# ml-jku/LaM-SLidE

Measured on AMD Instinct MI355X. Metric: sampled trajectories/sec (50-step ODE) + decoded-coord L2 vs ref, MD17, higher is better.
Workload: dtype bf16; 1 GPU; md17_bench; tail=False, ln_fuse=True, T=30, L=256, C=32, D=512, H=16, depth=4, sampler=ODE, state_updates=50, batch_per_gpu=32, global_batch=32, parallelism=batch-shard x1, 1 gather to rank 0 per step, noise_elem_stride_per_rank=7864320, kernels=general, trajectories_per_pass=32

## Files before the change

### include/lsl_api.h

```cpp
#ifndef LSL_API_H
#define LSL_API_H

#include <stddef.h>
#include <stdint.h>

#ifdef __cplusplus
extern "C" {
#endif
#if defined(__GNUC__)
#pragma GCC visibility push(default)
#endif

#define LSL_VERSION 6

typedef struct lsl_model lsl_model;

typedef struct lsl_model_desc {
    int32_t in_dim;
    int32_t hidden;
    int32_t heads;
    int32_t head_dim;
    int32_t head_dim_pad;
    int32_t mlp_dim;
    int32_t depth;
// ... 66 lines not shown
int32_t lsl_model_tail(const lsl_model *m);

int lsl_model_set_ln_fuse(lsl_model *m, int32_t on);
int32_t lsl_model_ln_fuse(const lsl_model *m);

int32_t lsl_pass_size(const lsl_model *m, int32_t B, int32_t T, int32_t L);

int32_t lsl_sampler_path(const lsl_model *m, int32_t T, int32_t L);

size_t lsl_workspace_bytes(const lsl_model *m, int32_t B, int32_t T, int32_t L);

int lsl_forward(lsl_model *m, const lsl_io *io, void *workspace, size_t workspace_bytes, void *stream);

size_t lsl_forward_jvp_workspace_bytes(const lsl_model *m, int32_t B, int32_t T, int32_t L);
int lsl_forward_jvp(lsl_model *m, const lsl_io *io, const float *x_tangent, float *out_tangent, void *workspace, size_t workspace_bytes,
                    void *stream);
int lsl_dot_rows(const float *a, const float *b, int32_t B, uint64_t per_trajectory, double *out, void *scratch, size_t scratch_bytes,
                 void *stream);

typedef struct lsl_si_row { float alpha, sigma, p, q1, q0, w; } lsl_si_row;
#define LSL_SI_SLAB 4096
size_t lsl_si_loss_workspace_bytes(const lsl_model *m, int32_t B, int32_t T, int32_t L);
int lsl_si_loss(lsl_model *m, const lsl_io *io, const float *x1, const float *x0, const lsl_si_row *rows, float *loss,
                void *workspace, size_t workspace_bytes, void *stream);
int lsl_si_reduce(const float *pred, const float *x1, const float *x0, const lsl_si_row *rows, int32_t B, uint64_t per_trajectory,
                  float *loss, void *scratch, size_t scratch_bytes, void *stream);

int lsl_geom_loss_sums(const float *pred, const float *target, const uint8_t *mask, int32_t F, int32_t A, int32_t D, float *sums, void *stream);
int lsl_geom_loss_final(const float *sums, int32_t F, float *out, void *stream);

int lsl_peptide_loss_sums(const float *pred, const float *target_frame, const uint8_t *atom14_mask, const float *tors_target, const uint8_t *tors_mask,
                          const int64_t *aatype, const int8_t *restab, int32_t F, int32_t R, int32_t kind, float *sums, void *stream);
int lsl_peptide_loss_final(const float *geom_sums, const float *pept_sums, int32_t F, float *out, void *stream);

int lsl_class_loss_sums(const float *logits, const int64_t *target, const uint8_t *mask, int32_t F, int32_t A, int32_t K, float label_smoothing,
                        float *sums, int64_t *confusion, void *stream);
int lsl_class_loss_final(const float *sums, int32_t F, float *out, void *stream);

int lsl_disp_error_rows(const float *pred, const float *target, int32_t K, int32_t B, int32_t Tp, int32_t t0p, int32_t Tt, int32_t t0t, int32_t Tf,
                        int32_t A, int32_t D, float *rows, float *traj, void *stream);
int lsl_disp_error_final(const float *rows, const float *traj, const uint8_t *mask, int32_t K, int32_t num_runs, int32_t B, int32_t A, float *agents,
                         double *totals, void *stream);

int lsl_dihedral_angles(const float *pos, const int32_t *quads, const int32_t *quads_host, int64_t F, int32_t A, int32_t Q, float *angles,
                        void *stream);
int lsl_histogram(const float *x, int32_t S, int32_t n, int32_t Q, const double *edges, int32_t bins, int64_t *counts, const int32_t *pairs,
                  const int32_t *pairs_host, int32_t P, const double *edges2a, const double *edges2b, int32_t bins2, int64_t *counts2, void *stream);
size_t lsl_lag_products_workspace_bytes(int32_t S, int32_t n, int32_t C, int32_t nlag);
int lsl_lag_products(const float *x, int32_t S, int32_t n, int32_t C, int32_t nlag, float *ac, void *workspace, size_t workspace_bytes, void *stream);
int lsl_js_distance(const int64_t *counts_a, const int64_t *counts_b, int32_t rows, int32_t bins, double *out, void *stream);

int lsl_pair_distances(const float *pos, const int32_t *pairs, const int32_t *pairs_host, int64_t F, int32_t A, int32_t P, float *dist,
                       void *stream);
int lsl_ca_frame_stats(const float *pos, const int32_t *sel, const int32_t *sel_host, int64_t F, int32_t A, int32_t R, float clash_thr,
                       float break_thr, float contact_thr, float *rg, int32_t *flags, int64_t *tally, int64_t *contacts, void *stream);
int lsl_histogram_columns(const float *x, int32_t n, int32_t Q, const double *edges, int32_t bins, int64_t *counts, void *stream);
int lsl_js_distance_density(const int64_t *counts_a, const int64_t *counts_b, const double *measure, int32_t rows, int32_t bins, double pseudo,
                            double *out, void *stream);

size_t lsl_lagged_moments_workspace_bytes(int32_t S, int32_t n, int32_t F, int32_t lag);
int lsl_lagged_moments(const float *x, int32_t S, int32_t n, int32_t F, int32_t lag, double *moments, void *workspace, size_t workspace_bytes,
                       void *stream);
int lsl_project(const float *x, int32_t n, int32_t F, const double *mean, const double *W, int32_t d, float *y, float *lim, void *stream);
int lsl_assign_centers(const float *y, int32_t n, int32_t d, const float *centers, int32_t k, const int32_t *map, int32_t nstates, int32_t *labels,
                       int64_t *state_counts, void *stream);
int lsl_transition_counts(const int32_t *dtraj, int32_t S, int32_t n, int32_t lag, int32_t nstates, int64_t *counts, void *stream);

size_t lsl_weighted_moments_workspace_bytes(int32_t n, int32_t F, int32_t lag);
int lsl_weighted_moments(const float *x, int32_t n, int32_t F, int32_t lag, const double *w, double *moments, void *workspace, size_t workspace_bytes,
                         void *stream);
int lsl_affine_weights(const float *x, int32_t m, int32_t F, const double *u, double c, double *w, void *stream);
int lsl_project_wide(const float *x, int32_t n, int32_t F, const double *mean, const double *W, int32_t d, float *y, float *lim, void *stream);

size_t lsl_kmeans_workspace_bytes(int32_t S, int32_t n, int32_t d, int32_t k);
int lsl_kmeans_step(const float *y, int32_t S, int32_t n, int32_t d, float *centers, int32_t k, int32_t *labels, int64_t *counts, double *state,
                    int32_t *done, int32_t update, double rel_tol, double center_tol, void *workspace, size_t workspace_bytes, void *stream);
int lsl_kmeans_nearest_rows(const float *y, int32_t S, int32_t n, int32_t d, const float *centers, int32_t k, int32_t *rows, void *stream);

int lsl_msm_active_set(const int64_t *counts, int32_t S, int32_t ns, int32_t *active, int32_t *n_active, void *stream);
int lsl_msm_reversible_step(const int64_t *counts, const int32_t *active, int32_t S, int32_t ns, int32_t iters, int32_t maxiter, double maxerr,
                            int32_t restart, double *x, int32_t *n_iter, double *err, int32_t *done, void *stream);
int lsl_msm_transition_matrix(const int64_t *counts, const int32_t *active, const double *x, int32_t S, int32_t ns, double *T, double *pi, void *stream);

#define LSL_SUP_CENTER_ONLY 1
int lsl_superpose(const float *pos, const float *ref, int32_t ref_frames, const int32_t *sel, const int32_t *sel_host, int32_t n_sel,
                  const uint8_t *fixed, int64_t F, int32_t A, int32_t flags, float *out, float *rmsd, double *rot, double *trans, void *stream);
size_t lsl_atom_rmsf_workspace_bytes(int64_t F, int32_t A);
int lsl_atom_rmsf(const float *pos, int64_t F, int32_t A, double *mean_out, float *rmsf_out, void *workspace, size_t workspace_bytes,
                  void *stream);

int lsl_sample_ex(lsl_model *m, const lsl_io *io, const lsl_step_ex *steps, int32_t n_steps,
                  const float *noise, int32_t n_noise, uint64_t seed, uint64_t elem_offset, float *trace, int32_t n_trace,
                  void *workspace, size_t workspace_bytes, void *stream);
int lsl_sample(lsl_model *m, const lsl_io *io, const lsl_step *steps, int32_t n_steps,
               const float *noise, int32_t n_noise, uint64_t seed, uint64_t elem_offset, float *trace,
               void *workspace, size_t workspace_bytes, void *stream);

int lsl_randn(float *x, uint64_t n, uint64_t seed, uint64_t elem_offset, void *stream);

#define LSL_RK_SCRATCH_BYTES 8192
int lsl_rk_lincomb(float *out, const float *const *x, const float *c, int32_t n_x, uint64_t n, void *stream);
int lsl_rk_dense(float *out, const float *a, const float *b, const float *c, const float *d, const float *e, float x, uint64_t n, void *stream);
int lsl_rk_error_ratio(float *ratio, const float *y0, const float *y1, const float *const *k, const float *c, int32_t n_k, float atol, float rtol,
                       uint64_t n, void *scratch, void *stream);

#define LSL_DOPRI_MAX_ATTEMPTS 100000
#define LSL_DOPRI_CTL_OFFSET 0
#define LSL_DOPRI_LOG_OFFSET 256
#define LSL_DOPRI_STATE_OFFSET (256 + 32 * LSL_DOPRI_MAX_ATTEMPTS)
enum { LSL_PATH_LINEAR = 0, LSL_PATH_GVP = 1, LSL_PATH_VP = 2 };
enum { LSL_PRED_VELOCITY = 0, LSL_PRED_DATA = 1, LSL_PRED_NOISE = 2, LSL_PRED_SCORE = 3 };
enum { LSL_DOPRI_OK = 0, LSL_DOPRI_MAX_STEPS = 1, LSL_DOPRI_NON_FINITE = 2 };
typedef struct lsl_dopri_desc {
    int32_t path_type, model_type, reverse, max_steps;
    double rtol, atol;
} lsl_dopri_desc;
typedef struct lsl_dopri_ctl {
    double t, dt, t_lo;
    double ratio, t_new, dt_next;
    double rtol, atol;
    float *out;
    int32_t accept, out_end;
    int32_t accepted, rejected, nfe, next_out, done, status;
    int32_t n_out, max_steps, path_type, model_type, reverse;
} lsl_dopri_ctl;
size_t lsl_dopri_workspace_bytes(const lsl_model *m, int32_t B, int32_t T, int32_t L, int32_t n_out);
int lsl_dopri_begin(lsl_model *m, const lsl_io *io, const lsl_dopri_desc *desc, const double *grid, int32_t n_out, float *out, void *workspace,
                    size_t workspace_bytes, void *stream);
int lsl_dopri_advance(lsl_model *m, const lsl_io *io, int32_t n_attempts, void *workspace, size_t workspace_bytes, void *stream);

#define LSL_DOPRI_EACH_SUMMARY_OFFSET 0
#define LSL_DOPRI_EACH_CTL_OFFSET 256
#define LSL_DOPRI_EACH_LOG_OFFSET(B) (256 + 256 * ((128 * (size_t)(B) + 255) / 256))
#define LSL_DOPRI_EACH_STATE_OFFSET(B, log_rows) (LSL_DOPRI_EACH_LOG_OFFSET(B) + 256 * ((32 * (size_t)(B) * (size_t)(log_rows) + 255) / 256))
typedef struct lsl_dopri_each_summary {
    int32_t B;
    int32_t n_done;
    int32_t n_failed;
    int32_t max_attempts;
    int32_t done;
} lsl_dopri_each_summary;
size_t lsl_dopri_each_workspace_bytes(const lsl_model *m, int32_t B, int32_t T, int32_t L, int32_t n_out, int32_t log_rows);
int lsl_dopri_each_begin(lsl_model *m, const lsl_io *io, const lsl_dopri_desc *desc, const double *grid, int32_t n_out, float *out,
                         int32_t log_rows, void *workspace, size_t workspace_bytes, void *stream);
int lsl_dopri_each_advance(lsl_model *m, const lsl_io *io, int32_t n_attempts, void *workspace, size_t workspace_bytes, void *stream);

int lsl_debug_dopri_coeffs(int32_t path_type, int32_t model_type, const float *t, int32_t n, double *out, void *stream);

int lsl_debug_block(lsl_model *m, int32_t block_index , const float *h_in, float *h_out,
                    const float *mods , int32_t B, int32_t T, int32_t L,
                    void *workspace, size_t workspace_bytes, void *stream);
int lsl_debug_block_ex(lsl_model *m, int32_t block_index, const float *h_in, float *h_out, void *a_out, const float *mods, int32_t mod_rows,
                       int32_t B, int32_t T, int32_t L, void *workspace, size_t workspace_bytes, void *stream);
int lsl_debug_taps(lsl_model *m, int32_t block_index, const float *h_in, const float *mods, int32_t B, int32_t T, int32_t L,
                   void *qkv_out, void *z_out, void *workspace, size_t workspace_bytes, void *stream);
int lsl_debug_mods(lsl_model *m, const float *t, const float *y, int32_t B, float *vec_out, float *mods_out,
                   void *workspace, size_t workspace_bytes, void *stream);
int lsl_debug_mods_ex(lsl_model *m, const float *t, float t_scalar, const float *y, int32_t B, float *vec_out, float *mods_out, float *tfeat_out,
                      float *hid_out, float *yhid_out, float *yemb_out, void *workspace, size_t workspace_bytes, void *stream);
int lsl_debug_mods_steps(lsl_model *m, const float *times, int32_t count, float *mods_out, float *vec_out, void *workspace, size_t workspace_bytes,
                         void *stream);
int lsl_debug_embed(lsl_model *m, const float *x, const float *x_cond, const int64_t *mask, int32_t B, int32_t T, int32_t L, float *cond_emb_out,
                    float *h_out, float *hn_out, void *stats_out, void *workspace, size_t workspace_bytes, void *stream);
int lsl_debug_head(lsl_model *m, const float *h, const float *mods, int32_t mod_rows, float *x, float *out, const lsl_step_ex *rec, const float *noise,
                   uint64_t seed, uint64_t elem_offset, float *trace, const float *saved, float *save_out, int32_t B, int32_t T, int32_t L,
                   void *stream);

int lsl_profile_enable(lsl_model *m, int32_t kernel, int32_t max_launches);
const char *lsl_profile_kernel_name(const lsl_model *m);
int lsl_profile_read(lsl_model *m, double *total_ms, int32_t *launches);

typedef struct lsl_dec_block {
    const float *ln_w, *ln_b;
    const float *lnc_w, *lnc_b;
    const float *w_q;
    const float *w_kv;
    const float *w_out, *b_out;
    const float *q_scale, *k_scale;
    const float *ff_ln_w, *ff_ln_b;
    const float *ff_w1, *ff_b1;
    const float *ff_w2, *ff_b2;
} lsl_dec_block;

typedef struct lsl_decoder_desc {
    int32_t in_dim;
    int32_t dim_latent, dim_query, dim_emb, n_entities;
    int32_t heads_latent, dim_head_latent, heads_cross, dim_head_cross;
    int32_t num_block_attn, num_block_cross;
    int32_t act;
    int32_t out_dim;
    int32_t num_split;
} lsl_decoder_desc;

typedef struct lsl_decoder_weights {
    const float *pq_w, *pq_b;
    const float *table;
    const float *qm_w, *qm_b;
    const lsl_dec_block *self_blocks;
    const lsl_dec_block *cross_blocks;
    lsl_dec_block out_block;
    const float *ext_w, *ext_b;
    const float *head_w1, *head_b1;
    const float *head_w2, *head_b2;
} lsl_decoder_weights;

typedef struct lsl_decoder lsl_decoder;
int lsl_decoder_create(const lsl_decoder_desc *desc, const lsl_decoder_weights *w, lsl_decoder **out);
void lsl_decoder_destroy(lsl_decoder *d);
size_t lsl_decode_workspace_bytes(const lsl_decoder *d, int32_t frames, int32_t L, int32_t A);
int lsl_decode(lsl_decoder *d, const float *z, const int64_t *entities, int32_t frames, int32_t L, int32_t A, float *out,
               void *workspace, size_t workspace_bytes, void *stream);

#define LSL_DECODE_MAX_HEADS 8
typedef struct lsl_decoder_head {
    const float *w1, *b1;
    const float *w2, *b2;
    int32_t out_dim;
} lsl_decoder_head;
int lsl_decode_heads(lsl_decoder *d, const lsl_decoder_head *heads, int32_t n_heads, const float *z, const int64_t *entities,
                     int32_t frames, int32_t L, int32_t A, float *const *outs, void *workspace, size_t workspace_bytes, void *stream);

typedef struct lsl_encoder_desc {
    int32_t dim_input, dim_emb, n_entities, dim_latent, num_latents;
    int32_t heads_cross, dim_head_cross, heads_latent, dim_head_latent;
    int32_t num_block_cross, num_block_attn;
    int32_t act;
} lsl_encoder_desc;

typedef struct lsl_encoder_weights {
    const float *table;
    const float *mlp_w1, *mlp_b1;
    const float *mlp_w2, *mlp_b2;
    const float *latents;
    const lsl_dec_block *cross_blocks;
    const lsl_dec_block *self_blocks;
    const float *quant_w, *quant_b;
} lsl_encoder_weights;

typedef struct lsl_encoder lsl_encoder;
int lsl_encoder_create(const lsl_encoder_desc *desc, const lsl_encoder_weights *w, lsl_encoder **out);
void lsl_encoder_destroy(lsl_encoder *e);
size_t lsl_encode_workspace_bytes(const lsl_encoder *e, int32_t frames, int32_t A);
int lsl_encode(lsl_encoder *e, const float *x, const int64_t *entities, const unsigned char *mask, int32_t frames, int32_t A, float *out,
               void *workspace, size_t workspace_bytes, void *stream);

#if defined(__GNUC__)
#pragma GCC visibility pop
#endif
#ifdef __cplusplus
}
#endif
#endif
```

### lam_slide_amd/_lib.py

```python
from __future__ import annotations

import ctypes as C
import os
import subprocess
from collections import OrderedDict
from typing import Optional

import torch

_HERE = os.path.dirname(os.path.abspath(__file__))
LIB_PATH = os.path.join(_HERE, "liblamslide_hip.so")
SRC_DIR = os.path.join(_HERE, "csrc")
INCLUDE_DIR = os.path.join(os.path.dirname(_HERE), "include")

ABI_VERSION = 6
RK_SCRATCH_BYTES = 8192
GEOM_MAX_A, GEOM_MAX_D = 2048, 4
DISP_MAX_D, DISP_MAX_UNITS = 4, 16777215
TORS_MAX_A, TORS_MAX_Q, HIST_MAX_BINS, HIST2_MAX_BINS = 2044, 65536, 2048, 90
LAG_CHUNK, LAG_MAX_LAGS, LAG_MAX_ROWS = 448, 1 << 21, 65535
MOM_SEG = 1024
MOM_CHAIN = MOM_SEG
MOM_MAX_F, PROJ_MAX_D = 128, 16
ASG_MAX_K, ASG_MAX_D, ASG_CELLS, ASG_MAX_STATES, TR_MAX_STATES = 1024, 64, 8192, 1024, 128
KM_SEG, KM_MAX_S = 2048, 65535
WMOM_MIN_F, WMOM_MAX_F, WPROJ_MAX_D = 129, 2048, 64
WMOM_SEG, WMOM_CHAIN = 1024, 4130
PAIR_MAX_P, CA_MAX_R = 65536, 146
SI_SLAB = 4096
CLS_MAX_K, CLS_IGNORE = 128, -100

EXPORTED = (
    "lsl_version", "lsl_build_info", "lsl_last_error", "lsl_model_create", "lsl_model_set_weights", "lsl_model_destroy",
    "lsl_model_set_chunk", "lsl_model_set_attention_mode", "lsl_model_set_tail", "lsl_model_tail", "lsl_model_set_ln_fuse", "lsl_model_ln_fuse", "lsl_profile_kernel_name", "lsl_pass_size", "lsl_sampler_path", "lsl_workspace_bytes", "lsl_forward", "lsl_sample", "lsl_sample_ex", "lsl_debug_block", "lsl_debug_block_ex", "lsl_debug_taps", "lsl_debug_mods",
    "lsl_debug_mods_ex", "lsl_debug_mods_steps", "lsl_debug_embed", "lsl_debug_head",
    "lsl_si_loss_workspace_bytes", "lsl_si_loss", "lsl_si_reduce", "lsl_geom_loss_sums", "lsl_geom_loss_final",
    "lsl_peptide_loss_sums", "lsl_peptide_loss_final", "lsl_disp_error_rows", "lsl_disp_error_final",
    "lsl_dihedral_angles", "lsl_histogram", "lsl_lag_products_workspace_bytes", "lsl_lag_products", "lsl_js_distance",
    "lsl_pair_distances", "lsl_ca_frame_stats", "lsl_histogram_columns", "lsl_js_distance_density",
    "lsl_lagged_moments_workspace_bytes", "lsl_lagged_moments", "lsl_project", "lsl_assign_centers", "lsl_transition_counts",
    "lsl_kmeans_workspace_bytes", "lsl_kmeans_step", "lsl_kmeans_nearest_rows",
    "lsl_weighted_moments_workspace_bytes", "lsl_weighted_moments", "lsl_affine_weights", "lsl_project_wide",
    "lsl_msm_active_set", "lsl_msm_reversible_step", "lsl_msm_transition_matrix",
    "lsl_superpose", "lsl_atom_rmsf_workspace_bytes", "lsl_atom_rmsf",
    "lsl_profile_enable", "lsl_profile_read", "lsl_randn", "lsl_rk_lincomb", "lsl_rk_dense", "lsl_rk_error_ratio",
    "lsl_dopri_workspace_bytes", "lsl_dopri_begin", "lsl_dopri_advance", "lsl_debug_dopri_coeffs",
    "lsl_dopri_each_workspace_bytes", "lsl_dopri_each_begin", "lsl_dopri_each_advance",
    "lsl_forward_jvp_workspace_bytes", "lsl_forward_jvp", "lsl_dot_rows",
    "lsl_decoder_create", "lsl_decoder_destroy", "lsl_decode_workspace_bytes", "lsl_decode",
    "lsl_encoder_create", "lsl_encoder_destroy", "lsl_encode_workspace_bytes", "lsl_encode",
    "lsl_decode_heads", "lsl_class_loss_sums", "lsl_class_loss_final",
)


def mom_segments(n: int, lag: int) -> int:
    return -(-(int(n) - int(lag)) // MOM_SEG)


class ModelDesc(C.Structure):
    _fields_ = [(n, C.c_int32) for n in ("in_dim", "hidden", "heads", "head_dim", "head_dim_pad", "mlp_dim", "depth",
                                         "vec_in_dim", "normalize")] + [("theta", C.c_float)]


class BlockWeights(C.Structure):
    _fields_ = [(n, C.c_void_p) for n in ("w1", "b1", "qs", "ks", "w2", "b2")]


class Weights(C.Structure):
    _fields_ = [(n, C.c_void_p) for n in (
        "x_in_w", "x_in_b", "cond_w", "cond_b", "mask_emb", "time_freqs", "time_w1", "time_b1", "time_w2", "time_b2",
        "vec_w1", "vec_b1", "vec_w2", "vec_b2", "mod_w", "mod_b", "out_w", "out_b")] + [("blocks", C.POINTER(BlockWeights))]


class IO(C.Structure):
    _fields_ = [("x", C.c_void_p), ("x_cond", C.c_void_p), ("mask", C.c_void_p), ("y", C.c_void_p), ("t", C.c_void_p),
                ("out", C.c_void_p), ("B", C.c_int32), ("T", C.c_int32), ("L", C.c_int32)]


class DecBlock(C.Structure):
    _fields_ = [(n, C.c_void_p) for n in ("ln_w", "ln_b", "lnc_w", "lnc_b", "w_q", "w_kv", "w_out", "b_out", "q_scale", "k_scale",
                                          "ff_ln_w", "ff_ln_b", "ff_w1", "ff_b1", "ff_w2", "ff_b2")]


class DecoderDesc(C.Structure):
    _fields_ = [(n, C.c_int32) for n in ("in_dim", "dim_latent", "dim_query", "dim_emb", "n_entities", "heads_latent", "dim_head_latent",
                                         "heads_cross", "dim_head_cross", "num_block_attn", "num_block_cross", "act", "out_dim", "num_split")]


class DecoderWeights(C.Structure):
    _fields_ = [("pq_w", C.c_void_p), ("pq_b", C.c_void_p), ("table", C.c_void_p), ("qm_w", C.c_void_p), ("qm_b", C.c_void_p),
                ("self_blocks", C.POINTER(DecBlock)), ("cross_blocks", C.POINTER(DecBlock)), ("out_block", DecBlock),
                ("ext_w", C.c_void_p), ("ext_b", C.c_void_p), ("head_w1", C.c_void_p), ("head_b1", C.c_void_p), ("head_w2", C.c_void_p), ("head_b2", C.c_void_p)]


class DecoderHead(C.Structure):
    _fields_ = [("w1", C.c_void_p), ("b1", C.c_void_p), ("w2", C.c_void_p), ("b2", C.c_void_p), ("out_dim", C.c_int32)]


class EncoderDesc(C.Structure):
    _fields_ = [(n, C.c_int32) for n in ("dim_input", "dim_emb", "n_entities", "dim_latent", "num_latents", "heads_cross", "dim_head_cross",
                                         "heads_latent", "dim_head_latent", "num_block_cross", "num_block_attn", "act")]


class EncoderWeights(C.Structure):
    _fields_ = [("table", C.c_void_p), ("mlp_w1", C.c_void_p), ("mlp_b1", C.c_void_p), ("mlp_w2", C.c_void_p), ("mlp_b2", C.c_void_p),
                ("latents", C.c_void_p), ("cross_blocks", C.POINTER(DecBlock)), ("self_blocks", C.POINTER(DecBlock)),
                ("quant_w", C.c_void_p), ("quant_b", C.c_void_p)]


class Step(C.Structure):
    _fields_ = [("t", C.c_float), ("ax", C.c_float), ("am", C.c_float), ("aw", C.c_float)]


class StepEx(C.Structure):
    _fields_ = [("t", C.c_float), ("ax", C.c_float), ("am", C.c_float), ("aw", C.c_float), ("as_", C.c_float), ("flags", C.c_int32),
                ("noise_index", C.c_int32), ("trace_index", C.c_int32)]


class SiRow(C.Structure):
    _fields_ = [(n, C.c_float) for n in ("alpha", "sigma", "p", "q1", "q0", "w")]


STEP_NO_NETWORK, STEP_SAVE = 1, 2


class DopriDesc(C.Structure):
    _fields_ = [(n, C.c_int32) for n in ("path_type", "model_type", "reverse", "max_steps")] + [("rtol", C.c_double), ("atol", C.c_double)]


class DopriCtl(C.Structure):
    _fields_ = [(n, C.c_double) for n in ("t", "dt", "t_lo", "ratio", "t_new", "dt_next", "rtol", "atol")] + [("out", C.c_void_p)] + [
        (n, C.c_int32) for n in ("accept", "out_end", "accepted", "rejected", "nfe", "next_out", "done", "status", "n_out", "max_steps", "path_type",
                                 "model_type", "reverse")]


class DopriEachSummary(C.Structure):
    _fields_ = [(n, C.c_int32) for n in ("B", "n_done", "n_failed", "max_attempts", "done")]


class Dopri:
    MAX_ATTEMPTS = 100000
    CTL_OFFSET, LOG_OFFSET, STATE_OFFSET = 0, 256, 256 + 32 * MAX_ATTEMPTS
    PATHS = {"LINEAR": 0, "GVP": 1, "VP": 2}
    PREDICTIONS = {"VELOCITY": 0, "DATA": 1, "NOISE": 2, "SCORE": 3}
    STATUS_MAX_STEPS, STATUS_NON_FINITE = 1, 2
    EACH_SUMMARY_OFFSET, EACH_CTL_OFFSET, EACH_CTL_STRIDE, EACH_MAX_B = 0, 256, 128, 65535

    @staticmethod
    def each_log_offset(B: int) -> int:
        return 256 + 256 * ((128 * int(B) + 255) // 256)

    @staticmethod
    def each_state_offset(B: int, log_rows: int) -> int:
        return Dopri.each_log_offset(B) + 256 * ((32 * int(B) * int(log_rows) + 255) // 256)


BASE_FLAGS = ("-O3", "--offload-arch=gfx950", "-std=c++17", "-fPIC", "-fvisibility=hidden", "-Wno-unused-value")
UNITS = (("lsl_api.hip", ()), ("unit_lin1.hip", ("-fno-slp-vectorize",)), ("unit_loss.hip", ()), ("unit_stat.hip", ()), ("unit_stage1.hip", ()))
BUILD_DIR = os.path.join(_HERE, "build")


def unit_options(extra) -> str:
    return " ".join(BASE_FLAGS[:1] + tuple(extra))


def build(force: bool = False, verbose: bool = False) -> str:
    from concurrent.futures import ThreadPoolExecutor
    srcs = [os.path.join(SRC_DIR, f) for f in sorted(os.listdir(SRC_DIR))] + [os.path.join(INCLUDE_DIR, "lsl_api.h"), os.path.abspath(__file__)]
    if not force and os.path.exists(LIB_PATH) and all(os.path.getmtime(LIB_PATH) >= os.path.getmtime(s) for s in srcs):
        return LIB_PATH
    hipcc = os.environ.get("HIPCC", "/opt/rocm/bin/hipcc")
    os.makedirs(BUILD_DIR, exist_ok=True)

    def run(cmd):
        res = subprocess.run(cmd, capture_output=True, text=True)
        if verbose or res.returncode != 0:
            print(" ".join(cmd))
            print(res.stdout + res.stderr)
        if res.returncode != 0:
            raise RuntimeError("hipcc failed building liblamslide_hip.so")

    objs = [os.path.join(BUILD_DIR, os.path.splitext(name)[0] + ".o") for name, _ in UNITS]
    cmds = [[hipcc, *BASE_FLAGS, *extra, f'-DLSL_UNIT_OPTIONS="{unit_options(extra)}"', "-c", os.path.join(SRC_DIR, name), "-o", obj]
            for (name, extra), obj in zip(UNITS, objs)]
    with ThreadPoolExecutor(max_workers=min(16, len(cmds))) as pool:
        list(pool.map(run, cmds))
    run([hipcc, "--offload-arch=gfx950", "-shared", "-fPIC", "-Wl,--version-script=" + os.path.join(SRC_DIR, "exports.map"), "-o", LIB_PATH, *objs])
    return LIB_PATH


class LibraryMissing(RuntimeError):
    """liblamslide_hip.so has not been built (the only failure a caller may treat as "no library": anything else - a HIP error, an
    out-of-memory condition - propagates)."""


_lib: Optional[C.CDLL] = None


def load() -> C.CDLL:
    global _lib
    if _lib is not None:
        return _lib
    if not os.path.exists(LIB_PATH):
        raise LibraryMissing(f"{LIB_PATH} is missing: run `python -c 'import __graft_entry__ as g; g.build()'` "
                           "(the HIP extension is the only compute path of lam_slide_amd)")
    lib = C.CDLL(LIB_PATH)
    missing = [s for s in EXPORTED if not hasattr(lib, s)]
    if missing:
        raise RuntimeError(f"{LIB_PATH} is stale: it lacks {', '.join(missing)}; rebuild it (python -c 'import __graft_entry__ as g; g.build()')")
    lib.lsl_version.restype = C.c_int
    lib.lsl_build_info.restype = C.c_char_p
    lib.lsl_last_error.restype = C.c_char_p
    lib.lsl_model_create.argtypes = [C.POINTER(ModelDesc), C.POINTER(C.c_void_p)]
    lib.lsl_model_set_weights.argtypes = [C.c_void_p, C.POINTER(Weights)]
    lib.lsl_model_destroy.argtypes = [C.c_void_p]
    lib.lsl_model_destroy.restype = None
    lib.lsl_model_set_chunk.argtypes = [C.c_void_p, C.c_int32]
    lib.lsl_model_set_attention_mode.argtypes = [C.c_void_p, C.c_int32]
    lib.lsl_model_set_tail.argtypes = [C.c_void_p, C.c_int32]
    lib.lsl_model_tail.argtypes = [C.c_void_p]
    lib.lsl_model_set_ln_fuse.argtypes = [C.c_void_p, C.c_int32]
    lib.lsl_model_ln_fuse.argtypes = [C.c_void_p]
    lib.lsl_profile_kernel_name.argtypes = [C.c_void_p]
    lib.lsl_profile_kernel_name.restype = C.c_char_p
    lib.lsl_pass_size.argtypes = [C.c_void_p, C.c_int32, C.c_int32, C.c_int32]
    lib.lsl_sampler_path.argtypes = [C.c_void_p, C.c_int32, C.c_int32]
    lib.lsl_workspace_bytes.argtypes = [C.c_void_p, C.c_int32, C.c_int32, C.c_int32]
    lib.lsl_workspace_bytes.restype = C.c_size_t
    lib.lsl_forward.argtypes = [C.c_void_p, C.POINTER(IO), C.c_void_p, C.c_size_t, C.c_void_p]
    lib.lsl_sample.argtypes = [C.c_void_p, C.POINTER(IO), C.POINTER(Step), C.c_int32, C.c_void_p, C.c_int32, C.c_uint64, C.c_uint64,
                               C.c_void_p, C.c_void_p, C.c_size_t, C.c_void_p]
    lib.lsl_sample_ex.argtypes = [C.c_void_p, C.POINTER(IO), C.POINTER(StepEx), C.c_int32, C.c_void_p, C.c_int32, C.c_uint64, C.c_uint64,
                                  C.c_void_p, C.c_int32, C.c_void_p, C.c_size_t, C.c_void_p]
    lib.lsl_debug_block.argtypes = [C.c_void_p, C.c_int32, C.c_void_p, C.c_void_p, C.c_void_p, C.c_int32, C.c_int32, C.c_int32,
                                    C.c_void_p, C.c_size_t, C.c_void_p]
    lib.lsl_debug_block_ex.argtypes = [C.c_void_p, C.c_int32, C.c_void_p, C.c_void_p, C.c_void_p, C.c_void_p, C.c_int32, C.c_int32, C.c_int32,
                                       C.c_int32, C.c_void_p, C.c_size_t, C.c_void_p]
    lib.lsl_debug_taps.argtypes = [C.c_void_p, C.c_int32, C.c_void_p, C.c_void_p, C.c_int32, C.c_int32, C.c_int32, C.c_void_p, C.c_void_p,
                                   C.c_void_p, C.c_size_t, C.c_void_p]
    lib.lsl_debug_mods.argtypes = [C.c_void_p, C.c_void_p, C.c_void_p, C.c_int32, C.c_void_p, C.c_void_p, C.c_void_p, C.c_size_t,
                                   C.c_void_p]
    lib.lsl_debug_mods_ex.argtypes = [C.c_void_p, C.c_void_p, C.c_float, C.c_void_p, C.c_int32] + [C.c_void_p] * 6 + [C.c_void_p, C.c_size_t, C.c_void_p]
    lib.lsl_debug_mods_steps.argtypes = [C.c_void_p, C.POINTER(C.c_float), C.c_int32, C.c_void_p, C.c_void_p, C.c_void_p, C.c_size_t, C.c_void_p]
    lib.lsl_debug_embed.argtypes = [C.c_void_p, C.c_void_p, C.c_void_p, C.c_void_p, C.c_int32, C.c_int32, C.c_int32] + [C.c_void_p] * 4 + [
        C.c_void_p, C.c_size_t, C.c_void_p]
    lib.lsl_debug_head.argtypes = [C.c_void_p, C.c_void_p, C.c_void_p, C.c_int32, C.c_void_p, C.c_void_p, C.POINTER(StepEx), C.c_void_p, C.c_uint64,
                                   C.c_uint64, C.c_void_p, C.c_void_p, C.c_void_p, C.c_int32, C.c_int32, C.c_int32, C.c_void_p]
    lib.lsl_forward_jvp_workspace_bytes.argtypes = [C.c_void_p, C.c_int32, C.c_int32, C.c_int32]
    lib.lsl_forward_jvp_workspace_bytes.restype = C.c_size_t
    lib.lsl_forward_jvp.argtypes = [C.c_void_p, C.POINTER(IO), C.c_void_p, C.c_void_p, C.c_void_p, C.c_size_t, C.c_void_p]
    lib.lsl_dot_rows.argtypes = [C.c_void_p, C.c_void_p, C.c_int32, C.c_uint64, C.c_void_p, C.c_void_p, C.c_size_t, C.c_void_p]
    lib.lsl_si_loss_workspace_bytes.argtypes = [C.c_void_p, C.c_int32, C.c_int32, C.c_int32]
    lib.lsl_si_loss_workspace_bytes.restype = C.c_size_t
    lib.lsl_si_loss.argtypes = [C.c_void_p, C.POINTER(IO), C.c_void_p, C.c_void_p, C.c_void_p, C.c_void_p, C.c_void_p, C.c_size_t, C.c_void_p]
    lib.lsl_si_reduce.argtypes = [C.c_void_p, C.c_void_p, C.c_void_p, C.c_void_p, C.c_int32, C.c_uint64, C.c_void_p, C.c_void_p, C.c_size_t,
                                  C.c_void_p]
    lib.lsl_geom_loss_sums.argtypes = [C.c_void_p, C.c_void_p, C.c_void_p, C.c_int32, C.c_int32, C.c_int32, C.c_void_p, C.c_void_p]
    lib.lsl_geom_loss_final.argtypes = [C.c_void_p, C.c_int32, C.c_void_p, C.c_void_p]
    lib.lsl_peptide_loss_sums.argtypes = [C.c_void_p] * 7 + [C.c_int32, C.c_int32, C.c_int32, C.c_void_p, C.c_void_p]
    lib.lsl_peptide_loss_final.argtypes = [C.c_void_p, C.c_void_p, C.c_int32, C.c_void_p, C.c_void_p]
    lib.lsl_disp_error_rows.argtypes = [C.c_void_p, C.c_void_p] + [C.c_int32] * 9 + [C.c_void_p, C.c_void_p, C.c_void_p]
    lib.lsl_disp_error_final.argtypes = [C.c_void_p, C.c_void_p, C.c_void_p] + [C.c_int32] * 4 + [C.c_void_p, C.c_void_p, C.c_void_p]
    lib.lsl_dihedral_angles.argtypes = [C.c_void_p, C.c_void_p, C.c_void_p, C.c_int64, C.c_int32, C.c_int32, C.c_void_p, C.c_void_p]
    lib.lsl_histogram.argtypes = [C.c_void_p] + [C.c_int32] * 3 + [C.c_void_p, C.c_int32, C.c_void_p, C.c_void_p, C.c_void_p, C.c_int32, C.c_void_p,
                                  C.c_void_p, C.c_int32, C.c_void_p, C.c_void_p]
    lib.lsl_lag_products_workspace_bytes.argtypes = [C.c_int32] * 4
    lib.lsl_lag_products_workspace_bytes.restype = C.c_size_t
    lib.lsl_lag_products.argtypes = [C.c_void_p] + [C.c_int32] * 4 + [C.c_void_p, C.c_void_p, C.c_size_t, C.c_void_p]
    lib.lsl_js_distance.argtypes = [C.c_void_p, C.c_void_p, C.c_int32, C.c_int32, C.c_void_p, C.c_void_p]
    lib.lsl_pair_distances.argtypes = [C.c_void_p, C.c_void_p, C.c_void_p, C.c_int64, C.c_int32, C.c_int32, C.c_void_p, C.c_void_p]
    lib.lsl_ca_frame_stats.argtypes = [C.c_void_p, C.c_void_p, C.c_void_p, C.c_int64, C.c_int32, C.c_int32, C.c_float, C.c_float, C.c_float] + [C.c_void_p] * 5
    lib.lsl_histogram_columns.argtypes = [C.c_void_p, C.c_int32, C.c_int32, C.c_void_p, C.c_int32, C.c_void_p, C.c_void_p]
    lib.lsl_js_distance_density.argtypes = [C.c_void_p, C.c_void_p, C.c_void_p, C.c_int32, C.c_int32, C.c_double, C.c_void_p, C.c_void_p]
    lib.lsl_lagged_moments_workspace_bytes.argtypes = [C.c_int32] * 4
    lib.lsl_lagged_moments_workspace_bytes.restype = C.c_size_t
    lib.lsl_lagged_moments.argtypes = [C.c_void_p] + [C.c_int32] * 4 + [C.c_void_p, C.c_void_p, C.c_size_t, C.c_void_p]
    lib.lsl_project.argtypes = [C.c_void_p, C.c_int32, C.c_int32, C.c_void_p, C.c_void_p, C.c_int32, C.c_void_p, C.c_void_p, C.c_void_p]
    lib.lsl_assign_centers.argtypes = [C.c_void_p, C.c_int32, C.c_int32, C.c_void_p, C.c_int32, C.c_void_p, C.c_int32, C.c_void_p, C.c_void_p, C.c_void_p]
    lib.lsl_transition_counts.argtypes = [C.c_void_p] + [C.c_int32] * 4 + [C.c_void_p, C.c_void_p]
    lib.lsl_weighted_moments_workspace_bytes.argtypes = [C.c_int32] * 3
    lib.lsl_weighted_moments_workspace_bytes.restype = C.c_size_t
    lib.lsl_weighted_moments.argtypes = [C.c_void_p] + [C.c_int32] * 3 + [C.c_void_p, C.c_void_p, C.c_void_p, C.c_size_t, C.c_void_p]
    lib.lsl_affine_weights.argtypes = [C.c_void_p, C.c_int32, C.c_int32, C.c_void_p, C.c_double, C.c_void_p, C.c_void_p]
    lib.lsl_project_wide.argtypes = [C.c_void_p, C.c_int32, C.c_int32, C.c_void_p, C.c_void_p, C.c_int32, C.c_void_p, C.c_void_p, C.c_void_p]
    lib.lsl_kmeans_workspace_bytes.argtypes = [C.c_int32] * 4
    lib.lsl_kmeans_workspace_bytes.restype = C.c_size_t
    lib.lsl_kmeans_step.argtypes = [C.c_void_p] + [C.c_int32] * 3 + [C.c_void_p, C.c_int32] + [C.c_void_p] * 4 + [C.c_int32, C.c_double, C.c_double,
                                    C.c_void_p, C.c_size_t, C.c_void_p]
    lib.lsl_kmeans_nearest_rows.argtypes = [C.c_void_p] + [C.c_int32] * 3 + [C.c_void_p, C.c_int32, C.c_void_p, C.c_void_p]
    lib.lsl_msm_active_set.argtypes = [C.c_void_p, C.c_int32, C.c_int32, C.c_void_p, C.c_void_p, C.c_void_p]
    lib.lsl_msm_reversible_step.argtypes = [C.c_void_p, C.c_void_p] + [C.c_int32] * 4 + [C.c_double, C.c_int32] + [C.c_void_p] * 5
    lib.lsl_msm_transition_matrix.argtypes = [C.c_void_p] * 3 + [C.c_int32, C.c_int32, C.c_void_p, C.c_void_p, C.c_void_p]
    lib.lsl_superpose.argtypes = [C.c_void_p, C.c_void_p, C.c_int32, C.c_void_p, C.c_void_p, C.c_int32, C.c_void_p, C.c_int64, C.c_int32, C.c_int32] + [C.c_void_p] * 5
    lib.lsl_atom_rmsf_workspace_bytes.argtypes = [C.c_int64, C.c_int32]
    lib.lsl_atom_rmsf_workspace_bytes.restype = C.c_size_t
    lib.lsl_atom_rmsf.argtypes = [C.c_void_p, C.c_int64, C.c_int32, C.c_void_p, C.c_void_p, C.c_void_p, C.c_size_t, C.c_void_p]
    lib.lsl_randn.argtypes = [C.c_void_p, C.c_uint64, C.c_uint64, C.c_uint64, C.c_void_p]
    lib.lsl_rk_lincomb.argtypes = [C.c_void_p, C.POINTER(C.c_void_p), C.POINTER(C.c_float), C.c_int32, C.c_uint64, C.c_void_p]
    lib.lsl_rk_dense.argtypes = [C.c_void_p] * 6 + [C.c_float, C.c_uint64, C.c_void_p]
    lib.lsl_rk_error_ratio.argtypes = [C.c_void_p, C.c_void_p, C.c_void_p, C.POINTER(C.c_void_p), C.POINTER(C.c_float), C.c_int32, C.c_float, C.c_float,
                                       C.c_uint64, C.c_void_p, C.c_void_p]
    lib.lsl_dopri_workspace_bytes.argtypes = [C.c_void_p] + [C.c_int32] * 4
    lib.lsl_dopri_workspace_bytes.restype = C.c_size_t
    lib.lsl_dopri_begin.argtypes = [C.c_void_p, C.POINTER(IO), C.POINTER(DopriDesc), C.POINTER(C.c_double), C.c_int32, C.c_void_p, C.c_void_p, C.c_size_t,
                                    C.c_void_p]
    lib.lsl_dopri_advance.argtypes = [C.c_void_p, C.POINTER(IO), C.c_int32, C.c_void_p, C.c_size_t, C.c_void_p]
    lib.lsl_dopri_each_workspace_bytes.argtypes = [C.c_void_p] + [C.c_int32] * 5
    lib.lsl_dopri_each_workspace_bytes.restype = C.c_size_t
    lib.lsl_dopri_each_begin.argtypes = [C.c_void_p, C.POINTER(IO), C.POINTER(DopriDesc), C.POINTER(C.c_double), C.c_int32, C.c_void_p, C.c_int32, C.c_void_p,
                                         C.c_size_t, C.c_void_p]
    lib.lsl_dopri_each_advance.argtypes = [C.c_void_p, C.POINTER(IO), C.c_int32, C.c_void_p, C.c_size_t, C.c_void_p]
    lib.lsl_debug_dopri_coeffs.argtypes = [C.c_int32, C.c_int32, C.c_void_p, C.c_int32, C.c_void_p, C.c_void_p]
    lib.lsl_profile_enable.argtypes = [C.c_void_p, C.c_int32, C.c_int32]
    lib.lsl_profile_read.argtypes = [C.c_void_p, C.POINTER(C.c_double), C.POINTER(C.c_int32)]
    lib.lsl_decoder_create.argtypes = [C.POINTER(DecoderDesc), C.POINTER(DecoderWeights), C.POINTER(C.c_void_p)]
    lib.lsl_decoder_destroy.argtypes = [C.c_void_p]
    lib.lsl_decoder_destroy.restype = None
    lib.lsl_decode_workspace_bytes.argtypes = [C.c_void_p, C.c_int32, C.c_int32, C.c_int32]
    lib.lsl_decode_workspace_bytes.restype = C.c_size_t
    lib.lsl_decode.argtypes = [C.c_void_p, C.c_void_p, C.c_void_p, C.c_int32, C.c_int32, C.c_int32, C.c_void_p, C.c_void_p, C.c_size_t,
                               C.c_void_p]
    lib.lsl_decode_heads.argtypes = [C.c_void_p, C.POINTER(DecoderHead), C.c_int32, C.c_void_p, C.c_void_p, C.c_int32, C.c_int32, C.c_int32,
                                     C.POINTER(C.c_void_p), C.c_void_p, C.c_size_t, C.c_void_p]
    lib.lsl_class_loss_sums.argtypes = [C.c_void_p, C.c_void_p, C.c_void_p, C.c_int32, C.c_int32, C.c_int32, C.c_float, C.c_void_p, C.c_void_p,
                                        C.c_void_p]
    lib.lsl_class_loss_final.argtypes = [C.c_void_p, C.c_int32, C.c_void_p, C.c_void_p]
    lib.lsl_encoder_create.argtypes = [C.POINTER(EncoderDesc), C.POINTER(EncoderWeights), C.POINTER(C.c_void_p)]
    lib.lsl_encoder_destroy.argtypes = [C.c_void_p]
    lib.lsl_encoder_destroy.restype = None
    lib.lsl_encode_workspace_bytes.argtypes = [C.c_void_p, C.c_int32, C.c_int32]
    lib.lsl_encode_workspace_bytes.restype = C.c_size_t
    lib.lsl_encode.argtypes = [C.c_void_p, C.c_void_p, C.c_void_p, C.c_void_p, C.c_int32, C.c_int32, C.c_void_p, C.c_void_p, C.c_size_t,
                               C.c_void_p]
    if lib.lsl_version() != ABI_VERSION:
        raise RuntimeError(f"liblamslide_hip.so reports ABI version {lib.lsl_version()}, this package binds version {ABI_VERSION}: rebuild it "
                           "(python -c 'import __graft_entry__ as g; g.build()')")
    _lib = lib
    return lib


def last_error() -> str:
    return load().lsl_last_error().decode()


def check(rc: int):
    if rc == 0:
        return
    msg = last_error()
    if rc in (-3, -20, -21):
        raise ValueError(msg)
    raise RuntimeError(f"lamslide_hip error {rc}: {msg}")


def call(dev, name: str, *args) -> None:
    fn = getattr(load(), name)
    with torch.cuda.device(dev):
        check(fn(*args, torch.cuda.current_stream(dev).cuda_stream))


def to_host(t: "torch.Tensor"):
    if not t.is_cuda:
        return t.numpy()
    mode = torch.cuda.get_sync_debug_mode()
    torch.cuda.set_sync_debug_mode("default")
    try:
        return t.cpu().numpy()
    finally:
        torch.cuda.set_sync_debug_mode(mode)


def to_device(a, dev) -> "torch.Tensor":
    import numpy as np
    t = torch.from_numpy(np.ascontiguousarray(a))
    if torch.device(dev).type != "cuda":
        return t
    mode = torch.cuda.get_sync_debug_mode()
    torch.cuda.set_sync_debug_mode("default")
    try:
        return t.to(dev)
    finally:
        torch.cuda.set_sync_debug_mode(mode)


def device_form(*tensors, dtype=torch.float32, same_device: bool = True) -> bool:
    dev, grad = tensors[0].device, torch.is_grad_enabled()
    return all(t.is_cuda and t.dtype == dtype and (t.device == dev or not same_device) and not (grad and t.requires_grad) for t in tensors)


def flat(x, lead: tuple, trailing: tuple, dtype, dev, shape_error, device_error) -> "torch.Tensor":
    if tuple(x.shape) != tuple(lead) + tuple(trailing):
# ... 47 lines not shown
```

### lam_slide_amd/csrc/host_eval.hip.h

```cpp
#pragma once
#include "host_launch.hip.h"

namespace {


int run_mods(lsl_model *m, const Workspace &ws, const float *t_dev, float t_scalar, const float *yemb, int rows,
             float *vec_out, float *mods_out, hipStream_t st) {
    const lsl_weights &w = m->w;
    const int D = m->d.hidden;
    m->prof.begin(6, st);
    hipLaunchKernelGGL(k_time_features, dim3((rows * 128 + 255) / 256), dim3(256), 0, st, ws.tfeat, t_dev, t_scalar, w.time_freqs, rows);
    const bool single = !t_dev && !yemb;
    char k1[32], k2[32], k3[32];
    const bool lab = m->prof.kernel == 6;
    launch_dense<false, true>(ws.hid, ws.tfeat, w.time_w1, w.time_b1, nullptr, rows, 256, D, 0, st, single, 0, lab ? k1 : nullptr);
    launch_dense<false, false>(vec_out, ws.hid, w.time_w2, w.time_b2, yemb, rows, D, D, D, st, single, 0, lab ? k2 : nullptr);
    launch_dense<true, false>(mods_out, vec_out, w.mod_w, w.mod_b, nullptr, rows, D, m->MODW, 0, st, single, 0, lab ? k3 : nullptr);
    if (lab) m->prof.label(6, "k_time_features > %s > %s > %s", k1, k2, k3);
    m->prof.end(6, st);
    LSL_CHECK_LAUNCH("modulation");
    return 0;
}

int run_mods_steps(lsl_model *m, const Workspace &ws, const float *times, int count, hipStream_t st) {
    const lsl_weights &w = m->w;
    const int D = m->d.hidden;
    m->prof.begin(6, st);
    for (int c0 = 0; c0 < count; c0 += 48) {
        StepTimes tt;
        const int nc = std::min(48, count - c0);
        for (int s = 0; s < nc; ++s) tt.t[s] = times[c0 + s];
        hipLaunchKernelGGL(k_time_features_steps, dim3((nc * 128 + 255) / 256), dim3(256), 0, st, ws.tf_all + (size_t)c0 * 256, tt, nc, 1, w.time_freqs);
    }
    const unsigned gy = (unsigned)((count + 7) / 8);
    hipLaunchKernelGGL((k_dense_rows<false, true>), dim3((D + 3) / 4, gy), dim3(256), 0, st, ws.hid_all, ws.tf_all, w.time_w1, w.time_b1, nullptr, count, 256, D, 0, 0);
    hipLaunchKernelGGL((k_dense_rows<false, false>), dim3((D + 3) / 4, gy), dim3(256), 0, st, ws.vec_all, ws.hid_all, w.time_w2, w.time_b2, nullptr, count, D, D, D, 0);
    hipLaunchKernelGGL((k_dense_rows<true, false>), dim3((m->MODW + 3) / 4, (unsigned)((count + 15) / 16)), dim3(256), 0, st, ws.mods_all, ws.vec_all, w.mod_w, w.mod_b, nullptr, count, D, m->MODW, 0, 0);
    m->prof.label(6, "k_time_features_steps > k_dense_rows<0, 1> > k_dense_rows<0, 0> > k_dense_rows<1, 0> (row ranges of 8, 8, 16)");
    m->prof.end(6, st);
    LSL_CHECK_LAUNCH("modulation (group of records)");
    return 0;
}

int run_yemb(lsl_model *m, const Workspace &ws, const float *y, int rows, hipStream_t st, float *yhid_tap = nullptr) {
    const lsl_weights &w = m->w;
    const int D = m->d.hidden, V = m->d.vec_in_dim;
    char k1[32], k2[32];
    const bool lab = m->prof.kernel == 6;
    launch_dense<false, true>(ws.hid, y, w.vec_w1, w.vec_b1, nullptr, rows, V, D, 0, st, false, 0, lab ? k1 : nullptr);
    if (yhid_tap) hipMemcpyAsync(yhid_tap, ws.hid, (size_t)rows * D * 4, hipMemcpyDeviceToDevice, st);
    launch_dense<false, false>(ws.yemb, ws.hid, w.vec_w2, w.vec_b2, nullptr, rows, D, D, 0, st, false, 0, lab ? k2 : nullptr);
    if (lab) m->prof.label(6, "%s > %s", k1, k2);
    LSL_CHECK_LAUNCH("vec_in");
    return 0;
}

void run_tables(const lsl_model *m, const Workspace &ws, int T, int L, hipStream_t st) {
    const int half = m->d.head_dim_pad / 2;
    if (ws.w2p) {
        const size_t per = (size_t)m->d.hidden * m->K2;
        for (int bi = 0; bi < 2 * m->d.depth; ++bi)
            hipLaunchKernelGGL(k_lin2_pack, dim3(128), dim3(256), 0, st, ws.w2p + (size_t)bi * per, (const u16 *)m->blocks[bi].w2, m->d.hidden, m->K2);
    }
    if (ws.wtail) {
        for (int bi = 0; bi < 2 * m->d.depth; ++bi)
            hipLaunchKernelGGL(k_tail_pack, dim3(256), dim3(256), 0, st, ws.wtail + (size_t)bi * ws.wtail_stride, (const u16 *)m->blocks[bi].w1,
                               (const u16 *)m->blocks[bi].w2, m->d.hidden, m->HHD, m->d.mlp_dim);
    }
    hipLaunchKernelGGL(k_rope_table, dim3((L * half + 255) / 256), dim3(256), 0, st, ws.rope_l, L, m->d.head_dim, m->d.head_dim_pad, m->d.theta);
    hipLaunchKernelGGL(k_rope_table, dim3((T * half + 255) / 256), dim3(256), 0, st, ws.rope_t, T, m->d.head_dim, m->d.head_dim_pad, m->d.theta);
    const int nb = 2 * m->d.depth;
    for (int b0 = 0; b0 < 2 * nb; b0 += 16) {
        RopeScaledJobs jobs{};
        jobs.n_jobs = std::min(16, 2 * nb - b0);
        int max_pos = 0;
        for (int k = 0; k < jobs.n_jobs; ++k) {
            const int t = b0 + k, bi = t >> 1;
            jobs.out[k] = ws.rope_qk + (size_t)t * ws.rope_qk_stride;
            jobs.scale[k] = (t & 1) ? m->blocks[bi].ks : m->blocks[bi].qs;
            jobs.n_pos[k] = (bi & 1) ? T : L;
            jobs.sq_bound[k] = ws.kmax2 + ((t & 1) ? 0 : nb) + bi;
            max_pos = std::max(max_pos, jobs.n_pos[k]);
        }
        hipLaunchKernelGGL(k_rope_scaled, dim3((max_pos * half + 255) / 256, jobs.n_jobs), dim3(256), 0, st, jobs, m->d.head_dim, m->d.head_dim_pad, m->d.theta);
    }
}


enum class PlanMode { eval, debug_block, debug_taps };
enum class Lin2Kind { none, tail, ws, gemm };

struct PassPlan {
    PlanMode mode;
    int bc, n, npad, T, L, mod_stride, blocks;
    bool tail;
    int F1;
    bool lin1_ts;
    int lin1_waves;
    bool ln_stats;
    bool emb_stats;
    int gemm1;
    bool planes[2];
    AttnPlan attn[2];
    Lin2Kind lin2;
    Lin2Grid l2grid;
    int gemm2;

    bool a_from_tail(int bi) const { return mode == PlanMode::eval && tail && bi > 0; }
    bool lin1_lnf(int bi) const { return mode == PlanMode::eval && ln_stats && (bi > 0 || emb_stats); }
    bool lin2_stats(int bi) const { return ln_stats && bi + 1 < blocks; }
};

int plan_pass(const lsl_model *m, const Workspace &ws, int bc, int T, int L, int mod_stride, PlanMode mode, int block, PassPlan &p) {
    const lsl_model_desc &d = m->d;
    const int D = d.hidden, n = bc * T * L;
    p = PassPlan{};
    p.mode = mode;
    p.bc = bc;
    p.n = n;
    p.npad = (n + 255) & ~255;
    p.T = T;
    p.L = L;
    p.mod_stride = mod_stride;
    p.blocks = 2 * d.depth;
    p.tail = m->tail && mode != PlanMode::debug_taps;
    p.F1 = p.tail ? 3 * m->HHD : m->F1;
    p.lin1_ts = linear1_ts_ok(d.head_dim_pad, D, p.F1, m->HHD, n);
    p.lin1_waves = linear1_ts_waves(D, n);
    p.ln_stats = m->ln_fuse && !m->tail && ws.w2p && mode != PlanMode::debug_taps &&
                 linear1_lnf_ok(d.head_dim_pad, D, m->F1, m->HHD, n, T * L, mod_stride);
    p.emb_stats = p.ln_stats && mode == PlanMode::eval && !d.normalize && embed_stats_ok(d.in_dim, D);
    if (!p.lin1_ts) p.gemm1 = gemm_variant(false, p.F1, D, n);
    for (int t = 0; t < 2; ++t) {
        p.attn[t] = plan_attention(m->attention_linear, d.head_dim_pad, d.heads, d.head_dim, bc, T, L, t != 0);
        p.planes[t] = qkv_planes_ok(d.head_dim_pad, d.heads, t ? T : L, t != 0, p.lin1_ts, p.attn[t]);
    }
    const bool ws_reach = ws.w2p && (unsigned long long)n * (unsigned)(4 * D) < (1ull << 32);
    if (ws_reach) p.l2grid = linear2_ws_grid(D, n, T * L, mod_stride == 0);
    const bool on_ws = ws_reach && p.l2grid.gate_rows <= linear2_ws_max_gate_rows(m->K2);
    p.lin2 = mode == PlanMode::debug_taps ? Lin2Kind::none : p.tail ? Lin2Kind::tail : on_ws ? Lin2Kind::ws : Lin2Kind::gemm;
    if (p.lin2 == Lin2Kind::gemm) p.gemm2 = gemm_variant(true, D, m->K2, n);

    const int b0 = mode == PlanMode::eval ? 0 : block, b1 = mode == PlanMode::eval ? p.blocks : block + 1;
    for (int bi = b0; bi < b1; ++bi) {
        const int temporal = bi & 1, pdiv = temporal ? L : 1, pmod = temporal ? T : L;
        if ((unsigned long long)n * (unsigned)std::max(pdiv, pmod) >= (1ull << 32)) return fail(-3, "pass too large for the position arithmetic");
        if (p.planes[temporal] && (unsigned long long)p.npad * 3ull * (unsigned)m->HHD * 2ull >= (1ull << 32))
            return fail(-3, "pass too large for the q/k/v plane offsets (%d tokens: at most %llu with this model)", n, (unsigned long long)((1ull << 32) / (6ull * (unsigned)m->HHD)) - 256);
        if (p.attn[temporal].form == AttnForm::none)
            return fail(-3, "attention axis of %d positions is not on the stream kernel and too long for k_attention_rows (at most %d positions at %d-wide heads)",
                        pmod, attention_rows_max_s(d.head_dim_pad), d.head_dim_pad);
        if (p.lin2 == Lin2Kind::none) continue;
        if ((unsigned long long)n * (unsigned)(T * L) >= (1ull << 32)) return fail(-3, "pass too large for the trajectory arithmetic");
        if (p.tail && (unsigned long long)p.npad * (unsigned)(4 * D) >= (1ull << 32)) return fail(-3, "pass too large for the residual-stream offsets");
        if (p.lin2_stats(bi) && !on_ws) {
            if (ws_reach) return fail(-3, "ln_fuse: a pass of %d tokens has too many trajectories per token range for k_linear2_ws; use smaller passes (lsl_model_set_chunk)", n);
            return fail(-3, "ln_fuse: pass too large for the residual-stream offsets (%d tokens)", n);
        }
    }
    return 0;
}

struct CallPlans {
    PassPlan full, rest;
    const PassPlan &of(int bc) const { return bc == full.bc ? full : rest; }
};
int plan_call(const lsl_model *m, const Workspace &ws, const lsl_io *io, int chunk, int mod_stride, CallPlans &cp) {
    if (int rc = plan_pass(m, ws, chunk, io->T, io->L, mod_stride, PlanMode::eval, 0, cp.full)) return rc;
    if (io->B % chunk) return plan_pass(m, ws, io->B % chunk, io->T, io->L, mod_stride, PlanMode::eval, 0, cp.rest);
    return 0;
}

void label_block(lsl_model *m, const PassPlan &p, int bi) {
    const lsl_model_desc &d = m->d;
    Profiler &pr = m->prof;
    switch (pr.kernel) {
        case 0:
            if (!p.lin1_ts) pr.label(0, "k_gemm_glds<EpiLinear1<%d>> (tiling %d)", d.head_dim_pad, p.gemm1);
            else if (p.lin1_lnf(bi)) pr.label(0, "k_linear1_ts<%d, %d, 8, true> (LayerNorm fused)", d.head_dim_pad, d.hidden);
            else pr.label(0, "k_linear1_ts<%d, %d, %d>%s", d.head_dim_pad, d.hidden, p.lin1_waves, p.tail ? " (q | k | v)" : "");
            break;
        case 1:
            if (p.lin2 == Lin2Kind::tail) pr.label(1, "k_tail<%d, %d>", d.hidden, m->HHD);
            else if (p.lin2 == Lin2Kind::ws) pr.label(1, p.lin2_stats(bi) ? "k_linear2_ws<%d> (+ row statistics)" : "k_linear2_ws<%d>", m->K2);
            else if (p.lin2 == Lin2Kind::gemm) pr.label(1, "k_gemm_glds<EpiLinear2> (tiling %d)", p.gemm2);
            break;
        case 2: {
            const AttnPlan &a = p.attn[bi & 1];
            pr.label(2, "%s", a.form == AttnForm::linear ? "k_attention_linear" : a.stream() ? "k_attention_stream" : "k_attention_rows / k_attention_tiny");
            break;
        }
        default: break;
    }
}

unsigned magic_of(int dv) { return dv == 1 ? 0u : (unsigned)((1ull << 32) / (unsigned)dv + 1); }

template <int HDP>
void launch_linear1_gemm(const lsl_model *m, const Workspace &ws, const PassPlan &p, int bi, int pdiv, int pmod, float premul, hipStream_t st) {
    const lsl_block_weights &bw = m->blocks[bi];
    const EpiLinear1<HDP> e{bw.b1, bw.qs, bw.ks, (bi & 1) ? ws.rope_t : ws.rope_l, ws.rope_qk + (size_t)(2 * bi) * ws.rope_qk_stride,
                            ws.rope_qk + (size_t)(2 * bi + 1) * ws.rope_qk_stride, ws.qkv, ws.z, m->HHD, m->d.mlp_dim,
                            pdiv, pmod, magic_of(pdiv), magic_of(pmod), 1.0f / m->d.head_dim, premul, 0};
    launch_gemm(p.gemm1, (const u16 *)bw.w1, ws.a, p.F1, p.n, m->d.hidden, e, st, m->HHD);
}

AttnArgs attention_args(const lsl_model *m, const Workspace &ws, const PassPlan &p, int bi, float premul) {
    const lsl_model_desc &d = m->d;
    const AttnPlan &ap = p.attn[bi & 1];
    static const int nt_mask = tune_int("LSL_NT", 3);
    static const int attn_bound = tune_int("LSL_ATTN_BOUND", 1);
    AttnArgs aa{};
    aa.nt = (nt_mask >> 2) & 1;
    aa.qkv = ws.qkv; aa.z = ws.z; aa.HHD = m->HHD; aa.zw = m->K2; aa.H = d.heads; aa.hd = d.head_dim; aa.premul = premul;
    aa.kmax2 = ws.kmax2 + bi;
    aa.qmax2 = ws.kmax2 + 2 * d.depth + bi;
    aa.planes = p.planes[bi & 1] ? 1 : 0;
    aa.npad = p.npad;
    aa.bound = attn_bound == 2 || (attn_bound == 1 && ((bi & 1) ? p.T : p.L) > 96);
    aa.S = ap.S; aa.n_seq = ap.n_seq; aa.inner = ap.inner; aa.outer_stride = ap.outer_stride; aa.pos_stride = ap.pos_stride;
    aa.blk = ap.blk; aa.n_tok = ap.n_tok;
    return aa;
}

struct EvalTangent {
    virtual int embedded() = 0;
    virtual int normed(int bi, const float *mbase) = 0;
    virtual int attended(int bi, const float *mbase, float premul, int pdiv, int pmod) = 0;
    virtual int head(const float *fm) = 0;
    virtual ~EvalTangent() = default;
};

int run_block(lsl_model *m, const Workspace &ws, const PassPlan &p, int bi, const float *mods, hipStream_t st, void *a_tap = nullptr,
              EvalTangent *tg = nullptr) {
    const lsl_model_desc &d = m->d;
    const lsl_block_weights &bw = m->blocks[bi];
    const int D = d.hidden, n = p.n, tpt = p.T * p.L, mod_stride = p.mod_stride, temporal = bi & 1;
    const float *mbase = mods + (size_t)(bi / 2) * 6 * D + (temporal ? 3 * D : 0);
    const bool lnf = p.lin1_lnf(bi);
    const float premul = m->attention_linear ? 1.0f : (float)(1.4426950408889634 / std::sqrt((double)d.head_dim));
    const int pdiv = temporal ? p.L : 1, pmod = temporal ? p.T : p.L;
    label_block(m, p, bi);
    if (!p.a_from_tail(bi) && !lnf) {
        m->prof.begin(3, st);
        DISPATCH_D(D, launch_ln_mod_t, ws.a, ws.h, mbase, mbase + D, mod_stride, n, tpt, st);
        m->prof.end(3, st);
        if (a_tap) hipMemcpyAsync(a_tap, ws.a, (size_t)n * D * 2, hipMemcpyDeviceToDevice, st);
    }
    if (tg)
        if (int rc = tg->normed(bi, mbase)) return rc;
    m->prof.begin(0, st);
    if (p.lin1_ts) {
        const Lin1Args la{(const u16 *)bw.w1, lnf ? (const u16 *)ws.h : ws.a, bw.b1, ws.rope_qk + (size_t)(2 * bi) * ws.rope_qk_stride,
                          ws.rope_qk + (size_t)(2 * bi + 1) * ws.rope_qk_stride, ws.qkv, ws.z, p.F1, n, m->HHD, d.mlp_dim,
                          pdiv, pmod, magic_of(pdiv), magic_of(pmod), 1.0f / d.head_dim, premul, 1, 0, p.planes[temporal] ? 1 : 0, p.npad,
                          ws.lnstat, mbase, mbase + D, mod_stride, tpt, magic_of(tpt)};
        launch_linear1_ts(d.head_dim_pad, D, p.lin1_waves, lnf, la, st);
    } else if (d.head_dim_pad == 32) launch_linear1_gemm<32>(m, ws, p, bi, pdiv, pmod, premul, st);
    else launch_linear1_gemm<16>(m, ws, p, bi, pdiv, pmod, premul, st);
    m->prof.end(0, st);

    const AttnArgs aa = attention_args(m, ws, p, bi, premul);
    m->prof.begin(2, st);
    if (d.head_dim_pad == 32) launch_attention_t<32>(p.attn[temporal], aa, st);
    else launch_attention_t<16>(p.attn[temporal], aa, st);
    m->prof.end(2, st);
    if (p.lin2 == Lin2Kind::none) {
        LSL_CHECK_LAUNCH("block");
        return 0;
    }
    if (tg)
        if (int rc = tg->attended(bi, mbase, premul, pdiv, pmod)) return rc;
    m->prof.begin(1, st);
    if (p.lin2 == Lin2Kind::tail) {
        const bool next = bi + 1 < 2 * d.depth;
        const float *nb = mods + (size_t)((bi + 1) / 2) * 6 * D + (((bi + 1) & 1) ? 3 * D : 0);
        const TailArgs ta{ws.wtail + (size_t)bi * ws.wtail_stride, ws.a, ws.z, bw.b1 + 3 * m->HHD, bw.b2, mbase + 2 * D, ws.h, next ? ws.a : nullptr,
                          nb, nb + D, n, d.mlp_dim, m->K2, mod_stride, tpt, magic_of(tpt)};
        launch_tail(ta, st);
    } else if (p.lin2 == Lin2Kind::ws) {
        const bool stats = p.lin2_stats(bi);
        const Lin2Args l2{ws.w2p + (size_t)bi * D * m->K2, ws.z, bw.b2, mbase + 2 * D, ws.h, D, n, mod_stride, tpt, magic_of(tpt),
                          p.l2grid.slices, p.l2grid.rpx, p.l2grid.gate_rows, stats ? ws.lnparts : nullptr, p.npad};
        launch_linear2_ws(m->K2, l2, st);
        if (stats) hipLaunchKernelGGL(k_ln_finalize, dim3((n + 255) / 256), dim3(256), 0, st, ws.lnstat, ws.lnparts, D / 32, p.npad, n, 32.0f);
    } else {
        const EpiLinear2 e2{bw.b2, mbase + 2 * D, ws.h, D, mod_stride, tpt, 0, magic_of(tpt)};
        launch_gemm(p.gemm2, (const u16 *)bw.w2, ws.z, D, n, m->K2, e2, st);
    }
    m->prof.end(1, st);
    LSL_CHECK_LAUNCH(p.lin2 == Lin2Kind::tail ? "block (tail)" : "block");
    return 0;
}

struct EvalArgs {
    float *x = nullptr;
    float *out = nullptr;
    const float *t = nullptr;
    bool have_y = false;
    const lsl_step_ex *rec = nullptr;
    const float *noise = nullptr;
    uint64_t seed = 0, elem_off = 0;
    float *trace = nullptr;
    const float *saved = nullptr;
    float *save_out = nullptr;
    const float *mods_ready = nullptr;
};
StepUpdate step_update(const EvalArgs &e) {
    const lsl_step_ex r = e.rec ? *e.rec : lsl_step_ex{};
    return StepUpdate{e.noise, e.trace, e.saved, e.save_out, (unsigned long long)e.seed, (unsigned long long)e.elem_off, r.ax, r.am, r.aw, r.as, (unsigned)r.noise_index};
}

int run_embed(lsl_model *m, const Workspace &ws, const PassPlan &p, const float *x, hipStream_t st, float *h_tap = nullptr, EvalTangent *tg = nullptr) {
    const lsl_model_desc &d = m->d;
    const int D = d.hidden, n = p.n;
    m->prof.begin(5, st);
    launch_embed<1>(ws.h, x, m->w.x_in_w, nullptr, nullptr, nullptr, nullptr, ws.cond_emb, n, d.in_dim, D, st, p.emb_stats ? ws.lnparts : nullptr, p.npad,
                    &m->prof);
    if (p.emb_stats) hipLaunchKernelGGL(k_ln_finalize, dim3((n + 255) / 256), dim3(256), 0, st, ws.lnstat, ws.lnparts, D / 256, p.npad, n, 256.0f);
    if (h_tap) hipMemcpyAsync(h_tap, ws.h, (size_t)n * D * 4, hipMemcpyDeviceToDevice, st);
    if (tg)
        if (int rc = tg->embedded()) return rc;
    if (d.normalize) { DISPATCH_D(D, launch_ln_inplace_t, ws.h, n, 1e-5f, st); }
    m->prof.end(5, st);
    LSL_CHECK_LAUNCH("embed");
    return 0;
}

int run_head(lsl_model *m, const float *h, const float *fm, int mod_stride, int n, int tpt, const EvalArgs &e, hipStream_t st) {
    const int D = m->d.hidden;
    const HeadArgs a{e.x, e.out, h, fm, fm + D, mod_stride, m->w.out_w, m->w.out_b, n, m->d.in_dim, tpt, e.rec ? 1 : 0, step_update(e)};
    m->prof.begin(4, st);
    DISPATCH_D(D, launch_head_mfma, a, st, &m->prof);
    m->prof.end(4, st);
    LSL_CHECK_LAUNCH("head");
    return 0;
}

int run_eval(lsl_model *m, const Workspace &ws, const PassPlan &p, const EvalArgs &e, hipStream_t st, EvalTangent *tg = nullptr) {
    const lsl_model_desc &d = m->d;
    const int D = d.hidden, n = p.n;
    const lsl_step_ex r = e.rec ? *e.rec : lsl_step_ex{};
    const bool shared = p.mod_stride == 0;
    int rc = 0;
    const float *mods = ws.mods;
    if (e.mods_ready && shared) mods = e.mods_ready;
    else rc = run_mods(m, ws, e.t, r.t, e.have_y ? ws.yemb : nullptr, shared ? 1 : p.bc, ws.vec, ws.mods, st);
    if (rc) return rc;
    if ((rc = run_embed(m, ws, p, e.x, st, nullptr, tg))) return rc;
    for (int bi = 0; bi < 2 * d.depth; ++bi)
        if ((rc = run_block(m, ws, p, bi, mods, st, nullptr, tg))) return rc;
    const float *fm = mods + (size_t)d.depth * 6 * D;
    if ((rc = run_head(m, ws.h, fm, p.mod_stride, n, p.T * p.L, e, st))) return rc;
    return tg ? tg->head(fm) : 0;
}

int prepare_pass(lsl_model *m, const Workspace &ws, const float *x_cond, const int64_t *mask, const float *y, int bc, int T,
                 int L, hipStream_t st) {
    const lsl_model_desc &d = m->d;
    const int n = bc * T * L;
    launch_embed<0>(ws.cond_emb, x_cond, m->w.cond_w, m->w.cond_b, m->w.x_in_b, m->w.mask_emb, mask, nullptr, n, d.in_dim, d.hidden, st, nullptr, 0, &m->prof);
    LSL_CHECK_LAUNCH("cond_embed");
    if (y) return run_yemb(m, ws, y, bc, st);
    return 0;
}

bool resident_ok(const lsl_model *m, int T, int L) {
    static const int off = env_int("LSL_RESIDENT", 1) == 0;
    const lsl_model_desc &d = m->d;
    return !off && !m->attention_linear && d.hidden == RES_D && d.heads == RES_H && d.head_dim == RES_HD && d.head_dim_pad == RES_HD && d.mlp_dim == RES_M &&
           d.in_dim <= RES_MAX_C && d.in_dim % 4 == 0 && 2 * d.depth <= RES_MAX_BLOCKS && (long)T * L <= 48 && T <= 32 && L <= 32;
}

struct ResWorkspace {
    float *cond_emb, *yemb, *tfeat, *hid, *vec, *mods, *blkpar;
    u16 *blkw;
    int steps_per_launch;
    size_t bytes;
};
ResWorkspace carve_resident(const lsl_model *m, char *base, int B, int T, int L, bool have_y) {
    const size_t n = (size_t)B * T * L, D = m->d.hidden;
    size_t off = 0;
    auto take = [&](size_t bytes) {
        char *p = base ? base + off : nullptr;
        off += align_up(bytes, 256);
        return p;
    };
    ResWorkspace ws;
    const size_t rows = have_y ? (size_t)B : 1;
    size_t spl = ((size_t)256 << 20) / (rows * m->MODW * 4);
    ws.steps_per_launch = (int)std::max<size_t>(1, std::min<size_t>(spl, RES_MAX_STEPS));
    const size_t rt = rows * ws.steps_per_launch;
    ws.cond_emb = (float *)take(n * D * 4);
    ws.yemb = (float *)take((size_t)B * D * 4);
    ws.tfeat = (float *)take(rt * 256 * 4);
    ws.hid = (float *)take(std::max(rt, (size_t)B) * D * 4);
    ws.vec = (float *)take(rt * D * 4);
    ws.mods = (float *)take(rt * m->MODW * 4);
    ws.blkpar = (float *)take((size_t)2 * m->d.depth * RES_P_SHIFT * 4);
    ws.blkw = (u16 *)take((size_t)2 * m->d.depth * (RES_W1_ELEMS + RES_W2_ELEMS) * 2);
    ws.bytes = off;
    return ws;
}

template <int NNT>
void launch_resident(const ResArgs &a, int B, int T, int L, hipStream_t st) {
    auto kern = k_resident<NNT>;
    const size_t lds = ResLds<NNT>::bytes(T, L);
    LSL_ALLOW_LDS(kern, (size_t)163840);
    hipLaunchKernelGGL(kern, dim3(B), dim3(RES_NTHR), lds, st, a);
}

int resident_sample(lsl_model *m, const lsl_io *io, const lsl_step *steps, int n_steps, const float *noise, uint64_t seed, uint64_t elem_offset,
                    float *trace, void *workspace, hipStream_t st) {
    const lsl_model_desc &d = m->d;
    const lsl_weights &w = m->w;
    const int B = io->B, T = io->T, L = io->L, n_t = T * L, D = d.hidden;
    const bool have_y = io->y != nullptr;
    const ResWorkspace ws = carve_resident(m, (char *)workspace, B, T, L, have_y);
// ... 128 lines not shown
```

### lam_slide_amd/csrc/host_launch.hip.h

```cpp
#pragma once
#include <atomic>
#include <type_traits>

#include "host_common.hip.h"

namespace {

struct HeadArgs {
    float *x, *out;
    const float *h, *shift, *scale;
    int mod_stride;
    const float *Wo, *bo;
    int n, C, tpt, do_step;
    StepUpdate u;
};

#ifdef LSL_EXPERIMENTS
constexpr bool lsl_experiments = true;
template <int NE, int VEC>
bool launch_head_experiment(const HeadArgs &, hipStream_t);
template <class Epi>
bool launch_gemm_experiment(int, const GemmArgs &, const Epi &, hipStream_t, bool);
#else
constexpr bool lsl_experiments = false;
// ... 42 lines not shown
void launch_ln_inplace_t(float *h, int n, float eps, hipStream_t st) {
    hipLaunchKernelGGL((k_ln_inplace<NE, VEC>), dim3((n + 3) / 4), dim3(256), 0, st, h, n, eps);
}
template <int NE, int VEC>
void launch_head_mfma(const HeadArgs &a, hipStream_t st, Profiler *pr = nullptr) {
    if (launch_head_experiment<NE, VEC>(a, st)) return;
    auto kern = k_head_step_mfma<NE, VEC>;
    const size_t lds = head_mfma_lds_bytes<NE>(a.C <= 32);
    LSL_ALLOW_LDS(kern, head_mfma_lds_bytes<NE>(false));
    static const int per_cu = tune_int("LSL_HEAD_PER_CU", 2);
    const int wgs = device_cus() * (per_cu >= 2 && 2 * lds <= LDS_BUDGET ? 2 : 1);
    if (pr) pr->label(4, "k_head_step_mfma<%d, %d> (%s, %d per CU)", NE, VEC, a.C <= 32 ? "one slab" : "cycled slabs", wgs / device_cus());
    hipLaunchKernelGGL(kern, dim3(std::min((a.n + HEAD_TOK - 1) / HEAD_TOK, wgs)), dim3(256), lds, st, a.x, a.out, a.h, a.shift, a.scale, a.mod_stride,
                       a.Wo, a.bo, a.n, a.C, a.tpt, a.do_step, a.u);
}
void launch_state_affine(float *x, unsigned long long n, const StepUpdate &u, hipStream_t st) {
    hipLaunchKernelGGL(k_state_affine, dim3((unsigned)std::min<unsigned long long>((n + 255) / 256, 2048)), dim3(256), 0, st, x, n, u);
}

#define DISPATCH_D(D, FN, ...)                          \
    switch ((D) / 64) {                                 \
        case 1: FN<1, 1>(__VA_ARGS__); break;           \
        case 2: FN<2, 2>(__VA_ARGS__); break;           \
        case 3: FN<3, 1>(__VA_ARGS__); break;           \
        case 4: FN<4, 2>(__VA_ARGS__); break;           \
        case 5: FN<5, 1>(__VA_ARGS__); break;           \
        case 6: FN<6, 2>(__VA_ARGS__); break;           \
        case 7: FN<7, 1>(__VA_ARGS__); break;           \
        default: FN<8, 2>(__VA_ARGS__); break;          \
    }

bool embed_stats_ok(int C, int D) { return C <= 32 && D % 256 == 0 && D <= 512; }
template <int MODE>
int launch_embed(float *out, const float *in, const float *W, const float *b, const float *b2, const float *me,
                 const int64_t *mask, const float *base, int n, int C, int D, hipStream_t st, float2 *stats = nullptr, int npad = 0,
                 Profiler *pr = nullptr) {
    if (C > 32 && C % 8 == 0 && C <= 128 && D % 32 == 0) {
        const int tpw = 3, ngrp = (D / 32 + tpw - 1) / tpw;
        const long units = (long)((n + 31) / 32) * ngrp;
        const dim3 g((unsigned)((units + 3) / 4));
        if (pr) pr->label(5, "k_embed_mfma<%d, %d> (32-token tiles)", MODE, C / 8);
        switch (C / 8) {
#define LSL_EMB_CASE(CK) case CK: hipLaunchKernelGGL((k_embed_mfma<MODE, CK>), g, dim3(256), 0, st, out, in, W, b, b2, me, mask, base, n, C, D, tpw); return 0;
            LSL_EMB_CASE(5) LSL_EMB_CASE(6) LSL_EMB_CASE(7) LSL_EMB_CASE(8) LSL_EMB_CASE(9) LSL_EMB_CASE(10) LSL_EMB_CASE(11) LSL_EMB_CASE(12)
            LSL_EMB_CASE(13) LSL_EMB_CASE(14) LSL_EMB_CASE(15) LSL_EMB_CASE(16)
#undef LSL_EMB_CASE
        }
    }
    int tok = EMB_TOK;
    static const int stage = tune_int("LSL_EMBED_LDS", 1);
    const bool w_lds = stage && C == 32 && D % 4 == 0 && D <= 512;
    if (w_lds)
        while (tok > 16 && (n + tok - 1) / tok < 2 * device_cus()) tok /= 2;
    const dim3 grid(std::min((n + tok - 1) / tok, 2 * device_cus())), blk(256);
    const bool with_stats = stats && MODE == 1 && C <= 32 && embed_stats_ok(C, D);
    if (pr)
        pr->label(5, "k_embed<%d, %d, %d%s> (%d-token tiles%s)", C <= 32 ? 32 : C <= 64 ? 64 : C <= 96 ? 96 : 128, MODE, C <= 32 ? 4 : C <= 96 ? 2 : 1,
                  with_stats ? ", true" : "", tok, w_lds ? ", weights through LDS" : (C & 3) ? ", scalar weight loads" : "");
    if (C <= 32) {
        const size_t lds = w_lds ? embed_w_lds_bytes<32, 4>(D) : 0;
        if (with_stats) {
            auto kern = k_embed<32, 1, 4, true>;
            LSL_ALLOW_LDS(kern, (embed_w_lds_bytes<32, 4>(512)));
            hipLaunchKernelGGL(kern, grid, blk, lds, st, out, in, W, b, b2, me, mask, base, n, C, D, w_lds ? 1 : 0, tok, stats, npad);
            return 0;
        }
        auto kern = k_embed<32, MODE, 4>;
        LSL_ALLOW_LDS(kern, (embed_w_lds_bytes<32, 4>(512)));
        hipLaunchKernelGGL(kern, grid, blk, lds, st, out, in, W, b, b2, me, mask, base, n, C, D, w_lds ? 1 : 0, tok, (float2 *)nullptr, 0);
    } else if (C <= 64) hipLaunchKernelGGL((k_embed<64, MODE, 2>), grid, blk, 0, st, out, in, W, b, b2, me, mask, base, n, C, D, 0, tok, (float2 *)nullptr, 0);
    else if (C <= 96) hipLaunchKernelGGL((k_embed<96, MODE, 2>), grid, blk, 0, st, out, in, W, b, b2, me, mask, base, n, C, D, 0, tok, (float2 *)nullptr, 0);
    else hipLaunchKernelGGL((k_embed<128, MODE, 1>), grid, blk, 0, st, out, in, W, b, b2, me, mask, base, n, C, D, 0, tok, (float2 *)nullptr, 0);
    return 0;
}

template <int BF, int BT, int NWF, int NWT, int BK, int NS, bool PERSIST, class Epi>
void launch_gemm_glds(const GemmArgs &g, const Epi &epi, hipStream_t st) {
    auto kern = k_gemm_glds<BF, BT, NWF, NWT, BK, NS, PERSIST, Epi>;
    const size_t lds = GemmCfg<BF, BT, NWF, NWT, BK, NS, PERSIST, Epi>::lds_bytes + (Epi::lds_bias ? (size_t)((g.F + BF - 1) / BF) * BF * 4 : 0);
    LSL_ALLOW_LDS(kern, LDS_BUDGET);
    const int tiles = ((g.N + BT - 1) / BT) * ((g.F + BF - 1) / BF);
    int grid = tiles;
    if (PERSIST) {
        const int per_cu = (int)std::max<size_t>(1, LDS_BUDGET / lds);
        grid = device_cus() * per_cu;
        grid -= grid % 8;
        if (grid > tiles) grid = tiles;
    }
    hipLaunchKernelGGL(kern, dim3(grid), dim3(NWF * NWT * 64), lds, st, g, epi);
}

}

#ifdef LSL_EXPERIMENTS
#include "host_launch_experiments.hip.h"
#endif

namespace {

template <class Fn>
bool with_linear1_ts_instance(int hdp, int D, Fn &&fn) {
#define X(H, K) if (hdp == H && D == K) return fn(ic<H>{}, ic<K>{}), true;
    LSL_LIN1_TS_INSTANCES(X)
#undef X
    return false;
}
template <int HDP, int K, int NW = 8, bool LNF = false>
void launch_linear1_ts_t(const Lin1Args &a, hipStream_t st) {
    using C = Lin1Cfg<HDP, K, NW>;
    const int ntile = (a.N + C::TT - 1) / C::TT, nb = a.F / 32;
    const long units = (long)ntile * nb;
    int grid = (int)std::min<long>(device_cus(), units / 2);
    Lin1Args b = a;
    static const int align = tune_int("LSL_LIN1_ALIGN", 1);
    const int wpt = std::min(device_cus() / ntile, nb / 2);
    b.wpt = align && wpt >= 2 ? wpt : 0;
    if (b.wpt) grid = b.wpt * ntile;
    lsl_lin1_launch(HDP, K, NW, LNF, b, grid, LNF ? C::lds_bytes_lnf(a.F) : C::lds_bytes(a.F), st);
}
int linear1_ts_waves(int D, int N) {
    static const int nw4_max = tune_int("LSL_LIN1_NW4_MAX", 10240);
    return D == 512 && N <= nw4_max ? 4 : 8;
}
bool linear1_ts_ok(int hdp, int D, int F1, int HHD, int N) {
    static const int on = tune_int("LSL_LIN1_TS", 1);
    if (!on || F1 % 64 != 0 || HHD % 64 != 0 || N < 1) return false;
    size_t lds = 0;
    return with_linear1_ts_instance(hdp, D, [&](auto h, auto k) { lds = Lin1Cfg<decltype(h)::value, decltype(k)::value, 8>::lds_bytes(F1); }) && lds <= LDS_BUDGET;
}
int ln_fuse_env() {
    static const int v = env_int("LSL_LN_FUSE", -1);
    return v;
}
bool linear1_lnf_ok(int hdp, int D, int F1, int HHD, int N, int tpt, int mod_stride) {
    if (ln_fuse_env() == 0 || !linear1_ts_ok(hdp, D, F1, HHD, N)) return false;
    size_t lds = 0;
    int min_tpt = 0;
    with_linear1_ts_instance(hdp, D, [&](auto h, auto k) {
        using C = Lin1Cfg<decltype(h)::value, decltype(k)::value, 8>;
        lds = C::lds_bytes_lnf(F1);
        min_tpt = C::LN_SLOTS >= 3 ? C::TT / 2 : C::TT;
    });
    return (mod_stride == 0 || tpt >= min_tpt) && lds <= LDS_BUDGET;
}
void launch_linear1_ts(int hdp, int D, int waves, bool lnf, const Lin1Args &a, hipStream_t st) {
    with_linear1_ts_instance(hdp, D, [&](auto h, auto k) {
        constexpr int H = decltype(h)::value, K = decltype(k)::value;
        if (lnf) return launch_linear1_ts_t<H, K, 8, true>(a, st);
        if constexpr (K == 512) {
            if (waves == 4) return launch_linear1_ts_t<H, K, 4>(a, st);
        }
        launch_linear1_ts_t<H, K, 8>(a, st);
    });
}

#define LSL_LIN2_WS_INSTANCES(X) X(1536, 3, 3) X(1280, 4, 4) X(768, 3, 3) X(384, 3, 3)
template <class Fn>
bool with_linear2_ws_instance(int K2, Fn &&fn) {
#define X(K, NCH, NS) if (K2 == K) return fn(ic<K>{}, ic<NCH>{}, ic<NS>{}), true;
    LSL_LIN2_WS_INSTANCES(X)
#undef X
    return false;
}
bool linear2_ws_shape_ok(int D, int K2) {
    static const int on = env_int("LSL_LIN2_WS", 1);
    return on && D % 128 == 0 && D <= 512 && with_linear2_ws_instance(K2, [](auto, auto, auto) {});
}
struct Lin2Grid {
    int slices, rpx, gate_rows;
};
Lin2Grid linear2_ws_grid(int F, int N, int tpt, bool shared) {
    const int slices = F / 128, cus = device_cus(), NBLK = (N + 31) / 32;
    int rpx = std::max(1, cus / (8 * slices));
    while (rpx > 1 && 8 * rpx > NBLK) --rpx;
    const int ranges = 8 * rpx, max_blocks = (NBLK + ranges - 1) / ranges + 1;
    return {slices, rpx, shared ? 1 : (max_blocks * 32 + tpt - 1) / tpt + 1};
}
int linear2_ws_max_gate_rows(int K2) {
    int rows = 0;
    with_linear2_ws_instance(K2, [&](auto k, auto nch, auto ns) { rows = Lin2Cfg<decltype(k)::value, decltype(nch)::value, decltype(ns)::value, true>::max_gate_rows; });
    return rows;
}
template <int K, int NCH, int NS, bool LNS>
void launch_linear2_ws_t(const Lin2Args &a, hipStream_t st) {
    using C = Lin2Cfg<K, NCH, NS, true>;
    auto kern = k_linear2_ws<K, NCH, NS, true, LNS>;
    LSL_ALLOW_LDS(kern, LDS_BUDGET);
    hipLaunchKernelGGL(kern, dim3(8 * a.slices * a.rpx), dim3(512), C::lds_bytes(a.gate_rows), st, a);
}
void launch_linear2_ws(int K2, const Lin2Args &a, hipStream_t st) {
    with_linear2_ws_instance(K2, [&](auto k, auto nch, auto ns) {
        constexpr int K = decltype(k)::value, NCH = decltype(nch)::value, NS = decltype(ns)::value;
        if (a.stats) launch_linear2_ws_t<K, NCH, NS, true>(a, st);
        else launch_linear2_ws_t<K, NCH, NS, false>(a, st);
    });
}

int tail_env() {
    static const int v = env_int("LSL_TAIL", -1);
    return v;
}
bool tail_shape_ok(int D, int HHD, int M) {
    return tail_env() != 0 && D == 256 && HHD == 256 && M % 64 == 0 && M >= 64 && TailCfg<256, 256>::lds_bytes(M) <= LDS_BUDGET;
}
size_t tail_stream_bytes(const lsl_model *m) { return TailCfg<256, 256>::stream_bytes(m->d.mlp_dim); }
void launch_tail(const TailArgs &a, hipStream_t st) {
    using C = TailCfg<256, 256>;
    auto kern = k_tail<256, 256>;
    LSL_ALLOW_LDS(kern, LDS_BUDGET);
    const int nwt = (a.N + 31) / 32;
    hipLaunchKernelGGL(kern, dim3(std::min(nwt, device_cus())), dim3(512), C::lds_bytes(a.M), st, a);
}

int gemm_variant(bool lin2, int F, int K, int N) {
    static const int forced_all = tune_int("LSL_GEMM", -1);
    static const int forced_1 = tune_int("LSL_GEMM1", -1), forced_2 = tune_int("LSL_GEMM2", -1);
    const int forced_one = lin2 ? forced_2 : forced_1;
    const int forced = forced_one >= 0 ? forced_one : forced_all;
    const bool ragged = F % 256 != 0 && (F % 256 <= 128);
    const int ragged_variant = lin2 && K % 64 == 0 ? 11 : 10;
    if (forced >= 0) return forced;
    if (lin2 && F % 192 == 0 && F % 256 != 0 && K % 64 == 0 && (long)((N + 127) / 128) * (F / 192) * 2 >= (long)device_cus())
        return 28;
    if (ragged) return ragged_variant;
    static const int small_rule = tune_int("LSL_SMALL_TILES", 1);
    const long tiles256 = (long)((N + 255) / 256) * ((F + 255) / 256);
    const int cus = device_cus();
    if (small_rule && K % 64 == 0 && tiles256 * (lin2 ? 2 : 4) <= (long)cus * (lin2 ? 1 : 5))
        return 11;
    return lin2 ? (K % 128 == 0 ? 7 : 15) : (K % 128 == 0 ? 12 : 5);
}

template <class Epi>
void launch_gemm(int variant, const u16 *W, const u16 *X, int F, int N, int K, const Epi &epi_in, hipStream_t st, int hhd = 32) {
    constexpr bool lin2 = std::is_same<Epi, EpiLinear2>::value;
    static const int probe = tune_int("LSL_PROBE", 0);
    static const int stagger = tune_int("LSL_STAGGER", 0);
    GemmArgs g{W, X, F, N, K, stagger, probe};
    static const int nt = tune_int("LSL_NT", 3);
    Epi epi = epi_in;
    epi.probe = probe | ((nt >> (lin2 ? 1 : 0)) & 1 ? 32 : 0);
    const bool pp_ok = lin2 || hhd % 32 == 0;
    if (launch_gemm_experiment(variant, g, epi, st, pp_ok)) return;
    if (variant == 12 && K % 128 == 0) return launch_gemm_glds<256, 256, 2, 4, 64, 2, true>(g, epi, st);
    if constexpr (lsl_experiments || lin2) {
        if (variant == 7 && F % 32 == 0 && pp_ok && K % 128 == 0) return launch_gemm_glds<256, 256, 2, 4, 64, 2, true>(g, EpiPieces<Epi>(epi), st);
    }
    switch (variant) {
        case 5: return launch_gemm_glds<256, 256, 2, 4, 64, 2, false>(g, epi, st);
        case 10: return launch_gemm_glds<128, 128, 2, 2, 32, 3, false>(g, epi, st);
        case 11: return launch_gemm_glds<128, 128, 2, 2, 64, 2, false>(g, epi, st);
        case 28:
            if constexpr (lin2) return launch_gemm_glds<192, 128, 2, 4, 64, 3, false>(g, epi, st);
            else break;
        case 15: return launch_gemm_glds<256, 256, 4, 4, 64, 2, false>(g, epi, st);
        default: return launch_gemm_glds<256, 256, 2, 4, 64, 2, false>(g, epi, st);
    }
}


int attention_stream_mode(int S, int H) {
    static const int on = env_int("LSL_ATTN_STREAM", 1);
    if (!on) return 0;
    static const int long_min = tune_int("LSL_ATTN_LONG_MIN", 129);
    if (S >= long_min) return 2;
    if (S > 8 && S <= 32 && H % 8 == 0) return 1;
    return 0;
}

enum class AttnForm {
    linear,
    stream_short,
    stream_grouped,
    stream_long,
    stream_chunked,
    stream_chunked_den,
    tiny,
    rows,
    none
};
struct AttnPlan {
    AttnForm form;
    int stream_mode;
    int S, n_seq, inner, outer_stride, pos_stride, blk, n_tok;
    int nw, items, nkt;
    bool stream() const { return form >= AttnForm::stream_short && form <= AttnForm::stream_chunked_den; }
};
bool attention_grouped_ok(const AttnPlan &a, int H) {
    static const int on = env_int("LSL_ATTN_GROUP", 1), stream_on = env_int("LSL_ATTN_STREAM", 1);
    return on && stream_on && a.S >= 2 && a.S <= 8 && (a.S & (a.S - 1)) == 0 && a.inner == 1 && a.pos_stride == 1 && a.outer_stride == a.S && H % 8 == 0;
}
constexpr size_t attention_stream_lds(int hdp) { return (size_t)2 * 2 * 256 * hdp * 2 + (size_t)8 * 32 * hdp * 2; }
constexpr size_t attention_rows_lds(int hdp, int nw, int items, int key_rows) { return (size_t)items * 2 * key_rows * hdp * 2 + nw * sizeof(float); }
constexpr int attention_rows_max_s(int hdp) { return (int)((LDS_BUDGET - 16 * sizeof(float)) / (4 * hdp)) & ~31; }
static_assert(attention_rows_lds(32, 16, 1, attention_rows_max_s(32)) <= LDS_BUDGET && attention_rows_lds(32, 16, 1, attention_rows_max_s(32) + 32) > LDS_BUDGET);

AttnPlan plan_attention(bool linear, int hdp, int H, int hd, int bc, int T, int L, bool temporal) {
    AttnPlan p{};
    if (!temporal) {
        p.S = L; p.n_seq = bc * T; p.inner = 1; p.outer_stride = L; p.pos_stride = 1;
    } else {
        p.S = T; p.n_seq = bc * L; p.inner = L; p.outer_stride = T * L; p.pos_stride = L;
    }
    p.form = AttnForm::linear;
    if (linear) return p;
    const AttnPlan axis = p;
// ... 113 lines not shown
```

### lam_slide_amd/csrc/k_lin1.hip.h

```cpp
#pragma once
#include "k_mm_frag.hip.h"

struct Lin1Args {
    const u16 *W;
    const u16 *X;
    const float *bias;
    const float4 *rope_q, *rope_k;
    u16 *qkv;
    u16 *z;
    int F, N, HHD, M;
    int pos_div, pos_mod;
    unsigned div_magic, mod_magic;
    float inv_hd, q_premul;
    int nt;
    int wpt;
    int planes;
    int npad;
    const float2 *ln_stat;
    const float *ln_shift, *ln_scale;
    int ln_mod_stride, ln_tpt;
    unsigned ln_tpt_magic;
};

#ifndef LIN1_B2
#define LIN1_B2 1
#endif
#ifndef LIN1_B2_KMAX
#define LIN1_B2_KMAX 256
#endif

template <int HDP, int K, int NW = 8>
struct Lin1Cfg {
    static_assert(K % 128 == 0 && K <= 512, "hidden sizes 128 / 256 / 384 / 512");
    static constexpr int KS = K / 16;
    static constexpr int ROWB = 2 * K;
    static constexpr int PITCH = ROWB + 16;
    static constexpr int BLK = 32 * PITCH;
    static constexpr int NS = (LIN1_B2 && K <= LIN1_B2_KMAX) ? 4 : 3;
    static constexpr int RING = NS * BLK;
    static_assert(NW == 8 || NW == 4, "two waves per SIMD (256-token tiles) or one (128-token tiles)");
    static constexpr int TT = 32 * NW;
    static constexpr int STAGE = NW * 4096;
    static constexpr int LPR = ROWB / 16;
    static constexpr int PPW = 32 / NW;
    static constexpr size_t lds_bytes(int F) { return (size_t)RING + STAGE + (size_t)F * 4; }
    static constexpr int LN_SLOTS = K <= 256 ? 3 : 2;
    static constexpr size_t lds_bytes_lnf(int F) { return lds_bytes(F) + (size_t)LN_SLOTS * 2 * K * 4; }
};

#define LSL_LIN1_TS_INSTANCES(X) X(32, 128) X(32, 256) X(32, 384) X(32, 512) X(16, 128) X(16, 256) X(16, 384) X(16, 512)

bool lsl_lin1_launch(int hdp, int K, int waves, bool lnf, const Lin1Args &a, int grid, size_t lds, hipStream_t st);

#ifndef LSL_LIN1_HOST_SIDE

enum { LIN1_QK = 0, LIN1_V = 1, LIN1_MLP = 2 };

#ifndef LIN1_XLOAD
#define LIN1_XLOAD 1
#endif
#ifndef LIN1_PD
#define LIN1_PD 3
#endif

__device__ __forceinline__ float lin1_gelu(float x) {
    const float ax = fabsf(x);
    const float h = __builtin_amdgcn_exp2f(LSL_GELU_Q(ax));
    float relu;
    asm("v_max_f32 %0, 0, %1" : "=v"(relu) : "v"(x));
    return fmaf(-ax, h, relu);
}

template <int HDP, int K, int NW = 8, bool LNF = false>
__global__ void __launch_bounds__(NW * 64, NW / 4) k_linear1_ts(Lin1Args g) {
    using C = Lin1Cfg<HDP, K, NW>;
    constexpr int KS = C::KS, BLK = C::BLK, PPW = C::PPW, ROWB = C::ROWB;
    constexpr int NCO = HDP == 32 ? 8 : 4;
    extern __shared__ __attribute__((aligned(16))) char smem[];

    const int tid = threadIdx.x, lane = tid & 63;
    const int wave = __builtin_amdgcn_readfirstlane(tid >> 6);
    const int r = lane & 31, hf = lane >> 5;
    char *const stage = smem + C::RING + wave * 4096;
    float *const bias_lds = reinterpret_cast<float *>(smem + C::RING + C::STAGE);

    const int NB = g.F >> 5;
    const int ntile = (g.N + C::TT - 1) / C::TT;
    const long U = (long)ntile * NB;
    long i0, i1;
    if (g.wpt > 0) {
        const int tile = blockIdx.x / g.wpt, part = blockIdx.x - tile * g.wpt;
        i0 = (long)tile * NB + ((NB * part / g.wpt) & ~1);
        i1 = (long)tile * NB + (part + 1 == g.wpt ? NB : ((NB * (part + 1) / g.wpt) & ~1));
    } else {
        i0 = (U * blockIdx.x / gridDim.x) & ~1L;
        i1 = blockIdx.x + 1 == gridDim.x ? U : ((U * (blockIdx.x + 1) / gridDim.x) & ~1L);
    }
    if (i0 >= i1) return;

    for (int i = tid * 4; i < g.F; i += NW * 64 * 4) *reinterpret_cast<float4 *>(bias_lds + i) = *reinterpret_cast<const float4 *>(g.bias + i);

    const unsigned lds0 = (unsigned)(size_t)(LDS_PTR(char))(smem);
    const unsigned lane_src = lane * 16;
    const char *const w_rows = reinterpret_cast<const char *>(g.W) + (size_t)(PPW * wave) * ROWB;
    auto issue_piece = [&](const char *src, unsigned dst, auto ic) __attribute__((always_inline)) {
        constexpr int I = decltype(ic)::value & 3;
        if (decltype(ic)::value >= 4) {
            src += 4 * ROWB;
            dst += 4 * C::PITCH;
        }
        const unsigned ls = lane_src;
        if (C::LPR == 64 || lane < C::LPR) {
            if (I == 0 || decltype(ic)::value >= 4)
                asm volatile("s_add_u32 m0, %2, %3\n\ts_nop 4\n\tglobal_load_lds_dwordx4 %0, %1 offset:%4" ::"v"(ls), "s"(src), "s"(dst), "n"(16 * I), "n"(ROWB * I) : "memory", "scc");
            else
                asm volatile("s_add_u32 m0, %2, %3\n\ts_nop 0\n\tglobal_load_lds_dwordx4 %0, %1 offset:%4" ::"v"(ls), "s"(src), "s"(dst), "n"(16 * I), "n"(ROWB * I) : "memory", "scc");
        }
    };
    auto req_src = [&](int blk) __attribute__((always_inline)) { return w_rows + (size_t)blk * (32 * ROWB); };
    auto req_dst = [&](int slot) __attribute__((always_inline)) { return lds0 + slot * BLK + PPW * wave * C::PITCH; };
    auto issue = [&](int blk, int slot) __attribute__((always_inline)) {
        const char *src = req_src(blk);
        const unsigned dst = req_dst(slot);
        static_for<PPW>([&](auto pc) __attribute__((always_inline)) { issue_piece(src, dst, pc); });
    };
    const int aoff = r * C::PITCH + 16 * hf;

    bf16x8 xreg[KS];
    float4 co[NCO];
    f32x16 acc0, acc1;
    int slot_c = 0;
    int dma_blk, dma_slot;
    int n_wave = 0;
    float post = 1.0f;

    auto advance = [&](int &b) __attribute__((always_inline)) { b = b + 1 == NB ? 0 : b + 1; };
    auto next_slot = [&](int s) __attribute__((always_inline)) { return s == C::NS - 1 ? 0 : s + 1; };

    {
        int b = (int)(i0 - (i0 / NB) * NB);
        issue(b, 0);
        advance(b);
        issue(b, 1);
        advance(b);
        dma_blk = b;
        dma_slot = 2;
    }

    auto init_acc = [&](f32x16 &a, int blk) __attribute__((always_inline)) {
#pragma unroll
        for (int q4 = 0; q4 < 4; ++q4) {
            const float4 b = *reinterpret_cast<const float4 *>(bias_lds + blk * 32 + 8 * q4 + 4 * hf);
            a[4 * q4] = b.x; a[4 * q4 + 1] = b.y; a[4 * q4 + 2] = b.z; a[4 * q4 + 3] = b.w;
        }
    };
    constexpr bool B2 = LIN1_B2 != 0 && K <= LIN1_B2_KMAX;
    auto step_head = [&](auto flushed_c) __attribute__((always_inline)) {
        if (B2) {
            if (decltype(flushed_c)::value) wait_vmcnt<PPW>();
            else wait_vmcnt<0>();
        } else {
            if (decltype(flushed_c)::value) wait_vmcnt<PPW + 4>();
            else wait_vmcnt<PPW>();
        }
        __builtin_amdgcn_s_barrier();
        asm volatile("" ::: "memory");
    };
    const unsigned wr0 = (unsigned)(size_t)(LDS_PTR(char))(stage) + r * 128 + 8 * hf + ((r & 7) << 4);
    const unsigned rd0 = (unsigned)(size_t)(LDS_PTR(char))(stage) + (lane >> 3) * 128 + (((lane & 7) ^ ((lane >> 3) & 7)) << 4);
    const char *row_q = nullptr, *row_z = nullptr;
    const bool planes = g.planes != 0;
    constexpr unsigned PROW = 2u * HDP, CPH = HDP / 8;
    const unsigned plane_bytes = PROW * (unsigned)g.npad;
    const unsigned stride_q = planes ? PROW : 2u * 3 * g.HHD, stride_z = 2u * (g.HHD + g.M);
    const unsigned blk_q = planes ? (32 / HDP) * plane_bytes : 64u;
    const unsigned voff_q = planes ? ((lane & 7) / CPH) * plane_bytes + (lane >> 3) * PROW + 16 * ((lane & 7) % CPH) : (lane >> 3) * stride_q + 16 * (lane & 7);
    const unsigned voff_z = (lane >> 3) * stride_z + 16 * (lane & 7);
    const int slab_z = 3 * (g.HHD >> 5);
    const char *fl_base = nullptr;
    unsigned fl_stride8 = 0, fl_voff = 0;
    auto flush_setup = [&](int b_even) __attribute__((always_inline)) {
        const bool to_qkv = b_even < slab_z;
        fl_base = to_qkv ? row_q : row_z;
        fl_stride8 = 8 * (to_qkv ? stride_q : stride_z);
        fl_voff = to_qkv ? voff_q + blk_q * (unsigned)b_even : voff_z + 64u * (unsigned)b_even;
    };
    auto flush_read = [&](int half, u32x4 (&pk)[2]) __attribute__((always_inline)) {
#pragma unroll
        for (int i = 0; i < 2; ++i) pk[i] = *reinterpret_cast<const LDS_PTR(u32x4)>(rd0 + 1024 * (2 * half + i));
    };
    auto flush_store = [&](int half, const u32x4 (&pk)[2]) __attribute__((always_inline)) {
        stream_store16<true>(fl_voff + (2 * half) * fl_stride8, pk[0], fl_base);
        stream_store16<false>(fl_voff + (2 * half + 1) * fl_stride8, pk[1], fl_base);
    };
    auto flush_store_visible = [&](int half, const u32x4 (&pk)[2]) __attribute__((always_inline)) {
#pragma unroll
        for (int i = 0; i < 2; ++i)
            __builtin_nontemporal_store(pk[i], reinterpret_cast<u32x4 *>(const_cast<char *>(fl_base) + (size_t)(fl_voff + (2 * half + i) * fl_stride8)));
    };
    auto put_group = [&](int ii, int q, float v0, float v1, float v2, float v3) __attribute__((always_inline)) {
        const u32x2 pk = {pack2(v0, v1), pack2(v2, v3)};
        *reinterpret_cast<LDS_PTR(u32x2)>(wr0 ^ (unsigned)(64 * ii + 16 * q)) = pk;
    };
    auto epi_slice = [&](auto sec_c, int s, const f32x16 &a, int ii, float &c0, float &c1) __attribute__((always_inline)) {
        constexpr int SEC = decltype(sec_c)::value;
        if constexpr (SEC == LIN1_QK && HDP == 32) {
            if (s == 0) c0 = 0.0f;
            if (s < 2) {
#pragma unroll
                for (int e = 0; e < 8; ++e) c0 = fmaf(a[8 * s + e], a[8 * s + e], c0);
            }
            if (s == 1) c0 = qk_factor(c0, g.inv_hd, post);
            if (s >= 2 && s < 6) {
                const int q = s - 2;
                float o[4];
#pragma unroll
                for (int kk = 0; kk < 2; ++kk) rope_pair(c0, co[2 * q + kk], a[2 * (2 * q + kk)], a[2 * (2 * q + kk) + 1], o[2 * kk], o[2 * kk + 1]);
                put_group(ii, q, o[0], o[1], o[2], o[3]);
            }
        } else if constexpr (SEC == LIN1_QK) {
            if (s == 0) {
                c0 = 0.0f;
#pragma unroll
                for (int e = 0; e < 8; ++e) c0 = fmaf(a[e], a[e], c0);
            }
            if (s == 1) {
                c1 = 0.0f;
#pragma unroll
                for (int e = 0; e < 8; ++e) c1 = fmaf(a[8 + e], a[8 + e], c1);
                c0 = qk_factor(c0, g.inv_hd, post);
                c1 = qk_factor(c1, g.inv_hd, post);
            }
            if (s >= 2 && s < 6) {
                const int q = s - 2;
                const float rr = q < 2 ? c0 : c1;
                float o[4];
#pragma unroll
                for (int kk = 0; kk < 2; ++kk) rope_pair(rr, co[(2 * q + kk) & (NCO - 1)], a[2 * (2 * q + kk)], a[2 * (2 * q + kk) + 1], o[2 * kk], o[2 * kk + 1]);
                put_group(ii, q, o[0], o[1], o[2], o[3]);
            }
        } else if constexpr (SEC == LIN1_MLP) {
            const float g0 = lin1_gelu(a[2 * s]), g1 = lin1_gelu(a[2 * s + 1]);
            if (s & 1) put_group(ii, s >> 1, c0, c1, g0, g1);
            else { c0 = g0; c1 = g1; }
        } else {
            if (s < 4) put_group(ii, s, a[4 * s], a[4 * s + 1], a[4 * s + 2], a[4 * s + 3]);
        }
    };
    auto step = [&](auto sec_c, auto par_c, auto mfma_c, auto epi_c, auto side) __attribute__((always_inline)) {
        constexpr int PAR = decltype(par_c)::value;
        constexpr bool DO_MFMA = decltype(mfma_c)::value != 0, DO_EPI = decltype(epi_c)::value != 0;
        constexpr int MPS = KS / 8, PD = LIN1_PD, MH = (MPS + 1) / 2;
        f32x16 &ac = PAR ? acc0 : acc1;
        const f32x16 &ae = PAR ? acc1 : acc0;
        const char *sb = smem + slot_c * BLK + aoff;
        bf16x8 fr[PD];
        float c0 = 0.0f, c1 = 0.0f;
        if (DO_MFMA) {
#pragma unroll
            for (int ks = 0; ks < PD; ++ks) fr[ks] = as_bf16x8(*reinterpret_cast<const u32x4 *>(sb + 32 * ks));
        }
        side(ic<-1>());
        auto side_of = [&](int s) __attribute__((always_inline)) {
            static_for<8>([&](auto sc) __attribute__((always_inline)) { if (s == decltype(sc)::value) side(sc); });
        };
#pragma unroll
        for (int s = 0; s < 8; ++s) {
#pragma unroll
            for (int m = 0; m < MPS; ++m) {
                if (m == MH) side_of(s);
                if (DO_MFMA) {
                    const int ks = s * MPS + m;
                    ac = mfma32(fr[ks % PD], xreg[ks], ac);
                    if (ks + PD < KS) fr[ks % PD] = as_bf16x8(*reinterpret_cast<const u32x4 *>(sb + 32 * (ks + PD)));
                }
            }
            if (MH == MPS) side_of(s);
            if (DO_EPI) epi_slice(sec_c, s, ae, PAR, c0, c1);
            __builtin_amdgcn_sched_barrier(0);
        }
        if (decltype(mfma_c)::value != 0) slot_c = next_slot(slot_c);
    };
    ic<0> I0;
    ic<1> I1;
    auto no_side = [](auto) __attribute__((always_inline)) {};
    auto fused = [&](auto sec_c, auto par_c, auto flush_c, auto prev_c, int e) __attribute__((always_inline)) {
        constexpr int PAR = decltype(par_c)::value;
        constexpr bool FLUSH = decltype(flush_c)::value != 0;
        if (!B2 || PAR == 1) step_head(prev_c);
        u32x4 pk[2];
        if (FLUSH) flush_setup(e - 2);
        const char *src = req_src(dma_blk);
        const unsigned dst = req_dst(dma_slot);
        int blk2 = dma_blk;
        advance(blk2);
        const char *src2 = req_src(blk2);
        const unsigned dst2 = req_dst(next_slot(dma_slot));
        init_acc(PAR ? acc0 : acc1, e + 1);
        step(sec_c, par_c, I1, I1, [&](auto sl) __attribute__((always_inline)) {
            constexpr int SL = decltype(sl)::value;
            if (FLUSH) {
                if (SL == -1) flush_read(0, pk);
                if (SL == 0) {
                    flush_store(0, pk);
                    flush_read(1, pk);
                }
                if (SL == 1) flush_store(1, pk);
            }
            constexpr int PS = PPW / 4;
            if (!B2) {
                if (SL >= 2 && SL < 6) {
                    issue_piece(src, dst, ic<(SL >= 2 && SL < 6) ? PS * (SL - 2) : 0>());
                    if (PS == 2) issue_piece(src, dst, ic<(SL >= 2 && SL < 6) ? PS * (SL - 2) + 1 : 0>());
                }
            } else if (PAR == 1) {
                if (SL >= 0 && SL < 4) {
                    issue_piece(src, dst, ic<(SL >= 0 && SL < 4) ? PS * SL : 0>());
                    if (PS == 2) issue_piece(src, dst, ic<(SL >= 0 && SL < 4) ? PS * SL + 1 : 0>());
                }
                if (SL >= 4 && SL < 8) {
                    issue_piece(src2, dst2, ic<(SL >= 4 && SL < 8) ? PS * (SL - 4) : 0>());
                    if (PS == 2) issue_piece(src2, dst2, ic<(SL >= 4 && SL < 8) ? PS * (SL - 4) + 1 : 0>());
                }
            }
        });
        if (!B2) {
            advance(dma_blk);
            dma_slot = next_slot(dma_slot);
        } else if (PAR == 1) {
            advance(dma_blk);
            advance(dma_blk);
            dma_slot = next_slot(next_slot(dma_slot));
        }
    };
    auto run = [&](auto sec_c, int ea, int eb) __attribute__((always_inline)) {
        int e = ea;
        if (e < eb && (e & 1)) {
            fused(sec_c, I1, I0, I0, e);
            ++e;
        }
        for (; e + 1 < eb; e += 2) {
            fused(sec_c, I0, I1, I0, e);
            fused(sec_c, I1, I0, I1, e + 1);
        }
        if (e < eb) fused(sec_c, I0, I1, I0, e);
    };
    auto load_co = [&](const float4 *tab, unsigned pos) __attribute__((always_inline)) { rope_rows<HDP>(co, tab, pos, hf); };
    auto co_arrived = [&]() __attribute__((always_inline)) {
#pragma unroll
        for (int k = 0; k < NCO; ++k) asm volatile("" ::"v"(co[k].w));
    };
    ic<LIN1_QK> SQK;
    ic<LIN1_V> SV;
    ic<LIN1_MLP> SMLP;

    constexpr bool XLINES = LIN1_XLOAD != 0 && (K <= 384 || LIN1_XLOAD >= 2);
    auto load_x = [&](int nw) __attribute__((always_inline)) {
        if (!XLINES) {
            const u16 *xr = g.X + (size_t)(nw + r) * K + 8 * hf;
#pragma unroll
            for (int ks = 0; ks < KS; ++ks) xreg[ks] = as_bf16x8(*reinterpret_cast<const u32x4 *>(xr + 16 * ks));
        } else {
            load_lines<KS>(xreg, g.X, nw, K, lane);
        }
    };
    auto finish_x = [&]() __attribute__((always_inline)) {
        if (!XLINES) return;
        const unsigned t0 = lane >> 3;
        const unsigned xw = (unsigned)(size_t)(LDS_PTR(char))(stage) + t0 * 128;
        const unsigned xr0 = (unsigned)(size_t)(LDS_PTR(char))(stage) + r * 128;
#pragma unroll
        for (int j = 0; j < KS / 4; ++j) {
#pragma unroll
            for (int q = 0; q < 4; ++q)
                *reinterpret_cast<LDS_PTR(u32x4)>(xw + 1024 * q + ((((lane & 7) ^ ((t0 >> 1) + 4 * q)) & 7) << 4)) = as_u32x4(xreg[4 * j + q]);
#pragma unroll
            for (int m = 0; m < 4; ++m)
                xreg[4 * j + m] = as_bf16x8(*reinterpret_cast<const LDS_PTR(u32x4)>(xr0 + ((((2 * m + hf) ^ (r >> 1)) & 7) << 4)));
        }
    };

    float *const ln_tab = bias_lds + ((g.F + 3) & ~3);
    auto traj_of = [&](unsigned n) __attribute__((always_inline)) { return magic_div(n, g.ln_tpt_magic); };
    auto load_x_lnf = [&](int tile_, int nw) __attribute__((always_inline)) {
        typedef __attribute__((ext_vector_type(4))) float f4;
        const float *xf = reinterpret_cast<const float *>(g.X);
        const unsigned t_first = g.ln_mod_stride ? traj_of((unsigned)(tile_ * C::TT)) : 0u;
        const unsigned t_last = g.ln_mod_stride ? traj_of((unsigned)(g.N - 1)) : 0u;
        for (int i = tid * 4; i < C::LN_SLOTS * K; i += NW * 64 * 4) {
            const int slot = i / K, col = i - slot * K;
            const size_t mo = (size_t)min(t_first + (unsigned)slot, t_last) * g.ln_mod_stride + col;
            const f4 sc = *reinterpret_cast<const f4 *>(g.ln_scale + mo), sh = *reinterpret_cast<const f4 *>(g.ln_shift + mo);
            *reinterpret_cast<f4 *>(ln_tab + (size_t)slot * 2 * K + col) = f4{1.0f + sc[0], 1.0f + sc[1], 1.0f + sc[2], 1.0f + sc[3]};
            *reinterpret_cast<f4 *>(ln_tab + (size_t)slot * 2 * K + K + col) = sh;
        }
        const unsigned l = (unsigned)opaque_lane(lane), rowi = l >> 3, chunk = l & 7, rl = l & 31, hl = l >> 5;
        const unsigned sbase = (unsigned)(size_t)(LDS_PTR(char))(stage);
        const unsigned xr0 = sbase + rl * 128;
        const unsigned tab0 = (unsigned)(size_t)(LDS_PTR(char))(ln_tab) + 16 * chunk;
        const float *xr = xf + (size_t)(nw + rowi) * K + 4 * chunk;
        float2 st[4];
        unsigned tb[4];
#pragma unroll
        for (int q = 0; q < 4; ++q) {
            const unsigned nn = (unsigned)min(nw + (int)rowi + 8 * q, g.N - 1);
            st[q] = g.ln_stat[nn];
            const unsigned slot = g.ln_mod_stride ? min(traj_of(nn) - t_first, (unsigned)(C::LN_SLOTS - 1)) : 0u;
            tb[q] = tab0 + slot * (2 * K * 4);
        }
        __syncthreads();
#pragma unroll
        for (int p = 0; p < K / 64; ++p) {
            f4 v[2][4];
#pragma unroll
            for (int e = 0; e < 2; ++e)
#pragma unroll
                for (int q = 0; q < 4; ++q) v[e][q] = *reinterpret_cast<const f4 *>(xr + (size_t)(8 * q) * K + 64 * p + 32 * e);
#pragma unroll
            for (int q = 0; q < 4; ++q) {
                const unsigned row = rowi + 8 * q, sw = (row >> 1) & 7;
#pragma unroll
                for (int e = 0; e < 2; ++e) {
                    const f4 sc = *reinterpret_cast<const LDS_PTR(f4)>(tb[q] + 4 * (64 * p + 32 * e)), sh = *reinterpret_cast<const LDS_PTR(f4)>(tb[q] + 4 * (K + 64 * p + 32 * e));
                    f4 x = v[e][q];
#pragma unroll
                    for (int c = 0; c < 4; ++c) x[c] = fmaf(x[c], st[q].x, st[q].y) * sc[c] + sh[c];
                    const u32x2 pk = {pack2(x[0], x[1]), pack2(x[2], x[3])};
                    *reinterpret_cast<LDS_PTR(u32x2)>(sbase + row * 128 + ((((4 * e + (chunk >> 1)) ^ sw) & 7) << 4) + 8 * (chunk & 1)) = pk;
                }
            }
#pragma unroll
            for (int m = 0; m < 4; ++m)
                xreg[4 * p + m] = as_bf16x8(*reinterpret_cast<const LDS_PTR(u32x4)>(xr0 + ((((2 * m + hl) ^ (rl >> 1)) & 7) << 4)));
            __builtin_amdgcn_sched_barrier(0);
        }
    };
    const int qb = g.HHD >> 5;
    int tile = (int)(i0 / NB), b0 = (int)(i0 - (long)tile * NB), left = (int)(i1 - i0);
    bool first_seg = true;
    bool co_ready = false;
    __syncthreads();
    while (left > 0) {
        const int b1 = NB - b0 < left ? NB : b0 + left;
        n_wave = tile * C::TT + wave * 32;
        row_q = reinterpret_cast<const char *>(g.qkv) + (size_t)n_wave * stride_q;
        row_z = reinterpret_cast<const char *>(g.z) + (size_t)n_wave * stride_z - 4 * (size_t)g.HHD;
        if constexpr (LNF) load_x_lnf(tile, n_wave);
        else {
            if (first_seg) load_x(n_wave);
            finish_x();
        }
        const unsigned nn = (unsigned)min(n_wave + r, g.N - 1);
        const unsigned pos = token_pos(nn, g.div_magic, g.mod_magic, g.pos_mod);

        if (first_seg) wait_vmcnt<0>();
        else wait_vmcnt<4>();
        __builtin_amdgcn_s_barrier();
        asm volatile("" ::: "memory");
        issue(dma_blk, dma_slot);
        advance(dma_blk);
        dma_slot = next_slot(dma_slot);
        if (B2) {
            issue(dma_blk, dma_slot);
            advance(dma_blk);
            dma_slot = next_slot(dma_slot);
        }
        init_acc(acc0, b0);
        step(SV, I1, I1, I0, no_side);
        const int e_end = b1 - 1;
        if (b0 < 2 * qb) {
            if (!co_ready) load_co(b0 < qb ? g.rope_q : g.rope_k, pos);
            post = b0 < qb ? g.q_premul : 1.0f;
            fused(SQK, I0, I0, I0, b0);
        } else if (b0 < 3 * qb) {
            fused(SV, I0, I0, I0, b0);
        } else {
            fused(SMLP, I0, I0, I0, b0);
        }
        {
            const int lo = max(b0 + 1, 0), hi = min(e_end, qb);
            if (lo < hi) run(SQK, lo, hi);
        }
        {
            const int lo = max(b0 + 1, qb), hi = min(e_end, 2 * qb);
            if (lo < hi) {
                if (lo == qb) {
                    load_co(g.rope_k, pos);
                    post = 1.0f;
                    co_arrived();
                }
                run(SQK, lo, hi);
            }
        }
        {
            const int lo = max(b0 + 1, 2 * qb), hi = min(e_end, 3 * qb);
            if (lo < hi) run(SV, lo, hi);
        }
        {
            const int lo = max(b0 + 1, 3 * qb), hi = min(e_end, NB);
            if (lo < hi) run(SMLP, lo, hi);
        }
        const int left_next = left - (b1 - b0);
        co_ready = false;
        if (left_next > 0) {
            asm volatile("" ::: "memory");
            const int nw = (tile + 1) * C::TT + wave * 32;
            if constexpr (!LNF) load_x(nw);
            if (b1 - 1 >= 2 * qb) {
                const unsigned nn2 = (unsigned)min(nw + r, g.N - 1);
                load_co(g.rope_q, token_pos(nn2, g.div_magic, g.mod_magic, g.pos_mod));
                co_ready = true;
            }
            asm volatile("" ::: "memory");
        }
        {
            const int e = b1 - 1;
            if (e < 2 * qb) {
                step(SQK, I1, I0, I1, no_side);
            } else if (e < 3 * qb) {
                step(SV, I1, I0, I1, no_side);
            } else {
                step(SMLP, I1, I0, I1, no_side);
            }
            flush_setup(e - 1);
            u32x4 pk[2];
            flush_read(0, pk);
            flush_store_visible(0, pk);
            flush_read(1, pk);
            flush_store_visible(1, pk);
        }
        left = left_next;
        tile += 1;
        b0 = 0;
        first_seg = false;
    }
    wait_vmcnt<0>();
}

#endif
```

### lam_slide_amd/csrc/lsl_api.hip

```cpp
#include "../../include/lsl_api.h"

#include <hip/hip_runtime.h>

#include <algorithm>
#include <cmath>
#include <cstdarg>
#include <cstdio>
#include <cstdlib>
#include <cstring>
#include <initializer_list>
#include <string>
#include <vector>

#include "k_attn.hip.h"
#include "k_gemm.hip.h"
#define LSL_LIN1_HOST_SIDE
#include "k_lin1.hip.h"
#include "k_lin2.hip.h"
#include "k_tail.hip.h"
#include "k_small.hip.h"
#include "k_dopri5.hip.h"
#include "k_resident.hip.h"
#include "k_jvp.hip.h"
#ifdef LSL_EXPERIMENTS
#include "k_gemm_pp.hip.h"
#include "k_gemm_drain.hip.h"
#include "k_head_scalar.hip.h"
#endif

#include "host_eval.hip.h"
#include "host_jvp.hip.h"
#include "host_dopri.hip.h"

LSL_UNIT_INFO;

namespace {
thread_local char g_err[512] = "";
std::string &unit_info() {
    static std::string lines;
    return lines;
}
}

int fail(int code, const char *fmt, ...) {
    va_list ap;
    va_start(ap, fmt);
    vsnprintf(g_err, sizeof(g_err), fmt, ap);
    va_end(ap);
    return code;
}

void lsl_add_unit_info(const char *line) { unit_info().append("; ").append(line); }

LSL_HIDDEN void lsl_si_mix_launch(float *x, const float *x1, const float *x0, const lsl_si_row *rows, uint64_t per, uint64_t total, int cus, hipStream_t st);
LSL_HIDDEN int lsl_si_reduce_launch(const float *pred, const float *x1, const float *x0, const lsl_si_row *rows, int B, uint64_t per, float *loss,
                                    float *partial, hipStream_t st);

extern "C" {

int lsl_version(void) { return LSL_VERSION; }
const char *lsl_build_info(void) {
    static const std::string info = "clang " __clang_version__ " gfx950" + unit_info();
    return info.c_str();
}
const char *lsl_last_error(void) { return g_err; }

int lsl_model_create(const lsl_model_desc *desc, lsl_model **out) try {
    if (!desc || !out) return fail(-1, "null argument");
    const lsl_model_desc &d = *desc;
    if (d.heads <= 0 || d.hidden % d.heads != 0)
        return fail(-20, "Hidden size %d must be divisible by num_heads %d", d.hidden, d.heads);
    if (d.head_dim != d.hidden / d.heads) return fail(-21, "head_dim must equal hidden / heads");
    if (d.hidden % 64 != 0 || d.hidden < 64 || d.hidden > 512) return fail(-21, "hidden_size %d unsupported (multiple of 64, 64..512)", d.hidden);
    if (d.head_dim % 2 != 0 || d.head_dim > 32) return fail(-21, "head_dim %d unsupported (even, <= 32)", d.head_dim);
    if (d.head_dim_pad != (d.head_dim <= 16 ? 16 : 32)) return fail(-21, "head_dim_pad must be 16 (head_dim <= 16) or 32");
    if ((d.heads * d.head_dim_pad) % 32 != 0) return fail(-21, "heads * head_dim_pad must be a multiple of 32");
    if (d.mlp_dim <= 0 || d.mlp_dim % 32 != 0) return fail(-21, "mlp_dim %d must be a positive multiple of 32", d.mlp_dim);
    if ((d.heads * d.head_dim_pad + d.mlp_dim) % 64 != 0) return fail(-21, "heads*head_dim_pad + mlp_dim must be a multiple of 64");
    if (3 * d.heads * d.head_dim_pad + d.mlp_dim > 7936) return fail(-21, "3 * heads * head_dim_pad + mlp_dim = %d too wide (the linear1 bias lives in LDS beside a 128 KiB operand ring: <= 7936)", 3 * d.heads * d.head_dim_pad + d.mlp_dim);
    if (d.in_dim <= 0 || d.in_dim > 128) return fail(-21, "in_dim %d unsupported (1..128)", d.in_dim);
    if (d.depth <= 0 || d.depth > 64) return fail(-21, "depth %d unsupported", d.depth);
    if (d.vec_in_dim < 0 || d.vec_in_dim > 512) return fail(-21, "vec_in_dim %d unsupported (<= 512)", d.vec_in_dim);
    lsl_model *m = new (std::nothrow) lsl_model();
    if (!m) return fail(-5, "out of host memory");
    m->d = d;
    m->HHD = d.heads * d.head_dim_pad;
    m->F1 = 3 * m->HHD + d.mlp_dim;
    m->K2 = m->HHD + d.mlp_dim;
    m->MODW = (6 * d.depth + 2) * d.hidden;
    m->tail = tail_env() == 1 && tail_shape_ok(d.hidden, m->HHD, d.mlp_dim);
    m->ln_fuse = ln_fuse_env() == 1;
    *out = m;
    return 0;
} LSL_API_CATCH

int lsl_model_set_weights(lsl_model *m, const lsl_weights *w) try {
    if (!m || !w || !w->blocks) return fail(-1, "null argument");
    const void *req[] = {w->x_in_w, w->x_in_b, w->cond_w, w->cond_b, w->mask_emb, w->time_freqs, w->time_w1, w->time_b1,
                         w->time_w2, w->time_b2, w->mod_w, w->mod_b, w->out_w, w->out_b};
    for (const void *p : req)
        if (!p) return fail(-2, "missing weight pointer");
    if (m->d.vec_in_dim > 0 && (!w->vec_w1 || !w->vec_b1 || !w->vec_w2 || !w->vec_b2)) return fail(-2, "missing vec_in weights");
    m->blocks.assign(w->blocks, w->blocks + 2 * m->d.depth);
    for (const auto &b : m->blocks)
        if (!b.w1 || !b.b1 || !b.qs || !b.ks || !b.w2 || !b.b2) return fail(-2, "missing block weight pointer");
    m->w = *w;
    m->w.blocks = m->blocks.data();
    m->has_weights = true;
    m->graphs.clear();
    return 0;
} LSL_API_CATCH

void lsl_model_destroy(lsl_model *m) {
    if (m) m->prof.clear();
    delete m;
}

int lsl_profile_enable(lsl_model *m, int32_t kernel, int32_t max_launches) try {
    if (!m) return fail(-1, "null model");
    m->prof.clear();
    if (kernel < 0 || max_launches <= 0) return 0;
    m->prof.ev.resize(2 * (size_t)max_launches);
    for (auto &e : m->prof.ev)
        if (hipEventCreate(&e) != hipSuccess) return fail(-10, "hipEventCreate failed");
    m->prof.kernel = kernel;
    m->prof.cap = max_launches;
    return 0;
} LSL_API_CATCH

int lsl_profile_read(lsl_model *m, double *total_ms, int32_t *launches) {
    if (!m || !total_ms || !launches) return fail(-1, "null argument");
    double tot = 0.0;
    for (int i = 0; i < m->prof.used; ++i) {
        hipEventSynchronize(m->prof.ev[2 * i + 1]);
        float ms = 0.0f;
        if (hipEventElapsedTime(&ms, m->prof.ev[2 * i], m->prof.ev[2 * i + 1]) != hipSuccess) return fail(-10, "hipEventElapsedTime failed");
        tot += ms;
    }
    *total_ms = tot;
    *launches = m->prof.used;
    m->prof.used = 0;
    return 0;
}

int lsl_model_set_chunk(lsl_model *m, int32_t c) try {
    if (!m || c < 0) return fail(-1, "bad argument");
    m->chunk = c;
    m->graphs.clear();
    return 0;
} LSL_API_CATCH

int lsl_model_set_attention_mode(lsl_model *m, int32_t mode) try {
    if (!m || (mode != 0 && mode != 1)) return fail(-1, "attention mode must be 0 (scaled_dot_product) or 1 (linear)");
    m->attention_linear = mode == 1;
    m->graphs.clear();
    return 0;
} LSL_API_CATCH

int lsl_model_set_tail(lsl_model *m, int32_t on) try {
    if (!m || (on != 0 && on != 1)) return fail(-1, "tail must be 0 or 1");
    if (on && !tail_shape_ok(m->d.hidden, m->HHD, m->d.mlp_dim))
        return fail(-21, "no tail kernel for this model (hidden 256 with heads * head_dim_pad = 256, mlp_dim a multiple of 64; LSL_TAIL=0 disables it)");
    if (m->tail != (on == 1)) m->graphs.clear();
    m->tail = on == 1;
    return 0;
} LSL_API_CATCH
int32_t lsl_model_tail(const lsl_model *m) { return m && m->tail ? 1 : 0; }
int lsl_model_set_ln_fuse(lsl_model *m, int32_t on) try {
    if (!m || (on != 0 && on != 1)) return fail(-1, "ln_fuse must be 0 or 1");
// ... 188 lines not shown
    CallPlans plans;
    if (int rc = plan_call(m, ws, io, chunk, io->y ? m->MODW : 0, plans)) return rc;
    run_tables(m, ws, io->T, io->L, st);
    const size_t per = (size_t)io->T * io->L * m->d.in_dim;
    const size_t total = per * io->B;
    static const int group_on = env_int("LSL_MODS_GROUP", 1);
    const int G = (group_on && !io->y) ? (group_on >= 2 ? std::min(group_on, ws.mods_group) : ws.mods_group) : 0;
    std::vector<int> net_idx;
    std::vector<float> net_t;
    if (G) {
        net_idx.resize((size_t)n_steps);
        for (int s = 0; s < n_steps; ++s) {
            net_idx[s] = (int)net_t.size();
            if (!(steps[s].flags & LSL_STEP_NO_NETWORK)) net_t.push_back(steps[s].t);
        }
    }
    int cur_group = -1;
    return for_each_pass(m, ws, io, chunk, st, [&](const Pass &ps) -> int {
        for (int s = 0; s < n_steps; ++s) {
            const lsl_step_ex &sp = steps[s];
            EvalArgs e;
            e.x = io->x + ps.elem;
            e.have_y = io->y != nullptr;
            e.rec = &sp;
            if (sp.aw != 0.0f && noise) e.noise = noise + (size_t)sp.noise_index * total + ps.elem;
            e.seed = seed;
            e.elem_off = elem_offset + ps.elem;
            e.trace = trace && sp.trace_index >= 0 ? trace + (size_t)sp.trace_index * total + ps.elem : nullptr;
            e.saved = sp.as != 0.0f ? ws.saved : nullptr;
            e.save_out = (sp.flags & LSL_STEP_SAVE) ? ws.saved : nullptr;
            if (sp.flags & LSL_STEP_NO_NETWORK) {
                launch_state_affine(e.x, (unsigned long long)ps.bc * per, step_update(e), st);
                LSL_CHECK_LAUNCH("state update");
                continue;
            }
            if (G) {
                const int k = net_idx[s], g = k / G;
                if (cur_group != g) {
                    if (int rc = run_mods_steps(m, ws, net_t.data() + (size_t)g * G, std::min(G, (int)net_t.size() - g * G), st)) return rc;
                    cur_group = g;
                }
                e.mods_ready = ws.mods_all + (size_t)(k - g * G) * m->MODW;
            }
            if (int rc = run_eval(m, ws, plans.of(ps.bc), e, st)) return rc;
        }
        return 0;
    });
}

int lsl_randn(float *x, uint64_t n, uint64_t seed, uint64_t elem_offset, void *stream) try {
    DeviceGuard dev_guard_((hipStream_t)stream);
    if (!x && n) return fail(-1, "null argument");
    if (!n) return 0;
    const unsigned long long blocks = (n + 255) / 256;
    const unsigned grid = (unsigned)std::min<unsigned long long>(blocks, (unsigned long long)device_cus() * 16);
    hipLaunchKernelGGL(k_randn, dim3(grid), dim3(256), 0, (hipStream_t)stream, x, (unsigned long long)n, (unsigned long long)seed, LSL_INIT_STEP,
                       (unsigned long long)elem_offset);
    LSL_CHECK_LAUNCH("lsl_randn");
    return 0;
} LSL_API_CATCH

int lsl_rk_lincomb(float *out, const float *const *x, const float *c, int32_t n_x, uint64_t n, void *stream) try {
    DeviceGuard dev_guard_((hipStream_t)stream);
    if (!out && n) return fail(-1, "null argument");
    RkTerms t;
    if (int rc = rk_terms(t, x, c, n_x)) return rc;
    if (!n) return 0;
    hipLaunchKernelGGL(k_rk_lincomb, dim3(rk_grid(n)), dim3(256), 0, (hipStream_t)stream, out, t, (unsigned long long)n);
    LSL_CHECK_LAUNCH("lsl_rk_lincomb");
    return 0;
} LSL_API_CATCH

int lsl_rk_dense(float *out, const float *a, const float *b, const float *c, const float *d, const float *e, float x, uint64_t n, void *stream) try {
    DeviceGuard dev_guard_((hipStream_t)stream);
    if (n && (!out || !a || !b || !c || !d || !e)) return fail(-1, "null argument");
    if (!n) return 0;
    hipLaunchKernelGGL(k_rk_poly4, dim3(rk_grid(n)), dim3(256), 0, (hipStream_t)stream, out, a, b, c, d, e, x, (unsigned long long)n);
    LSL_CHECK_LAUNCH("lsl_rk_dense");
    return 0;
} LSL_API_CATCH

int lsl_rk_error_ratio(float *ratio, const float *y0, const float *y1, const float *const *k, const float *c, int32_t n_k, float atol, float rtol,
                       uint64_t n, void *scratch, void *stream) try {
    DeviceGuard dev_guard_((hipStream_t)stream);
    if (!ratio || !y0 || !y1 || !scratch) return fail(-1, "null argument");
    if (!n) return fail(-3, "empty state");
    RkTerms t;
    if (int rc = rk_terms(t, k, c, n_k)) return rc;
    const unsigned grid = rk_error_blocks(n);
    static_assert(LSL_RK_SCRATCH_BYTES / 4 == 2048, "rk_error_blocks: one partial sum per workgroup");
    hipLaunchKernelGGL(k_rk_error_partial, dim3(grid), dim3(256), 0, (hipStream_t)stream, (float *)scratch, y0, y1, t, atol, rtol, (unsigned long long)n);
    hipLaunchKernelGGL(k_rk_error_final, dim3(1), dim3(256), 0, (hipStream_t)stream, ratio, (const float *)scratch, (int)grid, (unsigned long long)n);
    LSL_CHECK_LAUNCH("lsl_rk_error_ratio");
    return 0;
} LSL_API_CATCH

size_t lsl_dopri_workspace_bytes(const lsl_model *m, int32_t B, int32_t T, int32_t L, int32_t n_out) {
    if (!m || B <= 0 || T <= 0 || L <= 0 || n_out <= 0) return 0;
    return dopri_carve(m, nullptr, B, T, L, n_out).bytes;
}
size_t lsl_dopri_each_workspace_bytes(const lsl_model *m, int32_t B, int32_t T, int32_t L, int32_t n_out, int32_t log_rows) {
    if (!m || B <= 0 || B > DOPRI_EACH_MAX_B || T <= 0 || L <= 0 || n_out <= 0 || log_rows < 0 || log_rows > LSL_DOPRI_MAX_ATTEMPTS) return 0;
    return dopri_carve(m, nullptr, B, T, L, n_out, true, log_rows).bytes;
}

int lsl_dopri_begin(lsl_model *m, const lsl_io *io, const lsl_dopri_desc *desc, const double *grid, int32_t n_out, float *out, void *workspace,
                    size_t workspace_bytes, void *stream) try {
    return dopri_begin(m, io, desc, grid, n_out, out, false, LSL_DOPRI_MAX_ATTEMPTS, workspace, workspace_bytes, stream);
} LSL_API_CATCH

int lsl_dopri_each_begin(lsl_model *m, const lsl_io *io, const lsl_dopri_desc *desc, const double *grid, int32_t n_out, float *out, int32_t log_rows,
                         void *workspace, size_t workspace_bytes, void *stream) try {
    return dopri_begin(m, io, desc, grid, n_out, out, true, log_rows, workspace, workspace_bytes, stream);
} LSL_API_CATCH

int lsl_dopri_advance(lsl_model *m, const lsl_io *io, int32_t n_attempts, void *workspace, size_t workspace_bytes, void *stream) try {
    return dopri_advance(m, io, n_attempts, false, 1, LSL_DOPRI_MAX_ATTEMPTS, workspace, workspace_bytes, stream);
} LSL_API_CATCH

int lsl_dopri_each_advance(lsl_model *m, const lsl_io *io, int32_t n_attempts, void *workspace, size_t workspace_bytes, void *stream) try {
    if (!m || !io) return fail(-1, "null model or io");
    const auto call = m->dopri_each.find(workspace);
    if (call == m->dopri_each.end() || call->second.B != io->B || call->second.T != io->T || call->second.L != io->L)
        return fail(-3, "no lsl_dopri_each_begin on this handle laid this workspace out for B, T, L = %d, %d, %d", io->B, io->T, io->L);
    return dopri_advance(m, io, n_attempts, true, call->second.n_out, call->second.log_rows, workspace, workspace_bytes, stream);
} LSL_API_CATCH

int lsl_debug_dopri_coeffs(int32_t path_type, int32_t model_type, const float *t, int32_t n, double *out, void *stream) try {
    DeviceGuard dev_guard_((hipStream_t)stream);
    if (!t || !out || n <= 0) return fail(-3, "invalid arguments");
    if (path_type < LSL_PATH_LINEAR || path_type > LSL_PATH_VP || model_type < LSL_PRED_VELOCITY || model_type > LSL_PRED_SCORE) return fail(-3, "unknown path or model type");
    hipLaunchKernelGGL(k_dp_coeffs, dim3((unsigned)((n + 255) / 256)), dim3(256), 0, (hipStream_t)stream, (int)path_type, (int)model_type, t, (int)n, out);
    LSL_CHECK_LAUNCH("lsl_debug_dopri_coeffs");
    return 0;
} LSL_API_CATCH

int lsl_debug_block_ex(lsl_model *m, int32_t bi, const float *h_in, float *h_out, void *a_out, const float *mods, int32_t mod_rows, int32_t B,
                       int32_t T, int32_t L, void *workspace, size_t workspace_bytes, void *stream) try {
    DeviceGuard dev_guard_((hipStream_t)stream);
    const bool args_ok = mod_rows == 1 || mod_rows == B;
    if (int rc = check_debug(m, bi, args_ok, B, T, L, workspace, workspace_bytes)) return rc;
    hipStream_t st = (hipStream_t)stream;
    const Workspace ws = carve(m, (char *)workspace, B, T, L);
    PassPlan plan;
    if (int rc = plan_pass(m, ws, B, T, L, mod_rows == 1 ? 0 : m->MODW, PlanMode::debug_block, bi, plan)) return rc;
    run_tables(m, ws, T, L, st);
    const size_t bytes = (size_t)B * T * L * m->d.hidden * 4;
    hipMemcpyAsync(ws.h, h_in, bytes, hipMemcpyDeviceToDevice, st);
    if (int rc = run_block(m, ws, plan, bi, mods, st, a_out)) return rc;
    hipMemcpyAsync(h_out, ws.h, bytes, hipMemcpyDeviceToDevice, st);
    return 0;
} LSL_API_CATCH

int lsl_debug_block(lsl_model *m, int32_t bi, const float *h_in, float *h_out, const float *mods, int32_t B, int32_t T, int32_t L,
                    void *workspace, size_t workspace_bytes, void *stream) {
    return lsl_debug_block_ex(m, bi, h_in, h_out, nullptr, mods, B, B, T, L, workspace, workspace_bytes, stream);
}

int lsl_debug_taps(lsl_model *m, int32_t bi, const float *h_in, const float *mods, int32_t B, int32_t T, int32_t L, void *qkv_out,
                   void *z_out, void *workspace, size_t workspace_bytes, void *stream) try {
    DeviceGuard dev_guard_((hipStream_t)stream);
    const bool args_ok = h_in && mods && qkv_out && z_out && B > 0 && T > 0 && L > 0;
    if (int rc = check_debug(m, bi, args_ok, B, T, L, workspace, workspace_bytes)) return rc;
    hipStream_t st = (hipStream_t)stream;
    const Workspace ws = carve(m, (char *)workspace, B, T, L);
    PassPlan plan;
    if (int rc = plan_pass(m, ws, B, T, L, m->MODW, PlanMode::debug_taps, bi, plan)) return rc;
    run_tables(m, ws, T, L, st);
    const size_t n = (size_t)B * T * L;
    hipMemcpyAsync(ws.h, h_in, n * m->d.hidden * 4, hipMemcpyDeviceToDevice, st);
    if (int rc = run_block(m, ws, plan, bi, mods, st)) return rc;
    if (plan.planes[bi & 1]) {
        const long chunks = (long)n * 3 * m->d.heads * (m->d.head_dim_pad / 8);
        hipLaunchKernelGGL(k_planes_to_rows, dim3((unsigned)((chunks + 255) / 256)), dim3(256), 0, st, (u16 *)qkv_out, ws.qkv, (int)n,
                           (int)((n + 255) & ~(size_t)255), 3 * m->d.heads, m->d.head_dim_pad);
    } else
        hipMemcpyAsync(qkv_out, ws.qkv, n * 3 * m->HHD * 2, hipMemcpyDeviceToDevice, st);
    hipMemcpyAsync(z_out, ws.z, n * m->K2 * 2, hipMemcpyDeviceToDevice, st);
    LSL_CHECK_LAUNCH("debug taps");
    return 0;
} LSL_API_CATCH

int lsl_debug_mods_ex(lsl_model *m, const float *t, float t_scalar, const float *y, int32_t B, float *vec_out, float *mods_out, float *tfeat_out,
                      float *hid_out, float *yhid_out, float *yemb_out, void *workspace, size_t workspace_bytes, void *stream) try {
    DeviceGuard dev_guard_((hipStream_t)stream);
    const bool args_ok = m && B > 0 && vec_out && mods_out && (t || !y) && (!y || m->d.vec_in_dim > 0) && ((!yhid_out && !yemb_out) || y);
    if (int rc = check_debug(m, 0, args_ok, B, 1, 1, workspace, workspace_bytes)) return rc;
    hipStream_t st = (hipStream_t)stream;
    const Workspace ws = carve(m, (char *)workspace, B, 1, 1);
    const size_t D = m->d.hidden;
    char ylabel[sizeof(m->prof.name)] = "";
    if (y) {
        if (int rc = run_yemb(m, ws, y, B, st, yhid_out)) return rc;
        if (yemb_out) hipMemcpyAsync(yemb_out, ws.yemb, (size_t)B * D * 4, hipMemcpyDeviceToDevice, st);
        if (m->prof.kernel == 6) snprintf(ylabel, sizeof(ylabel), "%s", m->prof.name);
    }
    if (int rc = run_mods(m, ws, t, t_scalar, y ? ws.yemb : nullptr, B, vec_out, mods_out, st)) return rc;
    if (tfeat_out) hipMemcpyAsync(tfeat_out, ws.tfeat, (size_t)B * 256 * 4, hipMemcpyDeviceToDevice, st);
    if (hid_out) hipMemcpyAsync(hid_out, ws.hid, (size_t)B * D * 4, hipMemcpyDeviceToDevice, st);
    if (ylabel[0]) {
        char both[sizeof(m->prof.name)];
        snprintf(both, sizeof(both), "%s ; %s", ylabel, m->prof.name);
        m->prof.label(6, "%s", both);
    }
    LSL_CHECK_LAUNCH("debug mods");
    return 0;
} LSL_API_CATCH

int lsl_debug_mods(lsl_model *m, const float *t, const float *y, int32_t B, float *vec_out, float *mods_out, void *workspace,
                   size_t workspace_bytes, void *stream) {
    return lsl_debug_mods_ex(m, t, 0.0f, y, B, vec_out, mods_out, nullptr, nullptr, nullptr, nullptr, workspace, workspace_bytes, stream);
}

int lsl_debug_mods_steps(lsl_model *m, const float *times, int32_t count, float *mods_out, float *vec_out, void *workspace, size_t workspace_bytes,
                         void *stream) try {
    DeviceGuard dev_guard_((hipStream_t)stream);
    if (int rc = check_debug(m, 0, m && times && count > 0 && mods_out, 1, 1, 1, workspace, workspace_bytes)) return rc;
    hipStream_t st = (hipStream_t)stream;
    const Workspace ws = carve(m, (char *)workspace, 1, 1, 1);
    if (count > ws.mods_group) return fail(-3, "%d records: a group of this model holds %d (0: class-conditioned, tables per evaluation)", count, ws.mods_group);
    if (int rc = run_mods_steps(m, ws, times, count, st)) return rc;
    hipMemcpyAsync(mods_out, ws.mods_all, (size_t)count * m->MODW * 4, hipMemcpyDeviceToDevice, st);
    if (vec_out) hipMemcpyAsync(vec_out, ws.vec_all, (size_t)count * m->d.hidden * 4, hipMemcpyDeviceToDevice, st);
    LSL_CHECK_LAUNCH("debug mods (group of records)");
    return 0;
} LSL_API_CATCH

int lsl_debug_embed(lsl_model *m, const float *x, const float *x_cond, const int64_t *mask, int32_t B, int32_t T, int32_t L, float *cond_emb_out,
                    float *h_out, float *hn_out, void *stats_out, void *workspace, size_t workspace_bytes, void *stream) try {
    DeviceGuard dev_guard_((hipStream_t)stream);
    if (int rc = check_debug(m, 0, x && x_cond && mask && B > 0 && T > 0 && L > 0, B, T, L, workspace, workspace_bytes)) return rc;
    hipStream_t st = (hipStream_t)stream;
    const Workspace ws = carve(m, (char *)workspace, B, T, L);
    PassPlan plan;
    if (int rc = plan_pass(m, ws, B, T, L, 0, PlanMode::eval, 0, plan)) return rc;
    if (stats_out && !plan.emb_stats) return fail(-3, "stats_out: this handle's embedding leaves no row statistics (ln_fuse, no normalize, in_dim <= 32, hidden 256 / 512)");
    const size_t n = (size_t)plan.n, D = m->d.hidden;
    if (int rc = prepare_pass(m, ws, x_cond, mask, nullptr, B, T, L, st)) return rc;
    char clabel[sizeof(m->prof.name)];
    snprintf(clabel, sizeof(clabel), "%s", m->prof.name);
    if (cond_emb_out) hipMemcpyAsync(cond_emb_out, ws.cond_emb, n * D * 4, hipMemcpyDeviceToDevice, st);
    if (int rc = run_embed(m, ws, plan, x, st, h_out)) return rc;
    if (hn_out) hipMemcpyAsync(hn_out, ws.h, n * D * 4, hipMemcpyDeviceToDevice, st);
    if (stats_out) hipMemcpyAsync(stats_out, ws.lnstat, n * sizeof(float2), hipMemcpyDeviceToDevice, st);
    if (m->prof.kernel == 5) {
        char both[sizeof(m->prof.name)];
        snprintf(both, sizeof(both), "%s ; %s", clabel, m->prof.name);
        m->prof.label(5, "%s", both);
    }
    LSL_CHECK_LAUNCH("debug embed");
    return 0;
} LSL_API_CATCH

int lsl_debug_head(lsl_model *m, const float *h, const float *mods, int32_t mod_rows, float *x, float *out, const lsl_step_ex *rec, const float *noise,
                   uint64_t seed, uint64_t elem_offset, float *trace, const float *saved, float *save_out, int32_t B, int32_t T, int32_t L,
                   void *stream) try {
    DeviceGuard dev_guard_((hipStream_t)stream);
    if (!m || !m->has_weights) return fail(-2, "weights not set");
    const bool shape_ok = B > 0 && T > 0 && L > 0 && (unsigned long long)B * T * L * (unsigned)std::max(m->d.in_dim, m->d.hidden) < (1ull << 31);
    if (!shape_ok || !h || !mods || (mod_rows != 1 && mod_rows != B) || (rec ? !x : !out)) return fail(-3, "invalid arguments");
    if (rec && ((rec->flags & LSL_STEP_NO_NETWORK) || (rec->aw != 0.0f && rec->noise_index < 0) || (rec->as != 0.0f && !saved)))
        return fail(-3, "invalid record");
    EvalArgs e;
    e.x = x;
    e.out = out;
    e.rec = rec;
    if (rec) {
        e.noise = rec->aw != 0.0f ? noise : nullptr;
        e.seed = seed;
        e.elem_off = elem_offset;
        e.trace = trace;
        e.saved = rec->as != 0.0f ? saved : nullptr;
        e.save_out = save_out;
    }
    const float *fm = mods + (size_t)m->d.depth * 6 * m->d.hidden;
    return run_head(m, h, fm, mod_rows == 1 ? 0 : m->MODW, B * T * L, T * L, e, (hipStream_t)stream);
} LSL_API_CATCH

}
```

Before: 58.88 trajectories/s.

## Fuse temporal attention into the linear1 kernel for short temporal sequences

Adds a k_lin1_tfuse variant of the linear1 kernel. For temporal blocks (T<=32, hidden 512, 32-wide heads) it computes per-head Q/K/V tiles, applies RoPE from LDS tables, runs softmax attention with MFMA in registers, and writes the attention output straight to z. This removes the separate attention launch and the round trip of qkv through global memory. In exchange it reorders weight blocks per head, adds LDS for the rotation tables, and uses a max-bound shortcut for the softmax shift. It is enabled by default through LSL_LIN1_TFUSE when the shape gate passes.

Result: faster. 60.65 trajectories/s (median of 6 runs) (+3.0%).

```diff
diff --git a/include/lsl_api.h b/include/lsl_api.h
--- a/include/lsl_api.h
+++ b/include/lsl_api.h
@@ -242,6 +242,10 @@
                     void *workspace, size_t workspace_bytes, void *stream);
 int lsl_debug_block_ex(lsl_model *m, int32_t block_index, const float *h_in, float *h_out, void *a_out, const float *mods, int32_t mod_rows,
                        int32_t B, int32_t T, int32_t L, void *workspace, size_t workspace_bytes, void *stream);
+int lsl_debug_block_z(lsl_model *m, int32_t block_index, const float *h_in, float *h_out, void *z_out, const float *mods, int32_t mod_rows,
+                      int32_t B, int32_t T, int32_t L, void *workspace, size_t workspace_bytes, void *stream);
+int lsl_debug_tfuse_gate(int32_t enabled, int32_t eval_mode, int32_t lin1_ts, int32_t tail, int32_t attn_short, int32_t head_dim_pad, int32_t hidden,
+                         int32_t F1, int32_t T, int32_t L, int32_t z_width);
 int lsl_debug_taps(lsl_model *m, int32_t block_index, const float *h_in, const float *mods, int32_t B, int32_t T, int32_t L,
                    void *qkv_out, void *z_out, void *workspace, size_t workspace_bytes, void *stream);
 int lsl_debug_mods(lsl_model *m, const float *t, const float *y, int32_t B, float *vec_out, float *mods_out,
diff --git a/lam_slide_amd/_lib.py b/lam_slide_amd/_lib.py
--- a/lam_slide_amd/_lib.py
+++ b/lam_slide_amd/_lib.py
@@ -32,7 +32,7 @@
 
 EXPORTED = (
     "lsl_version", "lsl_build_info", "lsl_last_error", "lsl_model_create", "lsl_model_set_weights", "lsl_model_destroy",
-    "lsl_model_set_chunk", "lsl_model_set_attention_mode", "lsl_model_set_tail", "lsl_model_tail", "lsl_model_set_ln_fuse", "lsl_model_ln_fuse", "lsl_profile_kernel_name", "lsl_pass_size", "lsl_sampler_path", "lsl_workspace_bytes", "lsl_forward", "lsl_sample", "lsl_sample_ex", "lsl_debug_block", "lsl_debug_block_ex", "lsl_debug_taps", "lsl_debug_mods",
+    "lsl_model_set_chunk", "lsl_model_set_attention_mode", "lsl_model_set_tail", "lsl_model_tail", "lsl_model_set_ln_fuse", "lsl_model_ln_fuse", "lsl_profile_kernel_name", "lsl_pass_size", "lsl_sampler_path", "lsl_workspace_bytes", "lsl_forward", "lsl_sample", "lsl_sample_ex", "lsl_debug_block", "lsl_debug_block_ex", "lsl_debug_block_z", "lsl_debug_tfuse_gate", "lsl_debug_taps", "lsl_debug_mods",
     "lsl_debug_mods_ex", "lsl_debug_mods_steps", "lsl_debug_embed", "lsl_debug_head",
     "lsl_si_loss_workspace_bytes", "lsl_si_loss", "lsl_si_reduce", "lsl_geom_loss_sums", "lsl_geom_loss_final",
     "lsl_peptide_loss_sums", "lsl_peptide_loss_final", "lsl_disp_error_rows", "lsl_disp_error_final",
@@ -236,6 +236,8 @@
                                     C.c_void_p, C.c_size_t, C.c_void_p]
     lib.lsl_debug_block_ex.argtypes = [C.c_void_p, C.c_int32, C.c_void_p, C.c_void_p, C.c_void_p, C.c_void_p, C.c_int32, C.c_int32, C.c_int32,
                                        C.c_int32, C.c_void_p, C.c_size_t, C.c_void_p]
+    lib.lsl_debug_block_z.argtypes = lib.lsl_debug_block_ex.argtypes
+    lib.lsl_debug_tfuse_gate.argtypes = [C.c_int32] * 11
     lib.lsl_debug_taps.argtypes = [C.c_void_p, C.c_int32, C.c_void_p, C.c_void_p, C.c_int32, C.c_int32, C.c_int32, C.c_void_p, C.c_void_p,
                                    C.c_void_p, C.c_size_t, C.c_void_p]
     lib.lsl_debug_mods.argtypes = [C.c_void_p, C.c_void_p, C.c_void_p, C.c_int32, C.c_void_p, C.c_void_p, C.c_void_p, C.c_size_t,
diff --git a/lam_slide_amd/csrc/host_eval.hip.h b/lam_slide_amd/csrc/host_eval.hip.h
--- a/lam_slide_amd/csrc/host_eval.hip.h
+++ b/lam_slide_amd/csrc/host_eval.hip.h
@@ -102,6 +102,7 @@
     int gemm1;
     bool planes[2];
     AttnPlan attn[2];
+    bool tfuse;
     Lin2Kind lin2;
     Lin2Grid l2grid;
     int gemm2;
@@ -111,7 +112,7 @@
     bool lin2_stats(int bi) const { return ln_stats && bi + 1 < blocks; }
 };
 
-int plan_pass(const lsl_model *m, const Workspace &ws, int bc, int T, int L, int mod_stride, PlanMode mode, int block, PassPlan &p) {
+int plan_pass(const lsl_model *m, const Workspace &ws, int bc, int T, int L, int mod_stride, PlanMode mode, int block, PassPlan &p, bool z_tap = false) {
     const lsl_model_desc &d = m->d;
     const int D = d.hidden, n = bc * T * L;
     p = PassPlan{};
@@ -135,6 +136,7 @@
         p.attn[t] = plan_attention(m->attention_linear, d.head_dim_pad, d.heads, d.head_dim, bc, T, L, t != 0);
         p.planes[t] = qkv_planes_ok(d.head_dim_pad, d.heads, t ? T : L, t != 0, p.lin1_ts, p.attn[t]);
     }
+    p.tfuse = linear1_tf_ok(mode == PlanMode::eval || (z_tap && mode == PlanMode::debug_block), p.lin1_ts, p.tail, p.attn[1].form == AttnForm::stream_short, d.head_dim_pad, D, p.F1, T, L, m->K2);
     const bool ws_reach = ws.w2p && (unsigned long long)n * (unsigned)(4 * D) < (1ull << 32);
     if (ws_reach) p.l2grid = linear2_ws_grid(D, n, T * L, mod_stride == 0);
     const bool on_ws = ws_reach && p.l2grid.gate_rows <= linear2_ws_max_gate_rows(m->K2);
@@ -171,12 +173,13 @@
     return 0;
 }
 
-void label_block(lsl_model *m, const PassPlan &p, int bi) {
+void label_block(lsl_model *m, const PassPlan &p, int bi, bool tfuse) {
     const lsl_model_desc &d = m->d;
     Profiler &pr = m->prof;
     switch (pr.kernel) {
         case 0:
             if (!p.lin1_ts) pr.label(0, "k_gemm_glds<EpiLinear1<%d>> (tiling %d)", d.head_dim_pad, p.gemm1);
+            else if (tfuse) pr.label(0, "k_lin1_tfuse<%s> (temporal attention inside%s)", p.lin1_lnf(bi) ? "true" : "false", p.lin1_lnf(bi) ? ", LayerNorm fused" : "");
             else if (p.lin1_lnf(bi)) pr.label(0, "k_linear1_ts<%d, %d, 8, true> (LayerNorm fused)", d.head_dim_pad, d.hidden);
             else pr.label(0, "k_linear1_ts<%d, %d, %d>%s", d.head_dim_pad, d.hidden, p.lin1_waves, p.tail ? " (q | k | v)" : "");
             break;
@@ -187,7 +190,8 @@
             break;
         case 2: {
             const AttnPlan &a = p.attn[bi & 1];
-            pr.label(2, "%s", a.form == AttnForm::linear ? "k_attention_linear" : a.stream() ? "k_attention_stream" : "k_attention_rows / k_attention_tiny");
+            if (tfuse) pr.label(2, "(inside k_lin1_tfuse: no attention launch)");
+            else pr.label(2, "%s", a.form == AttnForm::linear ? "k_attention_linear" : a.stream() ? "k_attention_stream" : "k_attention_rows / k_attention_tiny");
             break;
         }
         default: break;
@@ -240,7 +244,8 @@
     const bool lnf = p.lin1_lnf(bi);
     const float premul = m->attention_linear ? 1.0f : (float)(1.4426950408889634 / std::sqrt((double)d.head_dim));
     const int pdiv = temporal ? p.L : 1, pmod = temporal ? p.T : p.L;
-    label_block(m, p, bi);
+    const bool tfuse = p.tfuse && temporal && !tg;
+    label_block(m, p, bi, tfuse);
     if (!p.a_from_tail(bi) && !lnf) {
         m->prof.begin(3, st);
         DISPATCH_D(D, launch_ln_mod_t, ws.a, ws.h, mbase, mbase + D, mod_stride, n, tpt, st);
@@ -254,17 +259,21 @@
         const Lin1Args la{(const u16 *)bw.w1, lnf ? (const u16 *)ws.h : ws.a, bw.b1, ws.rope_qk + (size_t)(2 * bi) * ws.rope_qk_stride,
                           ws.rope_qk + (size_t)(2 * bi + 1) * ws.rope_qk_stride, ws.qkv, ws.z, p.F1, n, m->HHD, d.mlp_dim,
                           pdiv, pmod, magic_of(pdiv), magic_of(pmod), 1.0f / d.head_dim, premul, 1, 0, p.planes[temporal] ? 1 : 0, p.npad,
-                          ws.lnstat, mbase, mbase + D, mod_stride, tpt, magic_of(tpt)};
-        launch_linear1_ts(d.head_dim_pad, D, p.lin1_waves, lnf, la, st);
+                          ws.lnstat, mbase, mbase + D, mod_stride, tpt, magic_of(tpt),
+                          p.T, p.L, p.bc * (p.L / 8), ws.kmax2 + bi, ws.kmax2 + 2 * d.depth + bi};
+        if (tfuse) launch_linear1_tf(lnf, la, st);
+        else launch_linear1_ts(d.head_dim_pad, D, p.lin1_waves, lnf, la, st);
     } else if (d.head_dim_pad == 32) launch_linear1_gemm<32>(m, ws, p, bi, pdiv, pmod, premul, st);
     else launch_linear1_gemm<16>(m, ws, p, bi, pdiv, pmod, premul, st);
     m->prof.end(0, st);
 
-    const AttnArgs aa = attention_args(m, ws, p, bi, premul);
-    m->prof.begin(2, st);
-    if (d.head_dim_pad == 32) launch_attention_t<32>(p.attn[temporal], aa, st);
-    else launch_attention_t<16>(p.attn[temporal], aa, st);
-    m->prof.end(2, st);
+    if (!tfuse) {
+        const AttnArgs aa = attention_args(m, ws, p, bi, premul);
+        m->prof.begin(2, st);
+        if (d.head_dim_pad == 32) launch_attention_t<32>(p.attn[temporal], aa, st);
+        else launch_attention_t<16>(p.attn[temporal], aa, st);
+        m->prof.end(2, st);
+    }
     if (p.lin2 == Lin2Kind::none) {
         LSL_CHECK_LAUNCH("block");
         return 0;
diff --git a/lam_slide_amd/csrc/host_launch.hip.h b/lam_slide_amd/csrc/host_launch.hip.h
--- a/lam_slide_amd/csrc/host_launch.hip.h
+++ b/lam_slide_amd/csrc/host_launch.hip.h
@@ -218,6 +218,35 @@
         }
         launch_linear1_ts_t<H, K, 8>(a, st);
     });
+}
+
+bool linear1_tf_shape_ok(bool on, bool eval_mode, bool lin1_ts, bool tail, bool attn_short, int hdp, int D, int F1, int T, int L, int zw) {
+    if (!on || !eval_mode || !lin1_ts || tail || !attn_short) return false;
+    if (hdp != 32 || D != 512 || T < 9 || T > 32 || L % 8 != 0) return false;
+    if (32ull * (unsigned)L * 2ull * (unsigned)zw >= (1ull << 32)) return false;
+    return Lin1Cfg<32, 512, 8>::lds_bytes_tf(F1) <= LDS_BUDGET;
+}
+bool linear1_tf_ok(bool eval_mode, bool lin1_ts, bool tail, bool attn_short, int hdp, int D, int F1, int T, int L, int zw) {
+    const int on = env_int("LSL_LIN1_TFUSE", 1);
+    return linear1_tf_shape_ok(on != 0, eval_mode, lin1_ts, tail, attn_short, hdp, D, F1, T, L, zw);
+}
+template <bool LNF>
+void launch_linear1_tf_t(const Lin1Args &a, hipStream_t st) {
+    using C = Lin1Cfg<32, 512, 8>;
+    auto kern = k_lin1_tfuse<LNF>;
+    LSL_ALLOW_LDS(kern, LDS_BUDGET);
+    const int ntile = a.tf_tiles, nb = a.F / 32;
+    const long units = (long)ntile * nb;
+    int grid = (int)std::min<long>(device_cus(), units / 2);
+    Lin1Args b = a;
+    const int qb3 = 3 * (a.HHD / 32), wpt = std::min(device_cus() / ntile, qb3 / 6 + (nb - qb3) / 2);
+    b.wpt = wpt >= 2 ? wpt : 0;
+    if (b.wpt) grid = b.wpt * ntile;
+    hipLaunchKernelGGL(kern, dim3(grid), dim3(512), C::lds_bytes_tf(a.F), st, b);
+}
+void launch_linear1_tf(bool lnf, const Lin1Args &a, hipStream_t st) {
+    if (lnf) launch_linear1_tf_t<true>(a, st);
+    else launch_linear1_tf_t<false>(a, st);
 }
 
 #define LSL_LIN2_WS_INSTANCES(X) X(1536, 3, 3) X(1280, 4, 4) X(768, 3, 3) X(384, 3, 3)
diff --git a/lam_slide_amd/csrc/k_lin1.hip.h b/lam_slide_amd/csrc/k_lin1.hip.h
--- a/lam_slide_amd/csrc/k_lin1.hip.h
+++ b/lam_slide_amd/csrc/k_lin1.hip.h
@@ -1,4 +1,5 @@
 #pragma once
+#include "k_attn.hip.h"
 #include "k_mm_frag.hip.h"
 
 struct Lin1Args {
@@ -20,6 +21,8 @@
     const float *ln_shift, *ln_scale;
     int ln_mod_stride, ln_tpt;
     unsigned ln_tpt_magic;
+    int tf_T, tf_L, tf_tiles;
+    const float *kmax2, *qmax2;
 };
 
 #ifndef LIN1_B2
@@ -46,13 +49,14 @@
     static constexpr size_t lds_bytes(int F) { return (size_t)RING + STAGE + (size_t)F * 4; }
     static constexpr int LN_SLOTS = K <= 256 ? 3 : 2;
     static constexpr size_t lds_bytes_lnf(int F) { return lds_bytes(F) + (size_t)LN_SLOTS * 2 * K * 4; }
+    static constexpr int TF_TAB = 32 * (HDP / 2) * 16;
+    static constexpr size_t lds_bytes_tf(int F) { return lds_bytes(F) + 2 * (size_t)TF_TAB; }
 };
 
 #define LSL_LIN1_TS_INSTANCES(X) X(32, 128) X(32, 256) X(32, 384) X(32, 512) X(16, 128) X(16, 256) X(16, 384) X(16, 512)
 
 bool lsl_lin1_launch(int hdp, int K, int waves, bool lnf, const Lin1Args &a, int grid, size_t lds, hipStream_t st);
 
-#ifndef LSL_LIN1_HOST_SIDE
 
 enum { LIN1_QK = 0, LIN1_V = 1, LIN1_MLP = 2 };
 
@@ -71,11 +75,12 @@
     return fmaf(-ax, h, relu);
 }
 
-template <int HDP, int K, int NW = 8, bool LNF = false>
-__global__ void __launch_bounds__(NW * 64, NW / 4) k_linear1_ts(Lin1Args g) {
+template <int HDP, int K, int NW, bool LNF, bool TF>
+__device__ __forceinline__ void lin1_ts_body(const Lin1Args g) {
     using C = Lin1Cfg<HDP, K, NW>;
     constexpr int KS = C::KS, BLK = C::BLK, PPW = C::PPW, ROWB = C::ROWB;
     constexpr int NCO = HDP == 32 ? 8 : 4;
+    static_assert(!TF || (HDP == 32 && K == 512 && NW == 8), "the fused temporal form: hidden 512, 32-wide heads, 8 waves");
     extern __shared__ __attribute__((aligned(16))) char smem[];
 
     const int tid = threadIdx.x, lane = tid & 63;
@@ -85,10 +90,25 @@
     float *const bias_lds = reinterpret_cast<float *>(smem + C::RING + C::STAGE);
 
     const int NB = g.F >> 5;
-    const int ntile = (g.N + C::TT - 1) / C::TT;
+    const int ntile = TF ? g.tf_tiles : (g.N + C::TT - 1) / C::TT;
     const long U = (long)ntile * NB;
+    const int qb3 = 3 * (g.HHD >> 5);
+    auto tf_cut_blk = [&](int o) __attribute__((always_inline)) { return o < qb3 ? o - o % 6 : o & ~1; };
+    auto tf_cut = [&](long x) __attribute__((always_inline)) {
+        const long t = x / NB;
+        return t * NB + tf_cut_blk((int)(x - t * NB));
+    };
     long i0, i1;
-    if (g.wpt > 0) {
+    if constexpr (TF) {
+        if (g.wpt > 0) {
+            const int tile = blockIdx.x / g.wpt, part = blockIdx.x - tile * g.wpt;
+            i0 = (long)tile * NB + tf_cut_blk(NB * part / g.wpt);
+            i1 = (long)tile * NB + (part + 1 == g.wpt ? NB : tf_cut_blk(NB * (part + 1) / g.wpt));
+        } else {
+            i0 = tf_cut(U * blockIdx.x / gridDim.x);
+            i1 = blockIdx.x + 1 == gridDim.x ? U : tf_cut(U * (blockIdx.x + 1) / gridDim.x);
+        }
+    } else if (g.wpt > 0) {
         const int tile = blockIdx.x / g.wpt, part = blockIdx.x - tile * g.wpt;
         i0 = (long)tile * NB + ((NB * part / g.wpt) & ~1);
         i1 = (long)tile * NB + (part + 1 == g.wpt ? NB : ((NB * (part + 1) / g.wpt) & ~1));
@@ -99,6 +119,18 @@
     if (i0 >= i1) return;
 
     for (int i = tid * 4; i < g.F; i += NW * 64 * 4) *reinterpret_cast<float4 *>(bias_lds + i) = *reinterpret_cast<const float4 *>(g.bias + i);
+    static_assert(C::RING % 256 == 0 && C::STAGE % 256 == 0, "the rotation tables' rows: XOR-addressed 256-byte lines");
+    const unsigned tf_tab = (unsigned)(size_t)(LDS_PTR(char))(smem) + C::RING + C::STAGE + (unsigned)g.F * 4;
+    auto tf_fill = [&](const float4 *tab, unsigned dst, int n_thr) __attribute__((always_inline)) {
+        if (tid < n_thr) {
+            const int p = tid >> 4, e = tid & 15;
+            *reinterpret_cast<LDS_PTR(f32x4_t)>(dst + p * 256 + ((e ^ (p & 15)) << 4)) = reinterpret_cast<const f32x4_t *>(tab)[min(p, g.tf_T - 1) * 16 + e];
+        }
+    };
+    if constexpr (TF) {
+        tf_fill(g.rope_q, tf_tab, 512);
+        tf_fill(g.rope_k, tf_tab + C::TF_TAB, 512);
+    }
 
     const unsigned lds0 = (unsigned)(size_t)(LDS_PTR(char))(smem);
     const unsigned lane_src = lane * 16;
@@ -117,7 +149,14 @@
                 asm volatile("s_add_u32 m0, %2, %3\n\ts_nop 0\n\tglobal_load_lds_dwordx4 %0, %1 offset:%4" ::"v"(ls), "s"(src), "s"(dst), "n"(16 * I), "n"(ROWB * I) : "memory", "scc");
         }
     };
-    auto req_src = [&](int blk) __attribute__((always_inline)) { return w_rows + (size_t)blk * (32 * ROWB); };
+    auto vsrc = [&](int u) __attribute__((always_inline)) {
+        if constexpr (!TF) return u;
+        else {
+            const int h = (u * 43691) >> 17;
+            return __builtin_amdgcn_readfirstlane(u < qb3 ? (u - 3 * h) * (g.HHD >> 5) + h : u);
+        }
+    };
+    auto req_src = [&](int blk) __attribute__((always_inline)) { return w_rows + (size_t)vsrc(blk) * (32 * ROWB); };
     auto req_dst = [&](int slot) __attribute__((always_inline)) { return lds0 + slot * BLK + PPW * wave * C::PITCH; };
     auto issue = [&](int blk, int slot) __attribute__((always_inline)) {
         const char *src = req_src(blk);
@@ -133,6 +172,9 @@
     int dma_blk, dma_slot;
     int n_wave = 0;
     float post = 1.0f;
+    const unsigned tf_pos = TF ? (unsigned)min(r, g.tf_T - 1) : 0u;
+    const unsigned co_row = tf_tab + tf_pos * 256 + (((2 * hf) ^ (tf_pos & 15)) << 4);
+    unsigned co_tab = 0;
 
     auto advance = [&](int &b) __attribute__((always_inline)) { b = b + 1 == NB ? 0 : b + 1; };
     auto next_slot = [&](int s) __attribute__((always_inline)) { return s == C::NS - 1 ? 0 : s + 1; };
@@ -150,18 +192,21 @@
     auto init_acc = [&](f32x16 &a, int blk) __attribute__((always_inline)) {
 #pragma unroll
         for (int q4 = 0; q4 < 4; ++q4) {
-            const float4 b = *reinterpret_cast<const float4 *>(bias_lds + blk * 32 + 8 * q4 + 4 * hf);
+            const float4 b = *reinterpret_cast<const float4 *>(bias_lds + vsrc(blk) * 32 + 8 * q4 + 4 * hf);
             a[4 * q4] = b.x; a[4 * q4 + 1] = b.y; a[4 * q4 + 2] = b.z; a[4 * q4 + 3] = b.w;
         }
     };
     constexpr bool B2 = LIN1_B2 != 0 && K <= LIN1_B2_KMAX;
-    auto step_head = [&](auto flushed_c) __attribute__((always_inline)) {
-        if (B2) {
-            if (decltype(flushed_c)::value) wait_vmcnt<PPW>();
+    static_assert(!TF || !B2, "the fused temporal form counts its stores per single block step");
+    auto step_head = [&](auto flushed_c, bool none) __attribute__((always_inline)) {
+        constexpr int STORES = decltype(flushed_c)::value;
+        if (TF && none) {
+            wait_vmcnt<PPW>();
+        } else if (B2) {
+            if (STORES) wait_vmcnt<PPW>();
             else wait_vmcnt<0>();
         } else {
-            if (decltype(flushed_c)::value) wait_vmcnt<PPW + 4>();
-            else wait_vmcnt<PPW>();
+            wait_vmcnt<PPW + STORES>();
         }
         __builtin_amdgcn_s_barrier();
         asm volatile("" ::: "memory");
@@ -175,28 +220,46 @@
     const unsigned stride_q = planes ? PROW : 2u * 3 * g.HHD, stride_z = 2u * (g.HHD + g.M);
     const unsigned blk_q = planes ? (32 / HDP) * plane_bytes : 64u;
     const unsigned voff_q = planes ? ((lane & 7) / CPH) * plane_bytes + (lane >> 3) * PROW + 16 * ((lane & 7) % CPH) : (lane >> 3) * stride_q + 16 * (lane & 7);
-    const unsigned voff_z = (lane >> 3) * stride_z + 16 * (lane & 7);
+    const unsigned tf_ls = TF ? (unsigned)g.tf_L * stride_z : 0u;
+    const unsigned voff_z = TF ? 4 * (lane >> 3) * tf_ls + 16 * (lane & 7) : (lane >> 3) * stride_z + 16 * (lane & 7);
+    const unsigned rd_tf = (unsigned)(size_t)(LDS_PTR(char))(stage) + (lane >> 3) * 512 + (((lane & 7) ^ (4 * ((lane >> 3) & 1))) << 4);
     const int slab_z = 3 * (g.HHD >> 5);
     const char *fl_base = nullptr;
     unsigned fl_stride8 = 0, fl_voff = 0;
     auto flush_setup = [&](int b_even) __attribute__((always_inline)) {
-        const bool to_qkv = b_even < slab_z;
-        fl_base = to_qkv ? row_q : row_z;
-        fl_stride8 = 8 * (to_qkv ? stride_q : stride_z);
-        fl_voff = to_qkv ? voff_q + blk_q * (unsigned)b_even : voff_z + 64u * (unsigned)b_even;
-    };
+        if constexpr (TF) {
+            fl_base = row_z;
+            fl_stride8 = tf_ls;
+            fl_voff = voff_z + 64u * (unsigned)b_even;
+        } else {
+            const bool to_qkv = b_even < slab_z;
+            fl_base = to_qkv ? row_q : row_z;
+            fl_stride8 = 8 * (to_qkv ? stride_q : stride_z);
+            fl_voff = to_qkv ? voff_q + blk_q * (unsigned)b_even : voff_z + 64u * (unsigned)b_even;
+        }
+    };
+    auto tf_slot_ok = [&](int j) __attribute__((always_inline)) { return 4 * (lane >> 3) + j < g.tf_T; };
     auto flush_read = [&](int half, u32x4 (&pk)[2]) __attribute__((always_inline)) {
 #pragma unroll
-        for (int i = 0; i < 2; ++i) pk[i] = *reinterpret_cast<const LDS_PTR(u32x4)>(rd0 + 1024 * (2 * half + i));
+        for (int i = 0; i < 2; ++i) {
+            if constexpr (TF) pk[i] = *reinterpret_cast<const LDS_PTR(u32x4)>((rd_tf ^ (unsigned)(16 * (2 * half + i))) + 128 * (2 * half + i));
+            else pk[i] = *reinterpret_cast<const LDS_PTR(u32x4)>(rd0 + 1024 * (2 * half + i));
+        }
     };
     auto flush_store = [&](int half, const u32x4 (&pk)[2]) __attribute__((always_inline)) {
-        stream_store16<true>(fl_voff + (2 * half) * fl_stride8, pk[0], fl_base);
-        stream_store16<false>(fl_voff + (2 * half + 1) * fl_stride8, pk[1], fl_base);
+        if constexpr (TF) {
+            if (tf_slot_ok(2 * half)) stream_store16<true>(fl_voff + (2 * half) * fl_stride8, pk[0], fl_base);
+            if (tf_slot_ok(2 * half + 1)) stream_store16<true>(fl_voff + (2 * half + 1) * fl_stride8, pk[1], fl_base);
+        } else {
+            stream_store16<true>(fl_voff + (2 * half) * fl_stride8, pk[0], fl_base);
+            stream_store16<false>(fl_voff + (2 * half + 1) * fl_stride8, pk[1], fl_base);
+        }
     };
     auto flush_store_visible = [&](int half, const u32x4 (&pk)[2]) __attribute__((always_inline)) {
 #pragma unroll
         for (int i = 0; i < 2; ++i)
-            __builtin_nontemporal_store(pk[i], reinterpret_cast<u32x4 *>(const_cast<char *>(fl_base) + (size_t)(fl_voff + (2 * half + i) * fl_stride8)));
+            if (!TF || tf_slot_ok(2 * half + i))
+                __builtin_nontemporal_store(pk[i], reinterpret_cast<u32x4 *>(const_cast<char *>(fl_base) + (size_t)(fl_voff + (2 * half + i) * fl_stride8)));
     };
     auto put_group = [&](int ii, int q, float v0, float v1, float v2, float v3) __attribute__((always_inline)) {
         const u32x2 pk = {pack2(v0, v1), pack2(v2, v3)};
@@ -215,7 +278,14 @@
                 const int q = s - 2;
                 float o[4];
 #pragma unroll
-                for (int kk = 0; kk < 2; ++kk) rope_pair(c0, co[2 * q + kk], a[2 * (2 * q + kk)], a[2 * (2 * q + kk) + 1], o[2 * kk], o[2 * kk + 1]);
+                for (int kk = 0; kk < 2; ++kk) {
+                    if constexpr (TF) {
+                        const f32x4_t cv = *reinterpret_cast<const LDS_PTR(f32x4_t)>((co_row ^ (unsigned)((4 * q + kk) << 4)) + co_tab);
+                        const float4 cf = make_float4(cv[0], cv[1], cv[2], cv[3]);
+                        rope_pair(c0, cf, a[2 * (2 * q + kk)], a[2 * (2 * q + kk) + 1], o[2 * kk], o[2 * kk + 1]);
+                    } else
+                        rope_pair(c0, co[2 * q + kk], a[2 * (2 * q + kk)], a[2 * (2 * q + kk) + 1], o[2 * kk], o[2 * kk + 1]);
+                }
                 put_group(ii, q, o[0], o[1], o[2], o[3]);
             }
         } else if constexpr (SEC == LIN1_QK) {
@@ -250,7 +320,7 @@
     auto step = [&](auto sec_c, auto par_c, auto mfma_c, auto epi_c, auto side) __attribute__((always_inline)) {
         constexpr int PAR = decltype(par_c)::value;
         constexpr bool DO_MFMA = decltype(mfma_c)::value != 0, DO_EPI = decltype(epi_c)::value != 0;
-        constexpr int MPS = KS / 8, PD = LIN1_PD, MH = (MPS + 1) / 2;
+        constexpr int MPS = KS / 8, PD = (TF && !LNF) ? 2 : LIN1_PD, MH = (MPS + 1) / 2;
         f32x16 &ac = PAR ? acc0 : acc1;
         const f32x16 &ae = PAR ? acc1 : acc0;
         const char *sb = smem + slot_c * BLK + aoff;
@@ -283,11 +353,13 @@
     };
     ic<0> I0;
     ic<1> I1;
+    ic<2> I2;
+    ic<4> I4;
     auto no_side = [](auto) __attribute__((always_inline)) {};
-    auto fused = [&](auto sec_c, auto par_c, auto flush_c, auto prev_c, int e) __attribute__((always_inline)) {
+    auto fused = [&](auto sec_c, auto par_c, auto flush_c, auto prev_c, int e, bool seg_first = false) __attribute__((always_inline)) {
         constexpr int PAR = decltype(par_c)::value;
         constexpr bool FLUSH = decltype(flush_c)::value != 0;
-        if (!B2 || PAR == 1) step_head(prev_c);
+        if (!B2 || PAR == 1) step_head(prev_c, seg_first);
         u32x4 pk[2];
         if (FLUSH) flush_setup(e - 2);
         const char *src = req_src(dma_blk);
@@ -341,7 +413,7 @@
         }
         for (; e + 1 < eb; e += 2) {
             fused(sec_c, I0, I1, I0, e);
-            fused(sec_c, I1, I0, I1, e + 1);
+            fused(sec_c, I1, I0, I4, e + 1);
         }
         if (e < eb) fused(sec_c, I0, I1, I0, e);
     };
@@ -355,8 +427,17 @@
     ic<LIN1_MLP> SMLP;
 
     constexpr bool XLINES = LIN1_XLOAD != 0 && (K <= 384 || LIN1_XLOAD >= 2);
+    auto tf_row0 = [&](int t) __attribute__((always_inline)) {
+        const int tpj = g.tf_L >> 3, b = t / tpj;
+        return b * g.tf_T * g.tf_L + 8 * (t - b * tpj) + wave;
+    };
     auto load_x = [&](int nw) __attribute__((always_inline)) {
-        if (!XLINES) {
+        if constexpr (TF) {
+            static_assert(!TF || !XLINES, "fragment-shaped loads: a lane's row is its frame");
+            const u16 *xr = g.X + ((size_t)nw + (size_t)tf_pos * g.tf_L) * K + 8 * hf;
+#pragma unroll
+            for (int ks = 0; ks < KS; ++ks) xreg[ks] = as_bf16x8(*reinterpret_cast<const u32x4 *>(xr + 16 * ks));
+        } else if (!XLINES) {
             const u16 *xr = g.X + (size_t)(nw + r) * K + 8 * hf;
 #pragma unroll
             for (int ks = 0; ks < KS; ++ks) xreg[ks] = as_bf16x8(*reinterpret_cast<const u32x4 *>(xr + 16 * ks));
@@ -380,14 +461,14 @@
         }
     };
 
-    float *const ln_tab = bias_lds + ((g.F + 3) & ~3);
+    float *ln_tab = bias_lds + ((g.F + 3) & ~3);
     auto traj_of = [&](unsigned n) __attribute__((always_inline)) { return magic_div(n, g.ln_tpt_magic); };
     auto load_x_lnf = [&](int tile_, int nw) __attribute__((always_inline)) {
         typedef __attribute__((ext_vector_type(4))) float f4;
         const float *xf = reinterpret_cast<const float *>(g.X);
-        const unsigned t_first = g.ln_mod_stride ? traj_of((unsigned)(tile_ * C::TT)) : 0u;
+        const unsigned t_first = g.ln_mod_stride ? traj_of((unsigned)(TF ? nw : tile_ * C::TT)) : 0u;
         const unsigned t_last = g.ln_mod_stride ? traj_of((unsigned)(g.N - 1)) : 0u;
-        for (int i = tid * 4; i < C::LN_SLOTS * K; i += NW * 64 * 4) {
+        for (int i = tid * 4; i < (TF ? 1 : C::LN_SLOTS) * K; i += NW * 64 * 4) {
             const int slot = i / K, col = i - slot * K;
             const size_t mo = (size_t)min(t_first + (unsigned)slot, t_last) * g.ln_mod_stride + col;
             const f4 sc = *reinterpret_cast<const f4 *>(g.ln_scale + mo), sh = *reinterpret_cast<const f4 *>(g.ln_shift + mo);
@@ -398,14 +479,16 @@
         const unsigned sbase = (unsigned)(size_t)(LDS_PTR(char))(stage);
         const unsigned xr0 = sbase + rl * 128;
         const unsigned tab0 = (unsigned)(size_t)(LDS_PTR(char))(ln_tab) + 16 * chunk;
-        const float *xr = xf + (size_t)(nw + rowi) * K + 4 * chunk;
+        const float *xr = xf + (size_t)(nw + (TF ? 0 : rowi)) * K + 4 * chunk;
         float2 st[4];
         unsigned tb[4];
+        unsigned fo[4];
 #pragma unroll
         for (int q = 0; q < 4; ++q) {
-            const unsigned nn = (unsigned)min(nw + (int)rowi + 8 * q, g.N - 1);
+            fo[q] = TF ? (unsigned)min((int)rowi + 8 * q, g.tf_T - 1) * (unsigned)g.tf_L : 0u;
+            const unsigned nn = TF ? (unsigned)nw + fo[q] : (unsigned)min(nw + (int)rowi + 8 * q, g.N - 1);
             st[q] = g.ln_stat[nn];
-            const unsigned slot = g.ln_mod_stride ? min(traj_of(nn) - t_first, (unsigned)(C::LN_SLOTS - 1)) : 0u;
+            const unsigned slot = (!TF && g.ln_mod_stride) ? min(traj_of(nn) - t_first, (unsigned)(C::LN_SLOTS - 1)) : 0u;
             tb[q] = tab0 + slot * (2 * K * 4);
         }
         __syncthreads();
@@ -415,7 +498,7 @@
 #pragma unroll
             for (int e = 0; e < 2; ++e)
 #pragma unroll
-                for (int q = 0; q < 4; ++q) v[e][q] = *reinterpret_cast<const f4 *>(xr + (size_t)(8 * q) * K + 64 * p + 32 * e);
+                for (int q = 0; q < 4; ++q) v[e][q] = *reinterpret_cast<const f4 *>(xr + (TF ? (size_t)fo[q] : (size_t)(8 * q)) * K + 64 * p + 32 * e);
 #pragma unroll
             for (int q = 0; q < 4; ++q) {
                 const unsigned row = rowi + 8 * q, sw = (row >> 1) & 7;
@@ -435,6 +518,101 @@
             __builtin_amdgcn_sched_barrier(0);
         }
     };
+    const unsigned st_lds = (unsigned)(size_t)(LDS_PTR(char))(stage);
+    const unsigned fr0 = (st_lds + r * 128 + ((r & 7) << 4)) ^ (unsigned)(16 * hf);
+    unsigned vt0 = 0;
+    {
+        const int gi = lane & 15, gq = gi >> 2, gp = gi & 3, grp = lane >> 4, rv = 4 * (grp >> 1) + gq;
+        vt0 = st_lds + stage_off(rv, 2 * (grp & 1) + (gp >> 1)) + 8 * (gp & 1);
+    }
+    const unsigned voff_o = TF ? 2 * (lane >> 2) * tf_ls + 16 * (lane & 3) : 0u;
+    const bool tf_ragged = TF && (g.tf_T & 31) != 0;
+    float tf_kmax2 = 0.0f;
+    bool tf_all_shifted = false;
+    if constexpr (TF) {
+        tf_kmax2 = *g.kmax2;
+        tf_all_shifted = sqrtf(*g.qmax2 * tf_kmax2) * g.q_premul * 1.02f <= 60.0f;
+    }
+    u32x4 tf_pw0 = {0u, 0u, 0u, 0u}, tf_pw1 = {0u, 0u, 0u, 0u};
+    float tf_inv_l = 0.0f;
+    auto attn_scores = [&](auto hq_c, auto hk_c) __attribute__((always_inline)) {
+        constexpr unsigned HQ = 64 * decltype(hq_c)::value, HK = 64 * decltype(hk_c)::value;
+        bf16x8 qf[2], kf[2];
+#pragma unroll
+        for (int s2 = 0; s2 < 2; ++s2) {
+            qf[s2] = as_bf16x8(*reinterpret_cast<const LDS_PTR(u32x4)>(fr0 ^ (HQ + 32 * s2)));
+            kf[s2] = as_bf16x8(*reinterpret_cast<const LDS_PTR(u32x4)>(fr0 ^ (HK + 32 * s2)));
+        }
+        f32x16 zero;
+#pragma unroll
+        for (int e = 0; e < 16; ++e) zero[e] = 0.0f;
+        auto scores = [&](const f32x16 &init) __attribute__((always_inline)) {
+            f32x16 t = mfma32(kf[0], qf[0], init);
+            t = mfma32(kf[1], qf[1], t);
+            if (tf_ragged) {
+#pragma unroll
+                for (int e = 0; e < 16; ++e)
+                    if (acc_row(e, hf) >= g.tf_T) t[e] = -INFINITY;
+            }
+            return t;
+        };
+        float mx = -INFINITY;
+        bool shifted = tf_all_shifted;
+        if (!tf_all_shifted) {
+            float qq = sq_norm(qf);
+            qq += xhalf(qq);
+            const float m = sqrtf(qq * tf_kmax2) * 1.02f;
+            shifted = __ballot(m > 60.0f) == 0;
+            if (shifted) mx = m;
+        }
+        f32x16 t;
+        if (shifted) t = scores(zero);
+        else {
+            const f32x16 t0 = scores(zero);
+            float mc = -INFINITY;
+#pragma unroll
+            for (int e = 0; e < 16; ++e) mc = fmaxf(mc, t0[e]);
+            mx = fmaxf(mc, xhalf(mc));
+            f32x16 negmx;
+#pragma unroll
+            for (int e = 0; e < 16; ++e) negmx[e] = -mx;
+            t = scores(negmx);
+        }
+        float p[16];
+#pragma unroll
+        for (int e = 0; e < 16; ++e) p[e] = __builtin_amdgcn_exp2f(t[e]);
+        tf_pw0 = p_frag(p, p + 4);
+        tf_pw1 = p_frag(p + 8, p + 12);
+        const u32x4 ones_w = {0x3F803F80u, 0x3F803F80u, 0x3F803F80u, 0x3F803F80u};
+        f32x16 lsum = mfma32(as_bf16x8(ones_w), as_bf16x8(tf_pw0), zero);
+        lsum = mfma32(as_bf16x8(ones_w), as_bf16x8(tf_pw1), lsum);
+        tf_inv_l = 1.0f / lsum[0];
+    };
+    auto attn_out = [&](auto hv_c, int head) __attribute__((always_inline)) {
+        constexpr int HV = decltype(hv_c)::value;
+        f32x16 o;
+#pragma unroll
+        for (int e = 0; e < 16; ++e) o[e] = 0.0f;
+#pragma unroll
+        for (int s2 = 0; s2 < 2; ++s2) {
+            const unsigned va = (vt0 ^ (unsigned)(64 * HV)) + 2048 * s2;
+            const s16x4 v0 = __builtin_amdgcn_ds_read_tr16_b64_v4i16((LDS_PTR(s16x4))(va));
+            const s16x4 v1 = __builtin_amdgcn_ds_read_tr16_b64_v4i16((LDS_PTR(s16x4))(va + 1024));
+            const s16x8 vv = {v0[0], v0[1], v0[2], v0[3], v1[0], v1[1], v1[2], v1[3]};
+            o = mfma32(__builtin_bit_cast(bf16x8, vv), as_bf16x8(s2 ? tf_pw1 : tf_pw0), o);
+        }
+#pragma unroll
+        for (int q4 = 0; q4 < 4; ++q4) *reinterpret_cast<LDS_PTR(u32x2)>(wr0 ^ (unsigned)(64 * HV + 16 * q4)) = o_pack(o, tf_inv_l, q4);
+        const char *ob = uni_ptr(row_z + 4 * (size_t)g.HHD + 64 * (size_t)head);
+        const int slot0 = 2 * (lane >> 2), c = lane & 3;
+#pragma unroll
+        for (int k = 0; k < 2; ++k) {
+            const u32x4 v = *reinterpret_cast<const LDS_PTR(u32x4)>(st_lds + stage_off(slot0 + k, 4 * HV + c));
+            if (slot0 + k < g.tf_T) stream_store16<true>(voff_o + k * tf_ls, v, ob);
+        }
+    };
+    bool tf_qkv_end = false;
+
     const int qb = g.HHD >> 5;
     int tile = (int)(i0 / NB), b0 = (int)(i0 - (long)tile * NB), left = (int)(i1 - i0);
     bool first_seg = true;
@@ -442,18 +620,24 @@
     __syncthreads();
     while (left > 0) {
         const int b1 = NB - b0 < left ? NB : b0 + left;
-        n_wave = tile * C::TT + wave * 32;
+        if constexpr (TF) n_wave = tf_row0(tile);
+        else n_wave = tile * C::TT + wave * 32;
         row_q = reinterpret_cast<const char *>(g.qkv) + (size_t)n_wave * stride_q;
         row_z = reinterpret_cast<const char *>(g.z) + (size_t)n_wave * stride_z - 4 * (size_t)g.HHD;
+        if constexpr (TF && LNF) {
+            __syncthreads();
+            ln_tab = reinterpret_cast<float *>(smem + dma_slot * BLK);
+        }
         if constexpr (LNF) load_x_lnf(tile, n_wave);
         else {
-            if (first_seg) load_x(n_wave);
+            if (first_seg || TF) load_x(n_wave);
             finish_x();
         }
         const unsigned nn = (unsigned)min(n_wave + r, g.N - 1);
         const unsigned pos = token_pos(nn, g.div_magic, g.mod_magic, g.pos_mod);
 
         if (first_seg) wait_vmcnt<0>();
+        else if (TF && tf_qkv_end) wait_vmcnt<2>();
         else wait_vmcnt<4>();
         __builtin_amdgcn_s_barrier();
         asm volatile("" ::: "memory");
@@ -467,6 +651,50 @@
         }
         init_acc(acc0, b0);
         step(SV, I1, I1, I0, no_side);
+        if constexpr (TF) {
+            const int left_next = left - (b1 - b0);
+            int e = b0;
+            for (const int qe = min(b1, qb3); e < qe; e += 6) {
+                const int head = (e * 43691) >> 17;
+                const bool sf = e == b0;
+                post = g.q_premul, co_tab = 0;
+                fused(SQK, I0, I0, I2, e, sf);
+                post = 1.0f, co_tab = C::TF_TAB;
+                fused(SQK, I1, I0, I2, e + 1, sf);
+                attn_scores(I0, I1);
+                fused(SV, I0, I0, I0, e + 2);
+                attn_out(I0, head);
+                post = g.q_premul, co_tab = 0;
+                fused(SQK, I1, I0, I2, e + 3);
+                post = 1.0f, co_tab = C::TF_TAB;
+                fused(SQK, I0, I0, I2, e + 4);
+                attn_scores(I1, I0);
+                if (e + 6 < b1) fused(SV, I1, I0, I0, e + 5);
+                else step(SV, I1, I0, I1, no_side);
+                attn_out(I1, head + 1);
+            }
+            tf_qkv_end = b1 <= qb3;
+            if (b1 > qb3) {
+                const int m0 = max(b0, qb3);
+                fused(SMLP, I0, I0, I2, m0, m0 == b0);
+                if (m0 + 2 < b1) {
+                    fused(SMLP, I1, I0, I0, m0 + 1);
+                    run(SMLP, m0 + 2, b1 - 1);
+                }
+                step(SMLP, I1, I0, I1, no_side);
+                flush_setup(b1 - 2);
+                u32x4 pk[2];
+                flush_read(0, pk);
+                flush_store_visible(0, pk);
+                flush_read(1, pk);
+                flush_store_visible(1, pk);
+            }
+            left = left_next;
+            tile += 1;
+            b0 = 0;
+            first_seg = false;
+            continue;
+        }
         const int e_end = b1 - 1;
         if (b0 < 2 * qb) {
             if (!co_ready) load_co(b0 < qb ? g.rope_q : g.rope_k, pos);
@@ -537,4 +765,12 @@
     wait_vmcnt<0>();
 }
 
-#endif
+template <int HDP, int K, int NW = 8, bool LNF = false>
+__global__ void __launch_bounds__(NW * 64, NW / 4) k_linear1_ts(Lin1Args g) {
+    lin1_ts_body<HDP, K, NW, LNF, false>(g);
+}
+
+template <bool LNF>
+__global__ void __launch_bounds__(512, 2) k_lin1_tfuse(Lin1Args g) {
+    lin1_ts_body<32, 512, 8, LNF, true>(g);
+}
diff --git a/lam_slide_amd/csrc/lsl_api.hip b/lam_slide_amd/csrc/lsl_api.hip
--- a/lam_slide_amd/csrc/lsl_api.hip
+++ b/lam_slide_amd/csrc/lsl_api.hip
@@ -14,7 +14,6 @@
 
 #include "k_attn.hip.h"
 #include "k_gemm.hip.h"
-#define LSL_LIN1_HOST_SIDE
 #include "k_lin1.hip.h"
 #include "k_lin2.hip.h"
 #include "k_tail.hip.h"
@@ -509,6 +508,30 @@
     return 0;
 } LSL_API_CATCH
 
+int lsl_debug_block_z(lsl_model *m, int32_t bi, const float *h_in, float *h_out, void *z_out, const float *mods, int32_t mod_rows, int32_t B,
+                      int32_t T, int32_t L, void *workspace, size_t workspace_bytes, void *stream) try {
+    DeviceGuard dev_guard_((hipStream_t)stream);
+    const bool args_ok = (mod_rows == 1 || mod_rows == B) && h_in && h_out && z_out && mods;
+    if (int rc = check_debug(m, bi, args_ok, B, T, L, workspace, workspace_bytes)) return rc;
+    hipStream_t st = (hipStream_t)stream;
+    const Workspace ws = carve(m, (char *)workspace, B, T, L);
+    PassPlan plan;
+    if (int rc = plan_pass(m, ws, B, T, L, mod_rows == 1 ? 0 : m->MODW, PlanMode::debug_block, bi, plan, true)) return rc;
+    run_tables(m, ws, T, L, st);
+    const size_t n = (size_t)B * T * L;
+    hipMemcpyAsync(ws.h, h_in, n * m->d.hidden * 4, hipMemcpyDeviceToDevice, st);
+    hipMemsetAsync(ws.z, 0xff, n * m->K2 * 2, st);
+    if (int rc = run_block(m, ws, plan, bi, mods, st)) return rc;
+    hipMemcpyAsync(h_out, ws.h, n * m->d.hidden * 4, hipMemcpyDeviceToDevice, st);
+    hipMemcpyAsync(z_out, ws.z, n * m->K2 * 2, hipMemcpyDeviceToDevice, st);
+    return 0;
+} LSL_API_CATCH
+
+int lsl_debug_tfuse_gate(int32_t enabled, int32_t eval_mode, int32_t lin1_ts, int32_t tail, int32_t attn_short, int32_t head_dim_pad, int32_t hidden,
+                         int32_t F1, int32_t T, int32_t L, int32_t z_width) {
+    return linear1_tf_shape_ok(enabled != 0, eval_mode != 0, lin1_ts != 0, tail != 0, attn_short != 0, head_dim_pad, hidden, F1, T, L, z_width) ? 1 : 0;
+}
+
 int lsl_debug_block(lsl_model *m, int32_t bi, const float *h_in, float *h_out, const float *mods, int32_t B, int32_t T, int32_t L,
                     void *workspace, size_t workspace_bytes, void *stream) {
     return lsl_debug_block_ex(m, bi, h_in, h_out, nullptr, mods, B, B, T, L, workspace, workspace_bytes, stream);
```
